# Mamo1031/Multimodal-MTRSSM

Measured on AMD Instinct MI355X. Metric: seq-steps/s (BxT) MoPoE-MRSSM train step, higher is better.
Workload: dtype bf16x2-split, fp32 accumulate; 1 GPU; BASELINE configs[1]: MoPoE-MRSSM train step, B=64/GPU T=50 deter=200 stoch=30, vision 1x64x64 + audio 1x128x32 + action 4; global_batch=64, seq_len=50, parallelism=dp1, hidden=200, embed=256, categoricals_x_classes=6x5, residual_blocks=3, activation=ELU, optimizer=AdamW lr 1e-3 + clip 10 (fused HIP), params=4151600, streams=1, launch=eager (host enqueues every launch), backend=none, rccl_ranks=0, collective_ranks=0, noise=uniforms keyed by global batch row (parallel.GlobalRowNoise)

## Files before the change

### include/mtrssm.h

```cpp
#ifndef MTRSSM_H
#define MTRSSM_H

#include <stddef.h>
#include <stdint.h>

#ifdef __cplusplus
extern "C" {
#endif

#define MTRSSM_VERSION 100

#define MTRSSM_OK 0
#define MTRSSM_EINVAL (-1)
#define MTRSSM_ELAUNCH (-2)
#define MTRSSM_ELDS (-3)

#define MTRSSM_ACT_IDENTITY 0
#define MTRSSM_ACT_RELU 1
#define MTRSSM_ACT_ELU 2
#define MTRSSM_ACT_TANH 3

int mtrssm_version(void);
const char* mtrssm_last_error(void);
const char* mtrssm_last_kernel(void);

typedef struct MtrssmMrssmDims {
  int32_t B, T;
  int32_t D, H;
  int32_t K, C;
  int32_t act;
  int32_t post;
  float kl_w_post;
  float kl_w_prior;
  int32_t rows_per_block;
  int32_t threads;
} MtrssmMrssmDims;

typedef struct MtrssmMrssmFwdWeights {
  const float* w1s_t;
  const float* w2_t;
  const float* b2;
  const float* wih_t;
  const float* bih;
  const float* whh_t;
  const float* bhh;
  const float* wh1_t;
  const float* b3;
  const float* w4;
  const float* b4;
  const float* wa2;
  const float* ba2;
  const float* wv2;
  const float* bv2;
} MtrssmMrssmFwdWeights;

typedef struct MtrssmMrssmFwdIO {
  const float* xa;
  const float* pa;
  const float* pv;
  const float* deter0;
  const float* stoch0;
  const float* u_post;
  const float* u_prior;
  float* deter;
  float* prior_logits;
  float* prior_stoch;
  float* post_logits;
  float* post_stoch;
  float* kl;
  float* sv_h1;
  float* sv_h2;
  float* sv_gates;
  float* sv_heads;
  float* sv_la;
  float* sv_lv;
  const int32_t* modality;
} MtrssmMrssmFwdIO;

int mtrssm_mrssm_rollout_fwd(const MtrssmMrssmDims* dims, const MtrssmMrssmFwdWeights* w,
                             const MtrssmMrssmFwdIO* io, void* stream);

typedef struct MtrssmMrssmClusterWeights {
  const float* w1s_t;
  const float* wf_t;
  const float* bf;
  const float* whh_t;
  const float* bhh;
  const float* wh1_t;
  const float* b3;
  const float* w4;
  const float* b4;
  const float* wa2;
  const float* ba2;
  const float* wv2;
  const float* bv2;
} MtrssmMrssmClusterWeights;
int mtrssm_mrssm_cluster_supported(const MtrssmMrssmDims* dims);
int64_t mtrssm_mrssm_cluster_workspace_bytes(const MtrssmMrssmDims* dims);
int mtrssm_mrssm_rollout_fwd_cluster(const MtrssmMrssmDims* dims, const MtrssmMrssmClusterWeights* weights, const MtrssmMrssmFwdIO* io,
                                     void* workspace, int64_t workspace_bytes, void* stream);

typedef struct MtrssmMrssmBwdWeights {
  const float* w1s_t;
  const float* w2;
  const float* wih;
  const float* whh;
  const float* wh1;
  const float* w4;
  const float* wa2;
  const float* wv2;
} MtrssmMrssmBwdWeights;

typedef struct MtrssmMrssmBwdIO {
  const float* deter0;
  const float* deter;
  const float* prior_logits;
  const float* post_logits;
  const float* sv_h1;
  const float* sv_h2;
  const float* sv_gates;
  const float* sv_heads;
  const float* sv_la;
  const float* sv_lv;
  const float* g_deter;
  const float* g_post_stoch;
  const float* g_prior_stoch;
  const float* g_post_logits;
  const float* g_prior_logits;
  const float* g_kl;
  float* g_deter0;
  float* g_stoch0;
  float* d_z1;
  float* d_h2;
  float* d_gi;
  float* d_gh;
  float* d_zh;
  float* d_lp;
  float* d_la;
  float* d_lv;
  const int32_t* modality;
} MtrssmMrssmBwdIO;

int64_t mtrssm_mrssm_cluster_bwd_workspace_bytes(const MtrssmMrssmDims* dims);
int mtrssm_mrssm_rollout_bwd_cluster(const MtrssmMrssmDims* dims, const MtrssmMrssmClusterWeights* weights, const MtrssmMrssmBwdIO* io,
                                     void* workspace, int64_t workspace_bytes, void* stream);

int mtrssm_mrssm_wide_supported(const MtrssmMrssmDims* dims, int32_t pieces);
int64_t mtrssm_mrssm_wide_workspace_bytes(const MtrssmMrssmDims* dims, int32_t pieces);
int64_t mtrssm_mrssm_wide_bwd_workspace_bytes(const MtrssmMrssmDims* dims, int32_t pieces);
int mtrssm_mrssm_rollout_fwd_wide(const MtrssmMrssmDims* dims, const MtrssmMrssmClusterWeights* weights, const MtrssmMrssmFwdIO* io,
                                  int32_t pieces, void* workspace, int64_t workspace_bytes, void* stream);
int mtrssm_mrssm_rollout_bwd_wide(const MtrssmMrssmDims* dims, const MtrssmMrssmClusterWeights* weights, const MtrssmMrssmBwdIO* io,
                                  int32_t pieces, void* workspace, int64_t workspace_bytes, void* stream);

int mtrssm_mrssm_rollout_bwd(const MtrssmMrssmDims* dims, const MtrssmMrssmBwdWeights* w,
                             const MtrssmMrssmBwdIO* io, void* stream);

typedef struct MtrssmMmtrssmDims {
  int32_t B, T;
  int32_t LD, HD;
  int32_t H;
  int32_t KL, CL;
  int32_t KH, CH;
  int32_t act;
  int32_t post;
  float tau_l, tau_h;
  float keep_l, keep_h;
  float kl_w_post, kl_w_prior;
  int32_t rows_per_block;
  int32_t threads;
} MtrssmMmtrssmDims;

typedef struct MtrssmMmtrssmFwdWeights {
  const float* wxl_s_t;
  const float* wdl_t;
  const float* wxh_t;
  const float* wdh_t;
  const float* bh;
  const float* wl1_t;
  const float* bl1;
  const float* wh1_t;
  const float* bh1;
  const float* wlp2;
  const float* blp2;
  const float* wa2;
  const float* ba2;
  const float* wv2;
  const float* bv2;
  const float* whp2;
  const float* bhp2;
  const float* whq2;
  const float* bhq2;
} MtrssmMmtrssmFwdWeights;

typedef struct MtrssmMmtrssmFwdIO {
  const float* xl;
  const float* pa;
  const float* pv;
  const float* deter_l0;
  const float* deter_h0;
  const float* hidden_l0;
  const float* hidden_h0;
  const float* stoch_l0;
  const float* stoch_h0;
  const float* u_post_l;
  const float* u_post_h;
  const float* u_prior_l;
  const float* u_prior_h;
  float* deter_l;
  float* deter_h;
  float* hidden_l;
  float* hidden_h;
  float* prior_logits_l;
  float* prior_logits_h;
  float* prior_stoch_l;
  float* prior_stoch_h;
  float* post_logits_l;
  float* post_logits_h;
  float* post_stoch_l;
  float* post_stoch_h;
  float* kl_l;
  float* kl_h;
  float* sv_l1;
  float* sv_h1;
  float* sv_la;
  float* sv_lv;
  const int32_t* modality;
} MtrssmMmtrssmFwdIO;

int mtrssm_mmtrssm_rollout_fwd(const MtrssmMmtrssmDims* dims, const MtrssmMmtrssmFwdWeights* w,
                               const MtrssmMmtrssmFwdIO* io, void* stream);

typedef struct MtrssmMmtrssmBwdWeights {
  const float* wxl_s_t;
  const float* wdl;
  const float* wxh_t;
  const float* wdh;
  const float* wl1;
  const float* wh1;
  const float* wlp2;
  const float* wa2;
  const float* wv2;
  const float* whp2;
  const float* whq2;
} MtrssmMmtrssmBwdWeights;

typedef struct MtrssmMmtrssmBwdIO {
  const float* deter_l0;
  const float* deter_h0;
  const float* deter_l;
  const float* deter_h;
  const float* prior_logits_l;
  const float* prior_logits_h;
  const float* post_logits_l;
  const float* post_logits_h;
  const float* sv_l1;
  const float* sv_h1;
  const float* sv_la;
  const float* sv_lv;
  const float* g_deter_l;
  const float* g_deter_h;
  const float* g_hidden_l;
  const float* g_hidden_h;
  const float* g_post_stoch_l;
  const float* g_post_stoch_h;
  const float* g_prior_stoch_l;
  const float* g_prior_stoch_h;
  const float* g_post_logits_l;
  const float* g_post_logits_h;
  const float* g_prior_logits_l;
  const float* g_prior_logits_h;
  const float* g_kl_l;
  const float* g_kl_h;
  float* g_deter_l0;
  float* g_deter_h0;
  float* g_hidden_l0;
  float* g_hidden_h0;
  float* g_stoch_l0;
  float* g_stoch_h0;
  float* d_ul;
  float* d_uh;
  float* d_zl1;
  float* d_zh1;
  float* d_lpl;
  float* d_la;
  float* d_lv;
  float* d_lph;
  float* d_lqh;
  const int32_t* modality;
} MtrssmMmtrssmBwdIO;

int mtrssm_mmtrssm_rollout_bwd(const MtrssmMmtrssmDims* dims, const MtrssmMmtrssmBwdWeights* w,
                               const MtrssmMmtrssmBwdIO* io, void* stream);

int mtrssm_mmtrssm_wide_supported(const MtrssmMmtrssmDims* dims, int32_t pieces);
int64_t mtrssm_mmtrssm_wide_workspace_bytes(const MtrssmMmtrssmDims* dims, int32_t pieces);
int64_t mtrssm_mmtrssm_wide_bwd_workspace_bytes(const MtrssmMmtrssmDims* dims, int32_t pieces);
int mtrssm_mmtrssm_rollout_fwd_wide(const MtrssmMmtrssmDims* dims, const MtrssmMmtrssmFwdWeights* w, const MtrssmMmtrssmFwdIO* io,
                                    int32_t pieces, void* workspace, int64_t workspace_bytes, void* stream);
int mtrssm_mmtrssm_rollout_bwd_wide(const MtrssmMmtrssmDims* dims, const MtrssmMmtrssmBwdWeights* w, const MtrssmMmtrssmBwdIO* io,
                                    int32_t pieces, void* workspace, int64_t workspace_bytes, void* stream);

typedef struct MtrssmConvGeom {
  int32_t N;
  int32_t C, Hs, Ws;
  int32_t C2;
  int32_t Cpad;
  int32_t KH, KW;
  int32_t SS, TS, OFFY, OFFX;
  int32_t Hq, Wq;
  int32_t OS, QY, QX;
  int32_t Ho, Wo;
  int32_t Cout, CoutPad;
  int32_t pre_act;
  int32_t act;
  int32_t mfma_split;
} MtrssmConvGeom;

int mtrssm_conv_gather_gemm(const MtrssmConvGeom* g, const float* src, const float* src2, const float* wp, const uint16_t* wq,
                            const float* bias, const float* actgrad_in, const float* add_in, float* out, void* stream);
int mtrssm_conv_gather_gemm_pair(const MtrssmConvGeom* ga, const float* srca, const float* src2a, const float* wpa, const uint16_t* wqa,
                                 const float* biasa, const float* actgrada, const float* adda, float* outa,
                                 const MtrssmConvGeom* gb, const float* srcb, const float* src2b, const float* wpb, const uint16_t* wqb,
                                 const float* biasb, const float* actgradb, const float* addb, float* outb, void* stream);
int mtrssm_conv_gather_pair_merges(const MtrssmConvGeom* ga, const MtrssmConvGeom* gb, int32_t has_wq);
int mtrssm_residual_block_fwd_supported(const MtrssmConvGeom* g3);
int mtrssm_residual_block_fwd(const MtrssmConvGeom* ga, const float* xa, const uint16_t* wq3a, const float* b3a, const float* w1a,
                              const float* b1a, float* ha, float* ya, const MtrssmConvGeom* gb, const float* xb, const uint16_t* wq3b,
                              const float* b3b, const float* w1b, const float* b1b, float* hb, float* yb, void* stream);
int mtrssm_pack_conv_weight(const float* w, int32_t O, int32_t I, int32_t KH, int32_t KW, int64_t so, int64_t si, int64_t sh,
                            int64_t sw, int32_t OPad, int32_t IPad, int32_t pieces, float* wp, uint16_t* wq, void* stream);
#define MTRSSM_PACK_DESC_WORDS 16
int mtrssm_pack_conv_weights(const int64_t* table, int32_t count, int32_t blocks_per_weight, void* stream);
int mtrssm_conv_weight_grad(const MtrssmConvGeom* g, const float* a, const float* src, const float* src2,
                            int32_t pre_act_a, float* dwp, float* dbias, void* workspace, int64_t workspace_bytes, void* stream);
int mtrssm_conv_weight_grad_deferred(const MtrssmConvGeom* g, const float* a, const float* src, const float* src2,
                                     int32_t pre_act_a, float* dwp, float* dbias, void* workspace, int64_t workspace_bytes, void* stream);
int mtrssm_conv_weight_grad_reduce(void* stream);
int mtrssm_conv_weight_grad_src_bias_supported(const MtrssmConvGeom* g, int32_t pre_act_a);
int mtrssm_residual_bwd1x1_supported(const MtrssmConvGeom* g);
int mtrssm_residual_bwd1x1(const MtrssmConvGeom* g, const float* gy, const float* h, const uint16_t* wq1t, float* gh, float* dwp,
                           float* dbias, void* workspace, int64_t workspace_bytes, int32_t defer, void* stream);
int mtrssm_conv_weight_grad_src_bias(const MtrssmConvGeom* g, const float* a, const float* src, int32_t pre_act_a, float* dwp,
                                     float* dsrc_bias, void* workspace, int64_t workspace_bytes, int32_t defer, void* stream);
int64_t mtrssm_conv_weight_grad_workspace_bytes(const MtrssmConvGeom* g, int32_t pre_act_a);
int mtrssm_unpack_conv_grads(const int64_t* table, int32_t count, int32_t blocks_per_entry, void* stream);
int mtrssm_convt_quad_supported(const MtrssmConvGeom* g4);
int mtrssm_convt_quad(const MtrssmConvGeom* ga4, const float* srca, const uint16_t* const* wqa4, const float* biasa, const float* actgrada,
                      float* outa, const MtrssmConvGeom* gb4, const float* srcb, const uint16_t* const* wqb4, const float* biasb,
                      const float* actgradb, float* outb, void* stream);
int mtrssm_convt_k4s2_thin(int32_t N, int32_t C, int32_t Hs, int32_t Ws, int32_t Cout, const float* src, const float* w,
                           const float* bias, int32_t pre_act, int32_t act, float* out, void* stream);
int mtrssm_convt_k4s2_band_supported(int32_t N, int32_t C, int32_t Hs, int32_t Ws, int32_t Cout);
int mtrssm_convt_k4s2_band(int32_t N, int32_t C, int32_t Hs, int32_t Ws, int32_t Cout, const float* src, const float* w,
                           const float* bias, int32_t pre_act, int32_t act, float* out, void* stream);
int mtrssm_conv_tgather_thin(int32_t N, int32_t O, int32_t Hs, int32_t Ws, int32_t Cout, int32_t KH, int32_t KW, int32_t stride, int32_t pad,
                             int32_t Ho, int32_t Wo, const float* y, const float* w, const float* bias, int32_t pre_act, int32_t act,
                             const float* actgrad_in, const float* add_in, float* out, void* stream);
int mtrssm_channel_sum(const float* x, int32_t N, int32_t C, int32_t HW, float* out, void* stream);

int mtrssm_episode_gather(const float* store, const int64_t* idx, const float* noise, int64_t n_episodes, int64_t B, int64_t T,
                          int64_t Tfull, int64_t E, float std_, float* input, float* target, void* stream);
int mtrssm_episode_gather_window(const float* store, const int64_t* idx, const int32_t* start, const float* noise, int64_t n_episodes,
                                 int64_t B, int64_t T, int64_t Tfull, int64_t E, float std_, float* input, float* target, void* stream);
int mtrssm_episode_gather_ragged(const float* store, const int64_t* idx, const int32_t* start, const int32_t* lengths, const float* noise,
                                 int64_t n_episodes, int64_t B, int64_t T, int64_t Tfull, int64_t E, float std_, float* input, float* target,
                                 int32_t* valid_out, void* stream);
int mtrssm_episode_gather_seeded(const float* store, const int64_t* idx, const int32_t* start, const int32_t* lengths, int32_t* valid_out,
                                 uint32_t key0, uint32_t key1, uint32_t epoch, int64_t n_episodes, int64_t B, int64_t T, int64_t Tfull,
                                 int64_t E, float std_, float* input, float* target, void* stream);

#define MTRSSM_STATE_MAX 6
typedef struct MtrssmStateTable {
  int32_t count;
  int32_t width[MTRSSM_STATE_MAX];
  int64_t src_stride[MTRSSM_STATE_MAX];
  const float* src[MTRSSM_STATE_MAX];
  const float* alt[MTRSSM_STATE_MAX];
  float* dst[MTRSSM_STATE_MAX];
} MtrssmStateTable;
int mtrssm_state_select(const MtrssmStateTable* table, const uint8_t* reset, int64_t B, void* stream);
int mtrssm_state_save(const MtrssmStateTable* table, int64_t B, int64_t steps, void* stream);
int mtrssm_state_save_at(const MtrssmStateTable* table, const int32_t* last, int64_t B, int64_t steps, void* stream);

int mtrssm_elbo_combine_fwd(const float* nll_a, const float* nll_v, const float* kl0, const float* kl1, int64_t n, float c0, float c1,
                            float* o_recon, float* o_k0, float* o_k1, float* o_loss, void* stream);
int mtrssm_elbo_combine_bwd(const float* g_recon, const float* g_k0, const float* g_k1, const float* g_loss, int64_t n, float c0, float c1,
                            float* g_nll_a, float* g_nll_v, float* g_kl0, float* g_kl1, void* stream);
int mtrssm_elbo_combine_counted_fwd(const float* nll_a, const float* nll_v, const float* kl0, const float* kl1, const float* live,
                                    const float* count, int64_t n, float c0, float c1, float* o_recon, float* o_k0, float* o_k1,
                                    float* o_loss, void* stream);
int mtrssm_elbo_combine_counted_bwd(const float* g_recon, const float* g_k0, const float* g_k1, const float* g_loss, const float* live,
                                    const float* count, int64_t n, float c0, float c1, float* g_nll_a, float* g_nll_v, float* g_kl0,
                                    float* g_kl1, void* stream);
int mtrssm_categorical_sample_fwd(const float* logits, const float* u, int64_t rows, int32_t K, int32_t C, float* logp, float* probs,
                                  float* onehot, void* stream);
int mtrssm_categorical_sample_bwd(const float* probs, const float* g_probs, const float* g_logp, int64_t rows, int32_t K, int32_t C,
                                  float* d_logits, void* stream);
int mtrssm_gaussian_nll_fwd(const float* pred, const float* target, int64_t frames, int64_t event, int32_t act,
                            float* out, void* stream);
int mtrssm_gaussian_nll_bwd(const float* pred, const float* target, const float* g_out,
                            int64_t frames, int64_t event, int32_t act, float* g_pred, void* stream);

int mtrssm_gaussian_nll_masked_fwd(const float* pred, const float* target, const float* present, const float* count,
                                   int64_t frames, int64_t event, int32_t act, float* out, void* stream);
int mtrssm_gaussian_nll_masked_bwd(const float* pred, const float* target, const float* present, const float* count,
                                   const float* g_out, int64_t frames, int64_t event, int32_t act, float* g_pred, void* stream);

int mtrssm_modality_dropout(const float* u, int64_t b_global, int64_t steps, int64_t span, float p_audio, float p_vision,
                            int64_t row0, int64_t b_local, int32_t* codes, float* present_audio, float* present_vision,
                            uint8_t* mask0, float* counts, void* stream);

int mtrssm_step_mask_ragged(const int32_t* valid, const float* u, int64_t b_global, int64_t steps, int64_t span, float p_audio,
                            float p_vision, int64_t row0, int64_t b_local, int32_t* codes, float* present_audio, float* present_vision,
                            float* live, uint8_t* mask0, int32_t* last, float* counts, void* stream);

int mtrssm_step_mask_forecast(const int32_t* valid, const float* u_mask, const float* u_context, int64_t b_global, int64_t steps,
                              int64_t span, float p_audio, float p_vision, int64_t lo, int64_t hi, int64_t row0, int64_t b_local,
                              int32_t* codes, float* seen_audio, float* seen_vision, float* target, float* observed, uint8_t* mask0,
                              int32_t* last, float* counts, void* stream);

int mtrssm_sumsq(const float* x, int64_t n, float* out, void* stream);
int mtrssm_adamw_step(float* param, const float* grad, float* exp_avg, float* exp_avg_sq, int64_t n,
                      const float* sumsq, float clip_norm, float grad_scale, float lr, float beta1,
                      float beta2, float eps, float weight_decay, int32_t step, void* stream);
int mtrssm_clear(void* p, int64_t bytes, void* stream);
int mtrssm_adamw_prepare(const float* grad, int64_t n, float* sumsq, float* state, const int32_t* status, float beta1, float beta2,
                         void* stream);
int mtrssm_adamw_apply(float* param, const float* grad, float* exp_avg, float* exp_avg_sq, const uint8_t* active, int64_t n,
                       const float* sumsq, const float* state, const int32_t* status, float clip_norm, float grad_scale, float beta1,
                       float beta2, float eps, float weight_decay, void* stream);

typedef struct MtrssmGemm {
  const float* A;
  const float* B;
  float* C;
  const float* bias;
  const float* zgrad;
  float* colsum;
  int32_t M, N, R, lda, ldb, ldc, ldz;
  int32_t a_rmajor, b_rmajor, act_a, act_b, act_out, act_z, accumulate, split_r;
  int32_t* tickets;
  int32_t n_tickets;
  int32_t mfma_split;
} MtrssmGemm;
int mtrssm_gemm(const MtrssmGemm* g, void* stream);
int mtrssm_gemm_group(const MtrssmGemm* problems, int32_t count, void* stream);

#ifdef __cplusplus
}
#endif
#endif
```

### multimodal_mtrssm_amd/_lib.py

```python

from __future__ import annotations

import ctypes as C
import os
from pathlib import Path

import torch
from torch import Tensor

_HERE = Path(__file__).resolve().parent
LIB_PATH = _HERE / "libmtrssm_hip.so"

ACT_IDS = {"Identity": 0, "ReLU": 1, "ELU": 2, "Tanh": 3}

_f = C.c_float
_i = C.c_int32
_p = C.c_void_p


def _struct(name: str, fields: list[tuple[str, type]]) -> type:
    return type(name, (C.Structure,), {"_fields_": fields})


def _ptrs(*names: str) -> list[tuple[str, type]]:
    return [(n, _p) for n in names]


MrssmDims = _struct("MtrssmMrssmDims", [
    ("B", _i), ("T", _i), ("D", _i), ("H", _i), ("K", _i), ("C", _i), ("act", _i), ("post", _i),
    ("kl_w_post", _f), ("kl_w_prior", _f), ("rows_per_block", _i), ("threads", _i),
])
MrssmFwdWeights = _struct("MtrssmMrssmFwdWeights", _ptrs(
    "w1s_t", "w2_t", "b2", "wih_t", "bih", "whh_t", "bhh", "wh1_t", "b3", "w4", "b4", "wa2", "ba2", "wv2", "bv2"))
MrssmFwdIO = _struct("MtrssmMrssmFwdIO", _ptrs(
    "xa", "pa", "pv", "deter0", "stoch0", "u_post", "u_prior",
    "deter", "prior_logits", "prior_stoch", "post_logits", "post_stoch", "kl",
    "sv_h1", "sv_h2", "sv_gates", "sv_heads", "sv_la", "sv_lv", "modality"))
MrssmClusterWeights = _struct("MtrssmMrssmClusterWeights", _ptrs(
    "w1s_t", "wf_t", "bf", "whh_t", "bhh", "wh1_t", "b3", "w4", "b4", "wa2", "ba2", "wv2", "bv2"))
MrssmBwdWeights = _struct("MtrssmMrssmBwdWeights", _ptrs("w1s_t", "w2", "wih", "whh", "wh1", "w4", "wa2", "wv2"))
MrssmBwdIO = _struct("MtrssmMrssmBwdIO", _ptrs(
    "deter0", "deter", "prior_logits", "post_logits", "sv_h1", "sv_h2", "sv_gates", "sv_heads", "sv_la", "sv_lv",
    "g_deter", "g_post_stoch", "g_prior_stoch", "g_post_logits", "g_prior_logits", "g_kl",
    "g_deter0", "g_stoch0", "d_z1", "d_h2", "d_gi", "d_gh", "d_zh", "d_lp", "d_la", "d_lv", "modality"))

MmtrssmDims = _struct("MtrssmMmtrssmDims", [
    ("B", _i), ("T", _i), ("LD", _i), ("HD", _i), ("H", _i), ("KL", _i), ("CL", _i), ("KH", _i), ("CH", _i),
    ("act", _i), ("post", _i), ("tau_l", _f), ("tau_h", _f), ("keep_l", _f), ("keep_h", _f),
    ("kl_w_post", _f), ("kl_w_prior", _f), ("rows_per_block", _i), ("threads", _i),
])
MmtrssmFwdWeights = _struct("MtrssmMmtrssmFwdWeights", _ptrs(
    "wxl_s_t", "wdl_t", "wxh_t", "wdh_t", "bh", "wl1_t", "bl1", "wh1_t", "bh1",
    "wlp2", "blp2", "wa2", "ba2", "wv2", "bv2", "whp2", "bhp2", "whq2", "bhq2"))
MmtrssmFwdIO = _struct("MtrssmMmtrssmFwdIO", _ptrs(
    "xl", "pa", "pv", "deter_l0", "deter_h0", "hidden_l0", "hidden_h0", "stoch_l0", "stoch_h0",
    "u_post_l", "u_post_h", "u_prior_l", "u_prior_h",
    "deter_l", "deter_h", "hidden_l", "hidden_h", "prior_logits_l", "prior_logits_h", "prior_stoch_l", "prior_stoch_h",
    "post_logits_l", "post_logits_h", "post_stoch_l", "post_stoch_h", "kl_l", "kl_h",
    "sv_l1", "sv_h1", "sv_la", "sv_lv", "modality"))
MmtrssmBwdWeights = _struct("MtrssmMmtrssmBwdWeights", _ptrs(
    "wxl_s_t", "wdl", "wxh_t", "wdh", "wl1", "wh1", "wlp2", "wa2", "wv2", "whp2", "whq2"))
MmtrssmBwdIO = _struct("MtrssmMmtrssmBwdIO", _ptrs(
    "deter_l0", "deter_h0", "deter_l", "deter_h", "prior_logits_l", "prior_logits_h", "post_logits_l", "post_logits_h",
    "sv_l1", "sv_h1", "sv_la", "sv_lv",
    "g_deter_l", "g_deter_h", "g_hidden_l", "g_hidden_h", "g_post_stoch_l", "g_post_stoch_h", "g_prior_stoch_l",
    "g_prior_stoch_h", "g_post_logits_l", "g_post_logits_h", "g_prior_logits_l", "g_prior_logits_h", "g_kl_l", "g_kl_h",
    "g_deter_l0", "g_deter_h0", "g_hidden_l0", "g_hidden_h0", "g_stoch_l0", "g_stoch_h0",
    "d_ul", "d_uh", "d_zl1", "d_zh1", "d_lpl", "d_la", "d_lv", "d_lph", "d_lqh", "modality"))

ConvGeom = _struct("MtrssmConvGeom", [(n, _i) for n in (
    "N", "C", "Hs", "Ws", "C2", "Cpad", "KH", "KW", "SS", "TS", "OFFY", "OFFX", "Hq", "Wq", "OS", "QY", "QX", "Ho", "Wo",
    "Cout", "CoutPad", "pre_act", "act", "mfma_split")])

Gemm = _struct("MtrssmGemm", _ptrs("A", "B", "C", "bias", "zgrad", "colsum") + [(n, _i) for n in (
    "M", "N", "R", "lda", "ldb", "ldc", "ldz", "a_rmajor", "b_rmajor", "act_a", "act_b", "act_out", "act_z", "accumulate", "split_r")]
    + [("tickets", _p), ("n_tickets", _i), ("mfma_split", _i)])

STATE_MAX = 6
StateTable = _struct("MtrssmStateTable", [
    ("count", _i), ("width", _i * STATE_MAX), ("src_stride", C.c_int64 * STATE_MAX), ("src", _p * STATE_MAX), ("alt", _p * STATE_MAX),
    ("dst", _p * STATE_MAX)])

SYMBOLS: dict[str, tuple[type | None, list[type]]] = {
    "mtrssm_version": (C.c_int, []),
    "mtrssm_last_error": (C.c_char_p, []),
    "mtrssm_last_kernel": (C.c_char_p, []),
    "mtrssm_mrssm_rollout_fwd": (C.c_int, [C.POINTER(MrssmDims), C.POINTER(MrssmFwdWeights), C.POINTER(MrssmFwdIO), _p]),
    "mtrssm_mrssm_cluster_supported": (C.c_int, [C.POINTER(MrssmDims)]),
    "mtrssm_mrssm_cluster_workspace_bytes": (C.c_int64, [C.POINTER(MrssmDims)]),
    "mtrssm_mrssm_rollout_fwd_cluster": (C.c_int, [C.POINTER(MrssmDims), C.POINTER(MrssmClusterWeights), C.POINTER(MrssmFwdIO), _p, C.c_int64, _p]),
    "mtrssm_mrssm_cluster_bwd_workspace_bytes": (C.c_int64, [C.POINTER(MrssmDims)]),
    "mtrssm_mrssm_rollout_bwd_cluster": (C.c_int, [C.POINTER(MrssmDims), C.POINTER(MrssmClusterWeights), C.POINTER(MrssmBwdIO), _p, C.c_int64, _p]),
    "mtrssm_mrssm_wide_supported": (C.c_int, [C.POINTER(MrssmDims), _i]),
    "mtrssm_mrssm_wide_workspace_bytes": (C.c_int64, [C.POINTER(MrssmDims), _i]),
    "mtrssm_mrssm_wide_bwd_workspace_bytes": (C.c_int64, [C.POINTER(MrssmDims), _i]),
    "mtrssm_mrssm_rollout_fwd_wide": (C.c_int, [C.POINTER(MrssmDims), C.POINTER(MrssmClusterWeights), C.POINTER(MrssmFwdIO), _i, _p, C.c_int64, _p]),
    "mtrssm_mrssm_rollout_bwd_wide": (C.c_int, [C.POINTER(MrssmDims), C.POINTER(MrssmClusterWeights), C.POINTER(MrssmBwdIO), _i, _p, C.c_int64, _p]),
    "mtrssm_mrssm_rollout_bwd": (C.c_int, [C.POINTER(MrssmDims), C.POINTER(MrssmBwdWeights), C.POINTER(MrssmBwdIO), _p]),
    "mtrssm_mmtrssm_rollout_fwd": (C.c_int, [C.POINTER(MmtrssmDims), C.POINTER(MmtrssmFwdWeights), C.POINTER(MmtrssmFwdIO), _p]),
    "mtrssm_mmtrssm_rollout_bwd": (C.c_int, [C.POINTER(MmtrssmDims), C.POINTER(MmtrssmBwdWeights), C.POINTER(MmtrssmBwdIO), _p]),
    "mtrssm_mmtrssm_wide_supported": (C.c_int, [C.POINTER(MmtrssmDims), _i]),
    "mtrssm_mmtrssm_wide_workspace_bytes": (C.c_int64, [C.POINTER(MmtrssmDims), _i]),
    "mtrssm_mmtrssm_wide_bwd_workspace_bytes": (C.c_int64, [C.POINTER(MmtrssmDims), _i]),
    "mtrssm_mmtrssm_rollout_fwd_wide": (C.c_int, [C.POINTER(MmtrssmDims), C.POINTER(MmtrssmFwdWeights), C.POINTER(MmtrssmFwdIO), _i, _p, C.c_int64, _p]),
    "mtrssm_mmtrssm_rollout_bwd_wide": (C.c_int, [C.POINTER(MmtrssmDims), C.POINTER(MmtrssmBwdWeights), C.POINTER(MmtrssmBwdIO), _i, _p, C.c_int64, _p]),
    "mtrssm_conv_gather_gemm": (C.c_int, [C.POINTER(ConvGeom), _p, _p, _p, _p, _p, _p, _p, _p, _p]),
    "mtrssm_conv_gather_gemm_pair": (C.c_int, [C.POINTER(ConvGeom), _p, _p, _p, _p, _p, _p, _p, _p,
                                               C.POINTER(ConvGeom), _p, _p, _p, _p, _p, _p, _p, _p, _p]),
    "mtrssm_conv_gather_pair_merges": (C.c_int, [C.POINTER(ConvGeom), C.POINTER(ConvGeom), _i]),
    "mtrssm_residual_block_fwd_supported": (C.c_int, [C.POINTER(ConvGeom)]),
    "mtrssm_residual_block_fwd": (C.c_int, [C.POINTER(ConvGeom), _p, _p, _p, _p, _p, _p, _p, C.POINTER(ConvGeom), _p, _p, _p, _p, _p, _p, _p, _p]),
    "mtrssm_pack_conv_weight": (C.c_int, [_p, _i, _i, _i, _i, C.c_int64, C.c_int64, C.c_int64, C.c_int64, _i, _i, _i, _p, _p, _p]),
    "mtrssm_pack_conv_weights": (C.c_int, [_p, _i, _i, _p]),
    "mtrssm_unpack_conv_grads": (C.c_int, [_p, _i, _i, _p]),
    "mtrssm_conv_weight_grad": (C.c_int, [C.POINTER(ConvGeom), _p, _p, _p, _i, _p, _p, _p, C.c_int64, _p]),
    "mtrssm_conv_weight_grad_deferred": (C.c_int, [C.POINTER(ConvGeom), _p, _p, _p, _i, _p, _p, _p, C.c_int64, _p]),
    "mtrssm_residual_bwd1x1_supported": (C.c_int, [C.POINTER(ConvGeom)]),
    "mtrssm_residual_bwd1x1": (C.c_int, [C.POINTER(ConvGeom), _p, _p, _p, _p, _p, _p, _p, C.c_int64, _i, _p]),
    "mtrssm_conv_weight_grad_src_bias_supported": (C.c_int, [C.POINTER(ConvGeom), _i]),
    "mtrssm_conv_weight_grad_src_bias": (C.c_int, [C.POINTER(ConvGeom), _p, _p, _i, _p, _p, _p, C.c_int64, _i, _p]),
    "mtrssm_conv_weight_grad_reduce": (C.c_int, [_p]),
    "mtrssm_conv_weight_grad_workspace_bytes": (C.c_int64, [C.POINTER(ConvGeom), _i]),
    "mtrssm_channel_sum": (C.c_int, [_p, _i, _i, _i, _p, _p]),
    "mtrssm_convt_k4s2_thin": (C.c_int, [_i, _i, _i, _i, _i, _p, _p, _p, _i, _i, _p, _p]),
    "mtrssm_convt_k4s2_band_supported": (C.c_int, [_i, _i, _i, _i, _i]),
    "mtrssm_convt_k4s2_band": (C.c_int, [_i, _i, _i, _i, _i, _p, _p, _p, _i, _i, _p, _p]),
    "mtrssm_convt_quad_supported": (C.c_int, [C.POINTER(ConvGeom)]),
    "mtrssm_convt_quad": (C.c_int, [C.POINTER(ConvGeom), _p, C.POINTER(C.c_void_p), _p, _p, _p, C.POINTER(ConvGeom), _p, C.POINTER(C.c_void_p),
                                    _p, _p, _p, _p]),
    "mtrssm_conv_tgather_thin": (C.c_int, [_i] * 11 + [_p, _p, _p, _i, _i, _p, _p, _p, _p]),
    "mtrssm_episode_gather": (C.c_int, [_p, _p, _p, C.c_int64, C.c_int64, C.c_int64, C.c_int64, C.c_int64, _f, _p, _p, _p]),
    "mtrssm_episode_gather_window": (C.c_int, [_p, _p, _p, _p, C.c_int64, C.c_int64, C.c_int64, C.c_int64, C.c_int64, _f, _p, _p, _p]),
    "mtrssm_state_select": (C.c_int, [C.POINTER(StateTable), _p, C.c_int64, _p]),
    "mtrssm_state_save": (C.c_int, [C.POINTER(StateTable), C.c_int64, C.c_int64, _p]),
    "mtrssm_state_save_at": (C.c_int, [C.POINTER(StateTable), _p, C.c_int64, C.c_int64, _p]),
    "mtrssm_episode_gather_ragged": (C.c_int, [_p, _p, _p, _p, _p, C.c_int64, C.c_int64, C.c_int64, C.c_int64, C.c_int64, _f, _p, _p, _p, _p]),
    "mtrssm_episode_gather_seeded": (C.c_int, [_p, _p, _p, _p, _p, C.c_uint32, C.c_uint32, C.c_uint32, C.c_int64, C.c_int64, C.c_int64, C.c_int64,
                                               C.c_int64, _f, _p, _p, _p]),
    "mtrssm_step_mask_ragged": (C.c_int, [_p, _p, C.c_int64, C.c_int64, C.c_int64, _f, _f, C.c_int64, C.c_int64, _p, _p, _p, _p, _p, _p, _p, _p]),
    "mtrssm_step_mask_forecast": (C.c_int, [_p, _p, _p, C.c_int64, C.c_int64, C.c_int64, _f, _f, C.c_int64, C.c_int64, C.c_int64, C.c_int64, _p, _p, _p,
                                            _p, _p, _p, _p, _p, _p]),
    "mtrssm_elbo_combine_counted_fwd": (C.c_int, [_p, _p, _p, _p, _p, _p, C.c_int64, C.c_float, C.c_float, _p, _p, _p, _p, _p]),
    "mtrssm_elbo_combine_counted_bwd": (C.c_int, [_p, _p, _p, _p, _p, _p, C.c_int64, C.c_float, C.c_float, _p, _p, _p, _p, _p]),
    "mtrssm_elbo_combine_fwd": (C.c_int, [_p, _p, _p, _p, C.c_int64, C.c_float, C.c_float, _p, _p, _p, _p, _p]),
    "mtrssm_elbo_combine_bwd": (C.c_int, [_p, _p, _p, _p, C.c_int64, C.c_float, C.c_float, _p, _p, _p, _p, _p]),
    "mtrssm_categorical_sample_fwd": (C.c_int, [_p, _p, C.c_int64, _i, _i, _p, _p, _p, _p]),
    "mtrssm_categorical_sample_bwd": (C.c_int, [_p, _p, _p, C.c_int64, _i, _i, _p, _p]),
    "mtrssm_gaussian_nll_fwd": (C.c_int, [_p, _p, C.c_int64, C.c_int64, _i, _p, _p]),
    "mtrssm_gaussian_nll_bwd": (C.c_int, [_p, _p, _p, C.c_int64, C.c_int64, _i, _p, _p]),
    "mtrssm_gaussian_nll_masked_fwd": (C.c_int, [_p, _p, _p, _p, C.c_int64, C.c_int64, _i, _p, _p]),
    "mtrssm_gaussian_nll_masked_bwd": (C.c_int, [_p, _p, _p, _p, _p, C.c_int64, C.c_int64, _i, _p, _p]),
    "mtrssm_modality_dropout": (C.c_int, [_p, C.c_int64, C.c_int64, C.c_int64, _f, _f, C.c_int64, C.c_int64, _p, _p, _p, _p, _p, _p]),
    "mtrssm_sumsq": (C.c_int, [_p, C.c_int64, _p, _p]),
    "mtrssm_adamw_step": (C.c_int, [_p, _p, _p, _p, C.c_int64, _p, _f, _f, _f, _f, _f, _f, _f, _i, _p]),
    "mtrssm_gemm": (C.c_int, [C.POINTER(Gemm), _p]),
    "mtrssm_gemm_group": (C.c_int, [C.POINTER(Gemm), _i, _p]),
    "mtrssm_clear": (C.c_int, [_p, C.c_int64, _p]),
    "mtrssm_adamw_prepare": (C.c_int, [_p, C.c_int64, _p, _p, _p, _f, _f, _p]),
    "mtrssm_adamw_apply": (C.c_int, [_p, _p, _p, _p, _p, C.c_int64, _p, _p, _p, _f, _f, _f, _f, _f, _f, _p]),
}

_LIB: C.CDLL | None = None


class MtrssmLibraryError(RuntimeError):
    """The HIP library is missing or a kernel call failed.  There is no fallback path."""


def load() -> C.CDLL:
    global _LIB
    if _LIB is not None:
        return _LIB
    path = Path(os.environ.get("MTRSSM_LIB", LIB_PATH))
    if not path.exists():
        msg = (f"{path} not found: build it with `make -C multimodal_mtrssm_amd/csrc` (or __graft_entry__.build()). "
               "multimodal_mtrssm_amd has no CPU or eager fallback for the rollout path.")
        raise MtrssmLibraryError(msg)
    lib = C.CDLL(str(path))
    for name, (res, args) in SYMBOLS.items():
        fn = getattr(lib, name)
        fn.restype = res
        fn.argtypes = args
    _LIB = lib
    return lib


def check(rc: int, what: str) -> None:
    if rc != 0:
        err = load().mtrssm_last_error()
        msg = f"{what} failed with code {rc}: {err.decode() if err else '?'}"
        raise MtrssmLibraryError(msg)


def ptr(t: Tensor | None) -> int | None:
    if t is None:
        return None
    if not t.is_cuda:
        msg = "multimodal_mtrssm_amd kernels run on MI355X only: got a CPU tensor (there is no CPU fallback)"
        raise MtrssmLibraryError(msg)
    if t.dtype != torch.float32 or not t.is_contiguous():
        msg = f"expected a contiguous float32 tensor, got {t.dtype} contiguous={t.is_contiguous()}"
        raise MtrssmLibraryError(msg)
    return t.data_ptr()


_INT32_FIELDS = frozenset({"modality"})


def index_ptr(t: Tensor | None) -> int | None:
    if t is None:
        return None
    if not t.is_cuda:
        msg = "multimodal_mtrssm_amd kernels run on MI355X only: got a CPU tensor (there is no CPU fallback)"
        raise MtrssmLibraryError(msg)
    if t.dtype != torch.int32 or not t.is_contiguous():
        msg = f"expected a contiguous int32 tensor, got {t.dtype} contiguous={t.is_contiguous()}"
        raise MtrssmLibraryError(msg)
    return t.data_ptr()


def raw_ptr(t: Tensor | None) -> int | None:
    if t is None:
        return None
    if not t.is_cuda:
        msg = "multimodal_mtrssm_amd kernels run on MI355X only: got a CPU tensor (there is no CPU fallback)"
        raise MtrssmLibraryError(msg)
    return t.data_ptr()


def stream_ptr(device: torch.device) -> int:
    return torch.cuda.current_stream(device).cuda_stream


class KernelTimers:

    def __init__(self) -> None:
        self.on = False
        self._rows: dict[str, list[tuple[torch.cuda.Event, torch.cuda.Event, float, float]]] = {}

    def enable(self) -> None:
        self.on = True
        self._rows = {}

    def disable(self) -> None:
        self.on = False

    def call(self, name: str, fn, *args, flops: float = 0.0, nbytes: float = 0.0) -> int:
        if not self.on:
            return fn(*args)
        start, end = torch.cuda.Event(enable_timing=True), torch.cuda.Event(enable_timing=True)
        start.record()
        rc = fn(*args)
        end.record()
        kernel = load().mtrssm_last_kernel()
        key = kernel.decode() if kernel else name
        self._rows.setdefault(key, []).append((start, end, flops, nbytes))
        return rc

    def summary(self) -> dict[str, dict[str, float]]:
        torch.cuda.synchronize()
        out: dict[str, dict[str, float]] = {}
        for k, rows in self._rows.items():
            total = sum(s.elapsed_time(e) for s, e, _, _ in rows)
            out[k] = {"launches": len(rows), "total_ms": total, "avg_ms": total / len(rows),
                      "flops": sum(r[2] for r in rows), "bytes": sum(r[3] for r in rows)}
        return out


TIMERS = KernelTimers()


def fill(struct: C.Structure, **tensors: Tensor | None) -> C.Structure:
    struct._refs = tensors
    for name, _ in struct._fields_:
        setattr(struct, name, index_ptr(tensors.get(name)) if name in _INT32_FIELDS else ptr(tensors.get(name)))
    unknown = set(tensors) - {n for n, _ in struct._fields_}
    if unknown:
        msg = f"unknown fields for {type(struct).__name__}: {sorted(unknown)}"
        raise KeyError(msg)
    return struct
```

### multimodal_mtrssm_amd/csrc/capi.hip

```cpp
#include <stdarg.h>
#include <stdio.h>

#include "scan_common.h"

namespace mtrssm {

static thread_local char g_err[512] = "";
static thread_local const char* g_kernel = "";

void set_last_kernel(const char* name) { g_kernel = name; }

void set_error(const char* fmt, ...) {
  va_list ap;
  va_start(ap, fmt);
  vsnprintf(g_err, sizeof(g_err), fmt, ap);
  va_end(ap);
}

int mrssm_fwd_launch(const MtrssmMrssmDims*, const MtrssmMrssmFwdWeights*, const MtrssmMrssmFwdIO*, hipStream_t);
int mrssm_bwd_launch(const MtrssmMrssmDims*, const MtrssmMrssmBwdWeights*, const MtrssmMrssmBwdIO*, hipStream_t);
int mmtrssm_fwd_launch(const MtrssmMmtrssmDims*, const MtrssmMmtrssmFwdWeights*, const MtrssmMmtrssmFwdIO*, hipStream_t);
int mmtrssm_bwd_launch(const MtrssmMmtrssmDims*, const MtrssmMmtrssmBwdWeights*, const MtrssmMmtrssmBwdIO*, hipStream_t);
int conv_gather_gemm_launch(const MtrssmConvGeom*, const float*, const float*, const float*, const unsigned short*, const float*, const float*, const float*, float*, hipStream_t);
int episode_gather_launch(const float*, const int64_t*, const float*, int64_t, int64_t, int64_t, int64_t, int64_t, float, float*, float*, hipStream_t);
int episode_gather_window_launch(const float*, const int64_t*, const int32_t*, const float*, int64_t, int64_t, int64_t, int64_t, int64_t, float, float*,
                                 float*, hipStream_t);
int state_select_launch(const MtrssmStateTable*, const unsigned char*, int64_t, hipStream_t);
int state_save_launch(const MtrssmStateTable*, int64_t, int64_t, hipStream_t);
int state_save_at_launch(const MtrssmStateTable*, const int32_t*, int64_t, int64_t, hipStream_t);
int episode_gather_ragged_launch(const float*, const int64_t*, const int32_t*, const int32_t*, const float*, int64_t, int64_t, int64_t, int64_t,
                                 int64_t, float, float*, float*, int32_t*, hipStream_t);
int episode_gather_seeded_launch(const float*, const int64_t*, const int32_t*, const int32_t*, int32_t*, uint32_t, uint32_t, uint32_t, int64_t, int64_t,
                                 int64_t, int64_t, int64_t, float, float*, float*, hipStream_t);
int step_mask_ragged_launch(const int32_t*, const float*, int64_t, int64_t, int64_t, float, float, int64_t, int64_t, int32_t*, float*, float*, float*,
                            unsigned char*, int32_t*, float*, hipStream_t);
int step_mask_forecast_launch(const int32_t*, const float*, const float*, int64_t, int64_t, int64_t, float, float, int64_t, int64_t, int64_t, int64_t,
                              int32_t*, float*, float*, float*, float*, unsigned char*, int32_t*, float*, hipStream_t);
int elbo_combine_counted_fwd_launch(const float*, const float*, const float*, const float*, const float*, const float*, int64_t, float, float, float*,
                                    float*, float*, float*, hipStream_t);
int elbo_combine_counted_bwd_launch(const float*, const float*, const float*, const float*, const float*, const float*, int64_t, float, float, float*,
                                    float*, float*, float*, hipStream_t);
int conv_gather_gemm_pair_launch(const MtrssmConvGeom*, const float*, const float*, const float*, const unsigned short*, const float*, const float*, const float*, float*,
                                 const MtrssmConvGeom*, const float*, const float*, const float*, const unsigned short*, const float*, const float*, const float*, float*, hipStream_t);
int conv_residual_fwd_supported(const MtrssmConvGeom*);
int conv_residual_fwd_launch(const MtrssmConvGeom*, const float*, const unsigned short*, const float*, const float*, const float*, float*, float*,
                             const MtrssmConvGeom*, const float*, const unsigned short*, const float*, const float*, const float*, float*, float*, hipStream_t);
int pack_conv_weight_launch(const float*, int, int, int, int, long, long, long, long, int, int, int, float*, unsigned short*, hipStream_t);
int pack_conv_weights_launch(const int64_t*, int, int, hipStream_t);
int conv_gather_pair_merges(const MtrssmConvGeom*, const MtrssmConvGeom*, bool);
int conv_weight_grad_launch(const MtrssmConvGeom*, const float*, const float*, const float*, int, float*, float*, void*, size_t, size_t*, hipStream_t);
int conv_weight_grad_deferred_launch(const MtrssmConvGeom*, const float*, const float*, const float*, int, float*, float*, void*, size_t, hipStream_t);
int conv_weight_grad_reduce_flush(hipStream_t);
int conv_residual_bwd1x1_supported(const MtrssmConvGeom*);
int conv_residual_bwd1x1_launch(const MtrssmConvGeom*, const float*, const float*, const unsigned short*, float*, float*, float*, void*, size_t, int,
                                hipStream_t);
int conv_weight_grad_src_bias_supported(const MtrssmConvGeom*, int);
int conv_weight_grad_src_bias_launch(const MtrssmConvGeom*, const float*, const float*, int, float*, float*, void*, size_t, int, hipStream_t);
int channel_sum_launch(const float*, int, int, int, float*, hipStream_t);
int convt_k4s2_band_supported(int, int, int, int, int);
int convt_k4s2_band_launch(int, int, int, int, int, const float*, const float*, const float*, int, int, float*, hipStream_t);
int convt_k4s2_thin_launch(int, int, int, int, int, const float*, const float*, const float*, int, int, float*, hipStream_t);
int conv_convt_quad_supported(const MtrssmConvGeom*);
int conv_convt_quad_launch(const MtrssmConvGeom*, const float*, const unsigned short* const*, const float*, const float*, float*,
                           const MtrssmConvGeom*, const float*, const unsigned short* const*, const float*, const float*, float*, hipStream_t);
int conv_tgather_thin_launch(int, int, int, int, int, int, int, int, int, int, int, const float*, const float*, const float*, int, int, const float*,
                             const float*, float*, hipStream_t);
int categorical_sample_fwd_launch(const float*, const float*, int64_t, int, int, float*, float*, float*, hipStream_t);
int categorical_sample_bwd_launch(const float*, const float*, const float*, int64_t, int, int, float*, hipStream_t);
int elbo_combine_fwd_launch(const float*, const float*, const float*, const float*, int64_t, float, float, float*, float*, float*, float*, hipStream_t);
int elbo_combine_bwd_launch(const float*, const float*, const float*, const float*, int64_t, float, float, float*, float*, float*, float*, hipStream_t);
int nll_fwd_launch(const float*, const float*, int64_t, int64_t, int, float*, hipStream_t);
int nll_bwd_launch(const float*, const float*, const float*, int64_t, int64_t, int, float*, hipStream_t);
int nll_masked_fwd_launch(const float*, const float*, const float*, const float*, int64_t, int64_t, int, float*, hipStream_t);
int nll_masked_bwd_launch(const float*, const float*, const float*, const float*, const float*, int64_t, int64_t, int, float*, hipStream_t);
int modality_dropout_launch(const float*, int64_t, int64_t, int64_t, float, float, int64_t, int64_t, int32_t*, float*, float*, unsigned char*, float*,
                            hipStream_t);
int sumsq_launch(const float*, int64_t, float*, hipStream_t);
int adamw_launch(float*, const float*, float*, float*, int64_t, const float*, float, float, float, float, float, float, float, int, hipStream_t);
int gemm_launch(const MtrssmGemm*, hipStream_t);
int gemm_group_launch(const MtrssmGemm*, int, hipStream_t);
int debug_set_cluster_profile(void*);
int debug_set_resident_profile(void*);
int debug_set_wide_profile(void*);
int debug_set_mmt_profile(void*);
int mrssm_cluster_supported(const MtrssmMrssmDims*);
size_t mrssm_cluster_workspace_bytes(const MtrssmMrssmDims*);
size_t mrssm_cluster_bwd_workspace_bytes(const MtrssmMrssmDims*);
int mrssm_bwd_cluster_launch(const MtrssmMrssmDims*, const MtrssmMrssmClusterWeights*, const MtrssmMrssmBwdIO*, void*, size_t, hipStream_t);
int mrssm_fwd_cluster_launch(const MtrssmMrssmDims*, const MtrssmMrssmClusterWeights*, const MtrssmMrssmFwdIO*, void*, size_t, hipStream_t);
int unpack_conv_grads_launch(const int64_t*, int, int, hipStream_t);
int mrssm_wide_supported(const MtrssmMrssmDims*, int);
size_t mrssm_wide_workspace_bytes(const MtrssmMrssmDims*, int);
size_t mrssm_wide_bwd_workspace_bytes(const MtrssmMrssmDims*, int);
int mrssm_wide_fwd_launch(const MtrssmMrssmDims*, const MtrssmMrssmClusterWeights*, const MtrssmMrssmFwdIO*, int, void*, size_t, hipStream_t);
int mrssm_wide_bwd_launch(const MtrssmMrssmDims*, const MtrssmMrssmClusterWeights*, const MtrssmMrssmBwdIO*, int, void*, size_t, hipStream_t);
int adamw_prepare_launch(const float*, int64_t, float*, float*, const int*, float, float, hipStream_t);
int adamw_apply_launch(float*, const float*, float*, float*, const unsigned char*, int64_t, const float*, const float*, const int*, float, float, float,
                       float, float, float, hipStream_t);

int mmtrssm_wide_supported(const MtrssmMmtrssmDims*, int);
size_t mmtrssm_wide_workspace_bytes(const MtrssmMmtrssmDims*, int);
size_t mmtrssm_wide_bwd_workspace_bytes(const MtrssmMmtrssmDims*, int);
int mmtrssm_wide_fwd_launch(const MtrssmMmtrssmDims*, const MtrssmMmtrssmFwdWeights*, const MtrssmMmtrssmFwdIO*, int, void*, size_t, hipStream_t);
int mmtrssm_wide_bwd_launch(const MtrssmMmtrssmDims*, const MtrssmMmtrssmBwdWeights*, const MtrssmMmtrssmBwdIO*, int, void*, size_t, hipStream_t);

int device_cu_count() {
  static int cached[64] = {0};
  int dev = 0;
  if (hipGetDevice(&dev) != hipSuccess) { (void)hipGetLastError(); return 0; }
  if (dev < 0 || dev >= 64) return 0;
  if (cached[dev] > 0) return cached[dev];
  int v = 0;
  if (hipDeviceGetAttribute(&v, hipDeviceAttributeMultiprocessorCount, dev) != hipSuccess || v <= 0) { (void)hipGetLastError(); return 0; }
  cached[dev] = v;
  return v;
}

}

using namespace mtrssm;
#define MTRSSM_API extern "C" __attribute__((visibility("default")))

MTRSSM_API int mtrssm_version(void) { return MTRSSM_VERSION; }
MTRSSM_API const char* mtrssm_last_error(void) { return g_err; }
MTRSSM_API const char* mtrssm_last_kernel(void) { return g_kernel; }

MTRSSM_API int mtrssm_mrssm_rollout_fwd(const MtrssmMrssmDims* d, const MtrssmMrssmFwdWeights* w, const MtrssmMrssmFwdIO* io, void* stream) {
  return mrssm_fwd_launch(d, w, io, static_cast<hipStream_t>(stream));
}
MTRSSM_API int mtrssm_mrssm_rollout_bwd(const MtrssmMrssmDims* d, const MtrssmMrssmBwdWeights* w, const MtrssmMrssmBwdIO* io, void* stream) {
  return mrssm_bwd_launch(d, w, io, static_cast<hipStream_t>(stream));
}
MTRSSM_API int mtrssm_mmtrssm_rollout_fwd(const MtrssmMmtrssmDims* d, const MtrssmMmtrssmFwdWeights* w, const MtrssmMmtrssmFwdIO* io, void* stream) {
  return mmtrssm_fwd_launch(d, w, io, static_cast<hipStream_t>(stream));
}
MTRSSM_API int mtrssm_mmtrssm_rollout_bwd(const MtrssmMmtrssmDims* d, const MtrssmMmtrssmBwdWeights* w, const MtrssmMmtrssmBwdIO* io, void* stream) {
  return mmtrssm_bwd_launch(d, w, io, static_cast<hipStream_t>(stream));
}
MTRSSM_API int mtrssm_categorical_sample_fwd(const float* logits, const float* u, int64_t rows, int32_t K, int32_t C, float* logp, float* probs,
                                            float* onehot, void* stream) {
  return categorical_sample_fwd_launch(logits, u, rows, K, C, logp, probs, onehot, static_cast<hipStream_t>(stream));
}
MTRSSM_API int mtrssm_categorical_sample_bwd(const float* probs, const float* g_probs, const float* g_logp, int64_t rows, int32_t K, int32_t C,
                                            float* d_logits, void* stream) {
  return categorical_sample_bwd_launch(probs, g_probs, g_logp, rows, K, C, d_logits, static_cast<hipStream_t>(stream));
}
MTRSSM_API int mtrssm_elbo_combine_fwd(const float* nll_a, const float* nll_v, const float* kl0, const float* kl1, int64_t n, float c0, float c1,
                                      float* o_recon, float* o_k0, float* o_k1, float* o_loss, void* stream) {
  return elbo_combine_fwd_launch(nll_a, nll_v, kl0, kl1, n, c0, c1, o_recon, o_k0, o_k1, o_loss, static_cast<hipStream_t>(stream));
}
MTRSSM_API int mtrssm_elbo_combine_bwd(const float* g_recon, const float* g_k0, const float* g_k1, const float* g_loss, int64_t n, float c0,
                                      float c1, float* g_nll_a, float* g_nll_v, float* g_kl0, float* g_kl1, void* stream) {
  return elbo_combine_bwd_launch(g_recon, g_k0, g_k1, g_loss, n, c0, c1, g_nll_a, g_nll_v, g_kl0, g_kl1, static_cast<hipStream_t>(stream));
}
MTRSSM_API int mtrssm_gaussian_nll_fwd(const float* pred, const float* target, int64_t frames, int64_t event, int32_t act, float* out, void* stream) {
  return nll_fwd_launch(pred, target, frames, event, act, out, static_cast<hipStream_t>(stream));
}
MTRSSM_API int mtrssm_gaussian_nll_bwd(const float* pred, const float* target, const float* g_out, int64_t frames, int64_t event, int32_t act,
                                       float* g_pred, void* stream) {
  return nll_bwd_launch(pred, target, g_out, frames, event, act, g_pred, static_cast<hipStream_t>(stream));
}
MTRSSM_API int mtrssm_gaussian_nll_masked_fwd(const float* pred, const float* target, const float* present, const float* count, int64_t frames,
                                              int64_t event, int32_t act, float* out, void* stream) {
  return nll_masked_fwd_launch(pred, target, present, count, frames, event, act, out, static_cast<hipStream_t>(stream));
}
MTRSSM_API int mtrssm_gaussian_nll_masked_bwd(const float* pred, const float* target, const float* present, const float* count,
                                              const float* g_out, int64_t frames, int64_t event, int32_t act, float* g_pred, void* stream) {
  return nll_masked_bwd_launch(pred, target, present, count, g_out, frames, event, act, g_pred, static_cast<hipStream_t>(stream));
}
MTRSSM_API int mtrssm_modality_dropout(const float* u, int64_t b_global, int64_t steps, int64_t span, float p_audio, float p_vision, int64_t row0,
                                       int64_t b_local, int32_t* codes, float* present_audio, float* present_vision, uint8_t* mask0,
                                       float* counts, void* stream) {
  return modality_dropout_launch(u, b_global, steps, span, p_audio, p_vision, row0, b_local, codes, present_audio, present_vision, mask0, counts,
                                 static_cast<hipStream_t>(stream));
}
MTRSSM_API int mtrssm_sumsq(const float* x, int64_t n, float* out, void* stream) {
  return sumsq_launch(x, n, out, static_cast<hipStream_t>(stream));
}
MTRSSM_API int mtrssm_adamw_step(float* param, const float* grad, float* exp_avg, float* exp_avg_sq, int64_t n, const float* sumsq,
                                 float clip_norm, float grad_scale, float lr, float beta1, float beta2, float eps, float weight_decay,
                                 int32_t step, void* stream) {
  return adamw_launch(param, grad, exp_avg, exp_avg_sq, n, sumsq, clip_norm, grad_scale, lr, beta1, beta2, eps, weight_decay, step,
                      static_cast<hipStream_t>(stream));
}
MTRSSM_API int mtrssm_unpack_conv_grads(const int64_t* table, int32_t count, int32_t blocks_per_entry, void* stream) {
  return unpack_conv_grads_launch(table, count, blocks_per_entry, static_cast<hipStream_t>(stream));
}
MTRSSM_API int mtrssm_mrssm_cluster_supported(const MtrssmMrssmDims* d) { return mrssm_cluster_supported(d); }
MTRSSM_API int64_t mtrssm_mrssm_cluster_workspace_bytes(const MtrssmMrssmDims* d) { return (int64_t)mrssm_cluster_workspace_bytes(d); }
MTRSSM_API int mtrssm_mrssm_rollout_fwd_cluster(const MtrssmMrssmDims* d, const MtrssmMrssmClusterWeights* w, const MtrssmMrssmFwdIO* io,
                                                void* workspace, int64_t workspace_bytes, void* stream) {
  return mrssm_fwd_cluster_launch(d, w, io, workspace, workspace_bytes < 0 ? 0 : (size_t)workspace_bytes, static_cast<hipStream_t>(stream));
}
extern "C" __attribute__((visibility("default"))) int mtrssm_debug_set_cluster_profile(void* buf) { return debug_set_cluster_profile(buf); }
extern "C" __attribute__((visibility("default"))) int mtrssm_debug_set_resident_profile(void* buf) { return debug_set_resident_profile(buf); }
extern "C" __attribute__((visibility("default"))) int mtrssm_debug_set_wide_profile(void* buf) { return debug_set_wide_profile(buf); }
extern "C" __attribute__((visibility("default"))) int mtrssm_debug_set_mmt_profile(void* buf) { return debug_set_mmt_profile(buf); }
MTRSSM_API int64_t mtrssm_mrssm_cluster_bwd_workspace_bytes(const MtrssmMrssmDims* d) { return (int64_t)mrssm_cluster_bwd_workspace_bytes(d); }
MTRSSM_API int mtrssm_mrssm_rollout_bwd_cluster(const MtrssmMrssmDims* d, const MtrssmMrssmClusterWeights* w, const MtrssmMrssmBwdIO* io,
                                                void* workspace, int64_t workspace_bytes, void* stream) {
  return mrssm_bwd_cluster_launch(d, w, io, workspace, workspace_bytes < 0 ? 0 : (size_t)workspace_bytes, static_cast<hipStream_t>(stream));
}
MTRSSM_API int mtrssm_mrssm_wide_supported(const MtrssmMrssmDims* d, int32_t pieces) { return mrssm_wide_supported(d, pieces); }
MTRSSM_API int64_t mtrssm_mrssm_wide_workspace_bytes(const MtrssmMrssmDims* d, int32_t pieces) { return (int64_t)mrssm_wide_workspace_bytes(d, pieces); }
MTRSSM_API int64_t mtrssm_mrssm_wide_bwd_workspace_bytes(const MtrssmMrssmDims* d, int32_t pieces) {
  return (int64_t)mrssm_wide_bwd_workspace_bytes(d, pieces);
}
MTRSSM_API int mtrssm_mrssm_rollout_fwd_wide(const MtrssmMrssmDims* d, const MtrssmMrssmClusterWeights* w, const MtrssmMrssmFwdIO* io, int32_t pieces,
                                             void* workspace, int64_t workspace_bytes, void* stream) {
  return mrssm_wide_fwd_launch(d, w, io, pieces, workspace, workspace_bytes < 0 ? 0 : (size_t)workspace_bytes, static_cast<hipStream_t>(stream));
}
MTRSSM_API int mtrssm_mrssm_rollout_bwd_wide(const MtrssmMrssmDims* d, const MtrssmMrssmClusterWeights* w, const MtrssmMrssmBwdIO* io, int32_t pieces,
                                             void* workspace, int64_t workspace_bytes, void* stream) {
  return mrssm_wide_bwd_launch(d, w, io, pieces, workspace, workspace_bytes < 0 ? 0 : (size_t)workspace_bytes, static_cast<hipStream_t>(stream));
}
MTRSSM_API int mtrssm_mmtrssm_wide_supported(const MtrssmMmtrssmDims* d, int32_t pieces) { return mmtrssm_wide_supported(d, pieces); }
MTRSSM_API int64_t mtrssm_mmtrssm_wide_workspace_bytes(const MtrssmMmtrssmDims* d, int32_t pieces) { return (int64_t)mmtrssm_wide_workspace_bytes(d, pieces); }
MTRSSM_API int64_t mtrssm_mmtrssm_wide_bwd_workspace_bytes(const MtrssmMmtrssmDims* d, int32_t pieces) {
  return (int64_t)mmtrssm_wide_bwd_workspace_bytes(d, pieces);
}
MTRSSM_API int mtrssm_mmtrssm_rollout_fwd_wide(const MtrssmMmtrssmDims* d, const MtrssmMmtrssmFwdWeights* w, const MtrssmMmtrssmFwdIO* io, int32_t pieces,
                                               void* workspace, int64_t workspace_bytes, void* stream) {
  return mmtrssm_wide_fwd_launch(d, w, io, pieces, workspace, workspace_bytes < 0 ? 0 : (size_t)workspace_bytes, static_cast<hipStream_t>(stream));
}
MTRSSM_API int mtrssm_mmtrssm_rollout_bwd_wide(const MtrssmMmtrssmDims* d, const MtrssmMmtrssmBwdWeights* w, const MtrssmMmtrssmBwdIO* io, int32_t pieces,
                                               void* workspace, int64_t workspace_bytes, void* stream) {
  return mmtrssm_wide_bwd_launch(d, w, io, pieces, workspace, workspace_bytes < 0 ? 0 : (size_t)workspace_bytes, static_cast<hipStream_t>(stream));
}
MTRSSM_API int mtrssm_gemm(const MtrssmGemm* g, void* stream) { return gemm_launch(g, static_cast<hipStream_t>(stream)); }
MTRSSM_API int mtrssm_gemm_group(const MtrssmGemm* problems, int32_t count, void* stream) {
  return gemm_group_launch(problems, count, static_cast<hipStream_t>(stream));
}
MTRSSM_API int mtrssm_clear(void* p, int64_t bytes, void* stream) {
  return clear_async(p, bytes < 0 ? 0 : (size_t)bytes, static_cast<hipStream_t>(stream));
}
MTRSSM_API int mtrssm_adamw_prepare(const float* grad, int64_t n, float* sumsq, float* state, const int32_t* status, float beta1, float beta2,
                                    void* stream) {
  return adamw_prepare_launch(grad, n, sumsq, state, status, beta1, beta2, static_cast<hipStream_t>(stream));
}
MTRSSM_API int mtrssm_adamw_apply(float* param, const float* grad, float* exp_avg, float* exp_avg_sq, const uint8_t* active, int64_t n,
                                  const float* sumsq, const float* state, const int32_t* status, float clip_norm, float grad_scale, float beta1,
                                  float beta2, float eps, float weight_decay, void* stream) {
  return adamw_apply_launch(param, grad, exp_avg, exp_avg_sq, active, n, sumsq, state, status, clip_norm, grad_scale, beta1, beta2, eps,
                            weight_decay, static_cast<hipStream_t>(stream));
}
MTRSSM_API int mtrssm_conv_gather_gemm(const MtrssmConvGeom* g, const float* src, const float* src2, const float* wp, const uint16_t* wq,
                                       const float* bias, const float* actgrad_in, const float* add_in, float* out, void* stream) {
  return conv_gather_gemm_launch(g, src, src2, wp, wq, bias, actgrad_in, add_in, out, static_cast<hipStream_t>(stream));
}
MTRSSM_API int mtrssm_episode_gather(const float* store, const int64_t* idx, const float* noise, int64_t n_episodes, int64_t B, int64_t T,
                                     int64_t Tfull, int64_t E, float std_, float* input, float* target, void* stream) {
  return episode_gather_launch(store, idx, noise, n_episodes, B, T, Tfull, E, std_, input, target, static_cast<hipStream_t>(stream));
}
MTRSSM_API int mtrssm_episode_gather_window(const float* store, const int64_t* idx, const int32_t* start, const float* noise, int64_t n_episodes,
                                            int64_t B, int64_t T, int64_t Tfull, int64_t E, float std_, float* input, float* target, void* stream) {
  return episode_gather_window_launch(store, idx, start, noise, n_episodes, B, T, Tfull, E, std_, input, target, static_cast<hipStream_t>(stream));
}
MTRSSM_API int mtrssm_state_select(const MtrssmStateTable* table, const uint8_t* reset, int64_t B, void* stream) {
  return state_select_launch(table, reset, B, static_cast<hipStream_t>(stream));
}
MTRSSM_API int mtrssm_state_save(const MtrssmStateTable* table, int64_t B, int64_t steps, void* stream) {
  return state_save_launch(table, B, steps, static_cast<hipStream_t>(stream));
}
MTRSSM_API int mtrssm_state_save_at(const MtrssmStateTable* table, const int32_t* last, int64_t B, int64_t steps, void* stream) {
  return state_save_at_launch(table, last, B, steps, static_cast<hipStream_t>(stream));
}
MTRSSM_API int mtrssm_episode_gather_ragged(const float* store, const int64_t* idx, const int32_t* start, const int32_t* lengths,
                                            const float* noise, int64_t n_episodes, int64_t B, int64_t T, int64_t Tfull, int64_t E, float std_,
                                            float* input, float* target, int32_t* valid_out, void* stream) {
  return episode_gather_ragged_launch(store, idx, start, lengths, noise, n_episodes, B, T, Tfull, E, std_, input, target, valid_out,
                                      static_cast<hipStream_t>(stream));
}
MTRSSM_API int mtrssm_episode_gather_seeded(const float* store, const int64_t* idx, const int32_t* start, const int32_t* lengths,
                                            int32_t* valid_out, uint32_t key0, uint32_t key1, uint32_t epoch, int64_t n_episodes, int64_t B,
                                            int64_t T, int64_t Tfull, int64_t E, float std_, float* input, float* target, void* stream) {
  return episode_gather_seeded_launch(store, idx, start, lengths, valid_out, key0, key1, epoch, n_episodes, B, T, Tfull, E, std_, input, target,
                                      static_cast<hipStream_t>(stream));
}
MTRSSM_API int mtrssm_step_mask_ragged(const int32_t* valid, const float* u, int64_t b_global, int64_t steps, int64_t span, float p_audio,
                                       float p_vision, int64_t row0, int64_t b_local, int32_t* codes, float* present_audio,
                                       float* present_vision, float* live, uint8_t* mask0, int32_t* last, float* counts, void* stream) {
  return step_mask_ragged_launch(valid, u, b_global, steps, span, p_audio, p_vision, row0, b_local, codes, present_audio, present_vision, live,
                                 mask0, last, counts, static_cast<hipStream_t>(stream));
}
MTRSSM_API int mtrssm_step_mask_forecast(const int32_t* valid, const float* u_mask, const float* u_context, int64_t b_global, int64_t steps,
                                         int64_t span, float p_audio, float p_vision, int64_t lo, int64_t hi, int64_t row0, int64_t b_local,
                                         int32_t* codes, float* seen_audio, float* seen_vision, float* target, float* observed, uint8_t* mask0,
                                         int32_t* last, float* counts, void* stream) {
  return step_mask_forecast_launch(valid, u_mask, u_context, b_global, steps, span, p_audio, p_vision, lo, hi, row0, b_local, codes, seen_audio,
                                   seen_vision, target, observed, mask0, last, counts, static_cast<hipStream_t>(stream));
}
MTRSSM_API int mtrssm_elbo_combine_counted_fwd(const float* nll_a, const float* nll_v, const float* kl0, const float* kl1, const float* live,
                                               const float* count, int64_t n, float c0, float c1, float* o_recon, float* o_k0, float* o_k1,
                                               float* o_loss, void* stream) {
  return elbo_combine_counted_fwd_launch(nll_a, nll_v, kl0, kl1, live, count, n, c0, c1, o_recon, o_k0, o_k1, o_loss,
                                         static_cast<hipStream_t>(stream));
}
MTRSSM_API int mtrssm_elbo_combine_counted_bwd(const float* g_recon, const float* g_k0, const float* g_k1, const float* g_loss, const float* live,
                                               const float* count, int64_t n, float c0, float c1, float* g_nll_a, float* g_nll_v, float* g_kl0,
                                               float* g_kl1, void* stream) {
  return elbo_combine_counted_bwd_launch(g_recon, g_k0, g_k1, g_loss, live, count, n, c0, c1, g_nll_a, g_nll_v, g_kl0, g_kl1,
                                         static_cast<hipStream_t>(stream));
}
MTRSSM_API int mtrssm_conv_gather_gemm_pair(const MtrssmConvGeom* ga, const float* srca, const float* src2a, const float* wpa, const uint16_t* wqa,
                                            const float* biasa, const float* actgrada, const float* adda, float* outa,
                                            const MtrssmConvGeom* gb, const float* srcb, const float* src2b, const float* wpb, const uint16_t* wqb,
                                            const float* biasb, const float* actgradb, const float* addb, float* outb, void* stream) {
  return conv_gather_gemm_pair_launch(ga, srca, src2a, wpa, wqa, biasa, actgrada, adda, outa, gb, srcb, src2b, wpb, wqb, biasb, actgradb, addb,
                                      outb, static_cast<hipStream_t>(stream));
}
MTRSSM_API int mtrssm_residual_block_fwd_supported(const MtrssmConvGeom* g3) { return conv_residual_fwd_supported(g3) != 0; }
MTRSSM_API int mtrssm_residual_block_fwd(const MtrssmConvGeom* ga, const float* xa, const uint16_t* wq3a, const float* b3a, const float* w1a,
                                         const float* b1a, float* ha, float* ya, const MtrssmConvGeom* gb, const float* xb, const uint16_t* wq3b,
                                         const float* b3b, const float* w1b, const float* b1b, float* hb, float* yb, void* stream) {
  return conv_residual_fwd_launch(ga, xa, wq3a, b3a, w1a, b1a, ha, ya, gb, xb, wq3b, b3b, w1b, b1b, hb, yb, static_cast<hipStream_t>(stream));
}
MTRSSM_API int mtrssm_pack_conv_weight(const float* w, int32_t O, int32_t I, int32_t KH, int32_t KW, int64_t so, int64_t si, int64_t sh,
                                       int64_t sw, int32_t OPad, int32_t IPad, int32_t pieces, float* wp, uint16_t* wq, void* stream) {
  return pack_conv_weight_launch(w, O, I, KH, KW, so, si, sh, sw, OPad, IPad, pieces, wp, wq, static_cast<hipStream_t>(stream));
}
MTRSSM_API int mtrssm_conv_gather_pair_merges(const MtrssmConvGeom* ga, const MtrssmConvGeom* gb, int32_t has_wq) {
  return conv_gather_pair_merges(ga, gb, has_wq != 0);
}
MTRSSM_API int mtrssm_pack_conv_weights(const int64_t* table, int32_t count, int32_t blocks_per_weight, void* stream) {
  return pack_conv_weights_launch(table, count, blocks_per_weight, static_cast<hipStream_t>(stream));
}
MTRSSM_API int mtrssm_conv_weight_grad(const MtrssmConvGeom* g, const float* a, const float* src, const float* src2, int32_t pre_act_a,
                                       float* dwp, float* dbias, void* workspace, int64_t workspace_bytes, void* stream) {
  return conv_weight_grad_launch(g, a, src, src2, pre_act_a, dwp, dbias, workspace, workspace_bytes < 0 ? 0 : (size_t)workspace_bytes, nullptr,
                                 static_cast<hipStream_t>(stream));
}
MTRSSM_API int mtrssm_conv_weight_grad_deferred(const MtrssmConvGeom* g, const float* a, const float* src, const float* src2, int32_t pre_act_a,
                                               float* dwp, float* dbias, void* workspace, int64_t workspace_bytes, void* stream) {
  return conv_weight_grad_deferred_launch(g, a, src, src2, pre_act_a, dwp, dbias, workspace, workspace_bytes < 0 ? 0 : (size_t)workspace_bytes,
                                          static_cast<hipStream_t>(stream));
}
MTRSSM_API int mtrssm_residual_bwd1x1_supported(const MtrssmConvGeom* g) { return conv_residual_bwd1x1_supported(g) != 0; }
MTRSSM_API int mtrssm_residual_bwd1x1(const MtrssmConvGeom* g, const float* gy, const float* h, const uint16_t* wq1t, float* gh, float* dwp,
                                      float* dbias, void* workspace, int64_t workspace_bytes, int32_t defer, void* stream) {
  return conv_residual_bwd1x1_launch(g, gy, h, wq1t, gh, dwp, dbias, workspace, workspace_bytes < 0 ? 0 : (size_t)workspace_bytes, defer,
                                     static_cast<hipStream_t>(stream));
}
MTRSSM_API int mtrssm_conv_weight_grad_src_bias_supported(const MtrssmConvGeom* g, int32_t pre_act_a) {
  return conv_weight_grad_src_bias_supported(g, pre_act_a);
}
MTRSSM_API int mtrssm_conv_weight_grad_src_bias(const MtrssmConvGeom* g, const float* a, const float* src, int32_t pre_act_a, float* dwp,
                                                float* dsrc_bias, void* workspace, int64_t workspace_bytes, int32_t defer, void* stream) {
  return conv_weight_grad_src_bias_launch(g, a, src, pre_act_a, dwp, dsrc_bias, workspace, workspace_bytes < 0 ? 0 : (size_t)workspace_bytes,
                                          defer, static_cast<hipStream_t>(stream));
}
MTRSSM_API int mtrssm_conv_weight_grad_reduce(void* stream) { return conv_weight_grad_reduce_flush(static_cast<hipStream_t>(stream)); }
MTRSSM_API int64_t mtrssm_conv_weight_grad_workspace_bytes(const MtrssmConvGeom* g, int32_t pre_act_a) {
  size_t need = 0;
  if (conv_weight_grad_launch(g, nullptr, nullptr, nullptr, pre_act_a, nullptr, nullptr, nullptr, 0, &need, nullptr) != MTRSSM_OK) return -1;
  return (int64_t)need;
}
MTRSSM_API int mtrssm_channel_sum(const float* x, int32_t N, int32_t C, int32_t HW, float* out, void* stream) {
  return channel_sum_launch(x, N, C, HW, out, static_cast<hipStream_t>(stream));
}
MTRSSM_API int mtrssm_conv_tgather_thin(int32_t N, int32_t O, int32_t Hs, int32_t Ws, int32_t Cout, int32_t KH, int32_t KW, int32_t stride,
                                        int32_t pad, int32_t Ho, int32_t Wo, const float* y, const float* w, const float* bias, int32_t pre_act,
                                        int32_t act, const float* actgrad_in, const float* add_in, float* out, void* stream) {
  return conv_tgather_thin_launch(N, O, Hs, Ws, Cout, KH, KW, stride, pad, Ho, Wo, y, w, bias, pre_act, act, actgrad_in, add_in, out,
                                  static_cast<hipStream_t>(stream));
}
MTRSSM_API int mtrssm_convt_quad_supported(const MtrssmConvGeom* g4) { return conv_convt_quad_supported(g4); }
MTRSSM_API int mtrssm_convt_quad(const MtrssmConvGeom* ga4, const float* srca, const uint16_t* const* wqa4, const float* biasa,
                                 const float* actgrada, float* outa, const MtrssmConvGeom* gb4, const float* srcb,
                                 const uint16_t* const* wqb4, const float* biasb, const float* actgradb, float* outb, void* stream) {
  return conv_convt_quad_launch(ga4, srca, reinterpret_cast<const unsigned short* const*>(wqa4), biasa, actgrada, outa, gb4, srcb,
                                reinterpret_cast<const unsigned short* const*>(wqb4), biasb, actgradb, outb,
                                static_cast<hipStream_t>(stream));
}
MTRSSM_API int mtrssm_convt_k4s2_band_supported(int32_t N, int32_t C, int32_t Hs, int32_t Ws, int32_t Cout) {
  return convt_k4s2_band_supported(N, C, Hs, Ws, Cout);
}
MTRSSM_API int mtrssm_convt_k4s2_band(int32_t N, int32_t C, int32_t Hs, int32_t Ws, int32_t Cout, const float* src, const float* w,
                                     const float* bias, int32_t pre_act, int32_t act, float* out, void* stream) {
  return convt_k4s2_band_launch(N, C, Hs, Ws, Cout, src, w, bias, pre_act, act, out, static_cast<hipStream_t>(stream));
}
MTRSSM_API int mtrssm_convt_k4s2_thin(int32_t N, int32_t C, int32_t Hs, int32_t Ws, int32_t Cout, const float* src, const float* w,
                                      const float* bias, int32_t pre_act, int32_t act, float* out, void* stream) {
  return convt_k4s2_thin_launch(N, C, Hs, Ws, Cout, src, w, bias, pre_act, act, out, static_cast<hipStream_t>(stream));
}
```

### multimodal_mtrssm_amd/csrc/mrssm_cluster.hip

```cpp
#include "scan_common.h"

namespace mtrssm {

void set_error(const char* fmt, ...);
void set_last_kernel(const char* name);
int device_cu_count();

constexpr int kClu = 4;
constexpr int kCluThreads = 256;
constexpr unsigned kSpinLimit = 1u << 22;

__device__ unsigned long long* g_cluster_prof = nullptr;
#define MTRSSM_CLU_STAMP(i)                                                                                  \
  do {                                                                                                       \
    if (prof && t >= 8 && t < 12) prof[(t - 8) * 16 + (i)] = __builtin_readcyclecounter();                   \
  } while (0)

__device__ __forceinline__ void granule_store(unsigned long long* p, unsigned epoch, float v) {
  __hip_atomic_store(p, ((unsigned long long)epoch << 32) | (unsigned long long)__float_as_uint(v), __ATOMIC_RELAXED,
                     __HIP_MEMORY_SCOPE_AGENT);
}

template <int NJ>
__device__ __forceinline__ bool wave_gather(const unsigned long long* g, float* dst, int total, unsigned epoch, int lane) {
  unsigned done = 0;
  const unsigned full = (1u << NJ) - 1u;
#pragma unroll
  for (int j = 0; j < NJ; ++j)
    if (lane + 64 * j >= total) done |= 1u << j;
  for (unsigned spins = 0;; ++spins) {
#pragma unroll
    for (int j = 0; j < NJ; ++j) {
      if (!(done & (1u << j))) {
        const unsigned long long x = __hip_atomic_load(g + lane + 64 * j, __ATOMIC_RELAXED, __HIP_MEMORY_SCOPE_AGENT);
        if ((unsigned)(x >> 32) == epoch) {
          dst[lane + 64 * j] = __uint_as_float((unsigned)x);
          done |= 1u << j;
        }
      }
    }
    if (__all(done == full)) return true;
    if (spins > kSpinLimit) return false;
    __builtin_amdgcn_s_sleep(1);
  }
}

template <int DH, int NP, int PPT, bool MASKED>
__global__ __launch_bounds__(kCluThreads) void mrssm_fwd_cluster_kernel(const MtrssmMrssmDims dm, const MtrssmMrssmClusterWeights w,
                                                                        const MtrssmMrssmFwdIO io, unsigned long long* __restrict__ gran,
                                                                        int* __restrict__ status, int nclusters) {
  extern __shared__ __attribute__((aligned(16))) float lds[];
  constexpr int D = DH, H = DH;
  constexpr int UD = D / kClu, UH = H / kClu;
  constexpr int NG = 3 * UD, NH = 3 * UH;
  constexpr int KP = DH / NP;
  constexpr int NPIECE = 2 * NG * NP;
  static_assert(KP % 4 == 0 && DH % NP == 0, "pieces are whole float4 runs");
  static_assert(PPT * kCluThreads >= NPIECE, "every piece has a thread");
  const int K = dm.K, C = dm.C, S = K * C, T = dm.T, act = dm.act;
  const int tid = threadIdx.x, lane = tid & (kWave - 1), wave = tid / kWave;
  const int blk = blockIdx.x;
  const int member = (blk >> 3) & (kClu - 1);
  const int cluster = (blk & 7) + 8 * (blk >> 5);
  if (cluster >= nclusters) return;

  int o = 0;
  auto take = [&](int n) { const int r = o; o += (n + 3) & ~3; return r; };
  const int Ls = take(S), Lh1 = take(DH), Ld0 = take(DH), Ld1 = take(DH), Lhd = take(3 * 64);
  const int Llp = take(S), Lla = take(S), Llv = take(S), Lmx = take(S);
  const int Lpart = take(kClu * 3 * S);
  const int Lred = take(NPIECE > NH * NP ? NPIECE : NH * NP);
  const int Lw1 = take(S * H);
  const int Lwh = take(D * NH);
  const int Lbl = take(3 * S);
  const int Lu = take(2 * 64);
  const int Lflag = take(4);
  (void)o;
  int* abort_flag = reinterpret_cast<int*>(lds + Lflag);

  float wreg[PPT][KP];
  int xsel[PPT];
#pragma unroll
  for (int i = 0; i < PPT; ++i) {
    const int pc = tid * PPT + i;
    const int pcc = pc < NPIECE ? pc : NPIECE - 1;
    const int col = pcc / NP, part = pcc - col * NP;
    const bool is_h = col >= NG;
    const int og = is_h ? col - NG : col;
    const int gcol = (og / UD) * D + member * UD + (og % UD);
    const float* src = (is_h ? w.whh_t : w.wf_t) + (size_t)(part * KP) * 3 * D + gcol;
    xsel[i] = (is_h ? 1 : 0) | (part * KP) << 1;
#pragma unroll
    for (int k = 0; k < KP; ++k) wreg[i][k] = src[(size_t)k * 3 * D];
  }
  float wrow[64];
  {
    const bool roleL = tid < 3 * S;
    const int which = roleL ? tid / S : 0, srow = roleL ? tid - which * S : 0;
    const float* rowsrc = (which == 0 ? w.w4 : (which == 1 ? w.wa2 : w.wv2)) + (size_t)srow * H + member * UH;
#pragma unroll
    for (int k = 0; k < 64; ++k) wrow[k] = k < UH ? rowsrc[k] : 0.f;
  }
  for (int idx = tid; idx < S * H; idx += kCluThreads) lds[Lw1 + idx] = w.w1s_t[idx];
  for (int idx = tid; idx < D * NH; idx += kCluThreads) {
    const int k = idx / NH, oh = idx - k * NH;
    lds[Lwh + idx] = w.wh1_t[(size_t)k * 3 * H + (oh / UH) * H + member * UH + (oh % UH)];
  }
  for (int i = tid; i < 3 * 64; i += kCluThreads) lds[Lhd + i] = 0.f;
  for (int i = tid; i < 3 * S; i += kCluThreads) {
    const int which = i / S, s2 = i - which * S;
    lds[Lbl + i] = (which == 0 ? w.b4 : (which == 1 ? w.ba2 : w.bv2))[s2];
  }
  float bias_g[6] = {0.f, 0.f, 0.f, 0.f, 0.f, 0.f};
  if (tid < UD) {
#pragma unroll
    for (int g = 0; g < 3; ++g) {
      bias_g[g] = w.bf[g * D + member * UD + tid];
      bias_g[3 + g] = w.bhh[g * D + member * UD + tid];
    }
  }
  const float bias_h = (tid < UH) ? w.b3[member * UH + tid] : 0.f;
  if (tid == 0) *abort_flag = 0;

  const int slotsD = UD, slotsL = 3 * S;
  const int per_parity = kClu * (slotsD + slotsL);
  unsigned long long* gbase = gran + (size_t)cluster * 2 * per_parity;
  unsigned epoch = 0;
  unsigned long long* prof = (blockIdx.x == 0 && tid == 0) ? g_cluster_prof : nullptr;

  for (int row = cluster; row < dm.B; row += nclusters) {
    int cur = Ld0, nxt = Ld1;
    lds_barrier();
    for (int i = tid; i < D; i += kCluThreads) lds[cur + i] = io.deter0[(size_t)row * D + i];
    for (int i = tid; i < S; i += kCluThreads) lds[Ls + i] = io.stoch0[(size_t)row * S + i];
    lds_barrier();

    auto load_inputs = [&](size_t q, float& xa_r, float& pa_r, float& up_r, float& ur_r, int& code_r) {
      code_r = modality_code<MASKED>(io.modality, q);
      xa_r = tid < H ? io.xa[q * H + tid] : 0.f;
      pa_r = 0.f;
      if (tid >= UH && tid < NH) {
        const int which = tid / UH, u = tid - which * UH;
        pa_r = (which == 1 ? io.pa : io.pv)[q * H + member * UH + u];
      }
      up_r = (wave == 3 && lane < K) ? io.u_post[q * K + lane] : 0.f;
      ur_r = (wave == 3 && lane < K && io.u_prior) ? io.u_prior[q * K + lane] : 0.f;
    };
    float xa_n, pav_n, up_n, ur_n;
    int code_n;
    load_inputs((size_t)row * T, xa_n, pav_n, up_n, ur_n, code_n);

    for (int t = 0; t < T; ++t) {
      const size_t bt = (size_t)row * T + t;
      unsigned long long* gpar = gbase + (size_t)(t & 1) * per_parity;
      const float xa_v = xa_n, pav = pav_n;
      const int code = code_n;
      if (wave == 3 && lane < K) { lds[Lu + lane] = up_n; lds[Lu + 64 + lane] = ur_n; }
      if (t + 1 < T) load_inputs(bt + 1, xa_n, pav_n, up_n, ur_n, code_n);

      MTRSSM_CLU_STAMP(0);
      if (tid < H) {
        const float* wc = lds + Lw1 + tid;
        float a0 = xa_v, a1 = 0.f, a2 = 0.f, a3 = 0.f;
        int k = 0;
        for (; k + 8 <= S; k += 8) {
          float wv[8], sv[8];
#pragma unroll
          for (int i = 0; i < 8; ++i) { wv[i] = wc[(size_t)(k + i) * H]; sv[i] = lds[Ls + k + i]; }
          a0 = fmaf(wv[0], sv[0], a0); a1 = fmaf(wv[1], sv[1], a1); a2 = fmaf(wv[2], sv[2], a2); a3 = fmaf(wv[3], sv[3], a3);
          a0 = fmaf(wv[4], sv[4], a0); a1 = fmaf(wv[5], sv[5], a1); a2 = fmaf(wv[6], sv[6], a2); a3 = fmaf(wv[7], sv[7], a3);
        }
        for (; k < S; ++k) a0 = fmaf(wc[(size_t)k * H], lds[Ls + k], a0);
        const float h = act_fwd((a0 + a1) + (a2 + a3), act);
        lds[Lh1 + tid] = h;
        if (member == 0 && io.sv_h1) io.sv_h1[bt * H + tid] = h;
      }
      lds_barrier();

      MTRSSM_CLU_STAMP(1);
#pragma unroll
      for (int i = 0; i < PPT; ++i) {
        const float* xv = lds + ((xsel[i] & 1) ? cur : Lh1) + (xsel[i] >> 1);
        float a0 = 0.f, a1 = 0.f, a2 = 0.f, a3 = 0.f;
#pragma unroll
        for (int k = 0; k < KP; k += 4) {
          const float4 x = *reinterpret_cast<const float4*>(xv + k);
          a0 = fmaf(wreg[i][k], x.x, a0);
          a1 = fmaf(wreg[i][k + 1], x.y, a1);
          a2 = fmaf(wreg[i][k + 2], x.z, a2);
          a3 = fmaf(wreg[i][k + 3], x.w, a3);
        }
        if (tid * PPT + i < NPIECE) lds[Lred + tid * PPT + i] = (a0 + a1) + (a2 + a3);
      }
      lds_barrier();

      MTRSSM_CLU_STAMP(2);
      ++epoch;
      if (tid < UD) {
        float gs[6];
#pragma unroll
        for (int g = 0; g < 6; ++g) {
          const float* pr = lds + Lred + ((g < 3 ? g : g - 3) * UD + tid + (g < 3 ? 0 : NG)) * NP;
          float a = bias_g[g];
#pragma unroll
          for (int q = 0; q < NP; ++q) a += pr[q];
          gs[g] = a;
        }
        const float rg = __fdividef(1.f, 1.f + __expf(-(gs[3] + gs[0])));
        const float zg = __fdividef(1.f, 1.f + __expf(-(gs[4] + gs[1])));
        const float ng = 1.f - __fdividef(2.f, __expf(2.f * (gs[2] + gs[5] * rg)) + 1.f);
        const int unit = member * UD + tid;
        const float dnew = (lds[cur + unit] - ng) * zg + ng;
        lds[nxt + unit] = dnew;
        granule_store(gpar + (size_t)member * slotsD + tid, epoch, dnew);
        io.deter[bt * D + unit] = dnew;
        if (io.sv_gates) {
          float* gsv = io.sv_gates + bt * 4 * D;
          gsv[unit] = rg; gsv[D + unit] = zg; gsv[2 * D + unit] = ng; gsv[3 * D + unit] = gs[5];
        }
      }
      if (wave == 3) {
        const bool ok = wave_gather<4>(gpar, lds + nxt, D, epoch, lane);
        if (!ok && lane == 0) { *abort_flag = 1; atomicExch(status, 1 + 2 * t); }
      }
      lds_barrier();
      if (*abort_flag) return;

      MTRSSM_CLU_STAMP(3);
      for (int pc = tid; pc < NH * NP; pc += kCluThreads) {
        const int oh = pc / NP, part = pc - oh * NP;
        const float* wcol = lds + Lwh + (size_t)(part * KP) * NH + oh;
        const float* dv = lds + nxt + part * KP;
        float p0 = 0.f, p1 = 0.f, p2 = 0.f, p3 = 0.f;
#pragma unroll
        for (int k = 0; k < KP; k += 8) {
          float wv[8];
#pragma unroll
          for (int i = 0; i < 8; ++i) wv[i] = k + i < KP ? wcol[(size_t)(k + i) * NH] : 0.f;
          const float4 d0 = *reinterpret_cast<const float4*>(dv + k);
          const float4 d1 = k + 4 < KP ? *reinterpret_cast<const float4*>(dv + k + 4) : make_float4(0.f, 0.f, 0.f, 0.f);
          p0 = fmaf(wv[0], d0.x, p0); p1 = fmaf(wv[1], d0.y, p1); p2 = fmaf(wv[2], d0.z, p2); p3 = fmaf(wv[3], d0.w, p3);
          p0 = fmaf(wv[4], d1.x, p0); p1 = fmaf(wv[5], d1.y, p1); p2 = fmaf(wv[6], d1.z, p2); p3 = fmaf(wv[7], d1.w, p3);
        }
        lds[Lred + pc] = (p0 + p1) + (p2 + p3);
      }
      lds_barrier();
      if (tid < NH) {
        float z = tid < UH ? bias_h : pav;
#pragma unroll
        for (int q = 0; q < NP; ++q) z += lds[Lred + tid * NP + q];
        const float h = act_fwd(z, act);
        const int which = tid / UH, u = tid - which * UH;
        lds[Lhd + which * 64 + u] = h;
        if (io.sv_heads) io.sv_heads[bt * 3 * H + which * H + member * UH + u] = h;
      }
      lds_barrier();

      MTRSSM_CLU_STAMP(4);
      ++epoch;
      unsigned long long* gl = gpar + (size_t)kClu * slotsD;
      if (tid < 3 * S) {
        const float* hv = lds + Lhd + (tid / S) * 64;
        float p0 = 0.f, p1 = 0.f;
#pragma unroll
        for (int u = 0; u < 64; u += 4) {
          const float4 x = *reinterpret_cast<const float4*>(hv + u);
          p0 = fmaf(wrow[u], x.x, p0);
          p1 = fmaf(wrow[u + 1], x.y, p1);
          p0 = fmaf(wrow[u + 2], x.z, p0);
          p1 = fmaf(wrow[u + 3], x.w, p1);
        }
        const float p = p0 + p1;
        lds[Lpart + member * 3 * S + tid] = p;
        granule_store(gl + (size_t)member * slotsL + tid, epoch, p);
      }
      if (wave == 3) {
        const bool ok = wave_gather<6>(gl, lds + Lpart, kClu * 3 * S, epoch, lane);
        if (!ok && lane == 0) { *abort_flag = 1; atomicExch(status, 2 + 2 * t); }
      }
      lds_barrier();
      if (*abort_flag) return;

      MTRSSM_CLU_STAMP(5);
      if (wave == 3) {
        const bool writer = member == 0;
        for (int i = lane; i < 3 * S; i += kWave) {
          const int which = i / S, s2 = i - which * S;
          float v = lds[Lbl + i];
#pragma unroll
          for (int m2 = 0; m2 < kClu; ++m2) v += lds[Lpart + m2 * 3 * S + i];
          lds[(which == 0 ? Llp : (which == 1 ? Lla : Llv)) + s2] = v;
        }
        wave_mopoe_mix_masked<true, MASKED>(lds + Lla, lds + Llv, lds + Llp, lds + Lmx, S, lane, code);
        for (int s = lane; s < S; s += kWave) {
          if (writer) {
            io.prior_logits[bt * S + s] = lds[Llp + s];
            io.post_logits[bt * S + s] = lds[Lmx + s];
            if (io.sv_la) { io.sv_la[bt * S + s] = lds[Lla + s]; io.sv_lv[bt * S + s] = lds[Llv + s]; }
          }
        }
        float kl = C <= 8 ? cat_block_fwd_fast8(lds + Lmx, lds + Llp, K, C, lane, lds + Lu, io.u_prior ? lds + Lu + 64 : nullptr, lds + Ls,
                                                io.post_stoch + bt * S, io.prior_stoch ? io.prior_stoch + bt * S : nullptr, writer)
                          : cat_block_fwd<true, true>(lds + Lmx, lds + Llp, K, C, lane, lds + Lu, io.u_prior ? lds + Lu + 64 : nullptr, lds + Ls,
                                                      io.post_stoch + bt * S, io.prior_stoch ? io.prior_stoch + bt * S : nullptr, writer);
        if (io.kl) {
          kl = wave_sum(kl);
          if (lane == 0 && writer) io.kl[bt] = kl;
        }
      }
      lds_barrier();
      MTRSSM_CLU_STAMP(7);
      const int tmp = cur; cur = nxt; nxt = tmp;
    }
  }
}

template <int NJ, typename Map>
__device__ __forceinline__ bool wave_gather_map(int total, unsigned epoch, int lane, Map map) {
  unsigned done = 0;
  const unsigned full = (1u << NJ) - 1u;
#pragma unroll
  for (int j = 0; j < NJ; ++j)
    if (lane + 64 * j >= total) done |= 1u << j;
  for (unsigned spins = 0;; ++spins) {
#pragma unroll
    for (int j = 0; j < NJ; ++j) {
      if (!(done & (1u << j))) {
        const unsigned long long* slot;
        float* dst;
        map(lane + 64 * j, slot, dst);
        const unsigned long long x = __hip_atomic_load(slot, __ATOMIC_RELAXED, __HIP_MEMORY_SCOPE_AGENT);
        if ((unsigned)(x >> 32) == epoch) {
          *dst = __uint_as_float((unsigned)x);
          done |= 1u << j;
        }
      }
    }
    if (__all(done == full)) return true;
    if (spins > kSpinLimit) return false;
    __builtin_amdgcn_s_sleep(1);
  }
}

template <int DH, int NPB, int PPT, bool MASKED>
__global__ __launch_bounds__(kCluThreads) void mrssm_bwd_cluster_kernel(const MtrssmMrssmDims dm, const MtrssmMrssmClusterWeights w,
                                                                        const MtrssmMrssmBwdIO io, unsigned long long* __restrict__ gran,
                                                                        int* __restrict__ status, int nclusters) {
  extern __shared__ __attribute__((aligned(16))) float lds[];
  constexpr int D = DH, H = DH;
  constexpr int UD = D / kClu, UH = H / kClu;
  constexpr int NG = 3 * UD, NH = 3 * UH;
  constexpr int NHP = (NH + 3) & ~3;
  constexpr int KPB = NG / NPB;
  constexpr int NPIECE = 2 * DH * NPB;
  constexpr int W1P = 8;
  constexpr int KW1 = (DH + W1P - 1) / W1P;
  static_assert(NG % NPB == 0 && KPB % 2 == 0, "row pieces are whole float2 runs");
  static_assert(PPT * kCluThreads >= NPIECE, "every row piece has a thread");
  const int K = dm.K, C = dm.C, S = K * C, T = dm.T, act = dm.act;
  const int tid = threadIdx.x, lane = tid & (kWave - 1), wave = tid / kWave;
  const int blk = blockIdx.x;
  const int member = (blk >> 3) & (kClu - 1);
  const int cluster = (blk & 7) + 8 * (blk >> 5);
  if (cluster >= nclusters) return;

  int o = 0;
  auto take = [&](int n) { const int r = o; o += (n + 3) & ~3; return r; };
  const int Lla = take(S), Llv = take(S), Lmx = take(S), Llp = take(S), Ldmx = take(S), Ldlp = take(S), Ldla = take(S), Ldlv = take(S);
  const int Lgps = take(S), Lcs = take(S);
  const int Lhd = take(NHP), Ldzh = take(NHP);
  const int Lgate = take(4 * UD), Ldprev = take(UD), Lgd = take(UD), Lcd = take(UD);
  const int Ldg = take(2 * NG);
  const int Lh1 = take(DH), Ldz1 = take(DH);
  const int Lpdd = take(kClu * UD);
  const int Lpcd = take(kClu * UD), Lpdh = take(kClu * DH);
  const int Lred = take(NPIECE > DH ? NPIECE : DH);
  const int Lred2 = take(W1P * 64 > 3 * 64 ? W1P * 64 : 3 * 64);
  const int Lwh = take(D * NHP);
  const int Lw2 = take(32 * NHP);
  const int Lflag = take(4);
  (void)o;
  int* abort_flag = reinterpret_cast<int*>(lds + Lflag);
  float* gk_lds = lds + Lflag + 1;

  float wreg[PPT][KPB];
#pragma unroll
  for (int i = 0; i < PPT; ++i) {
    const int pc = tid * PPT + i;
    const int pcc = pc < NPIECE ? pc : NPIECE - 1;
    const int rowi = pcc / NPB, part = pcc - rowi * NPB;
    const bool is_f = rowi >= DH;
    const float* src = (is_f ? w.wf_t : w.whh_t) + (size_t)(is_f ? rowi - DH : rowi) * 3 * D;
#pragma unroll
    for (int k = 0; k < KPB; ++k) {
      const int og = part * KPB + k;
      wreg[i][k] = src[(og / UD) * D + member * UD + (og % UD)];
    }
  }
  for (int idx = tid; idx < 32 * NHP; idx += kCluThreads) {
    const int s2 = idx / NHP, j = idx - s2 * NHP;
    float v = 0.f;
    if (s2 < S && j < NH) {
      const int which = j / UH, u = j - which * UH;
      v = (which == 0 ? w.w4 : (which == 1 ? w.wa2 : w.wv2))[(size_t)s2 * H + member * UH + u];
    }
    lds[Lw2 + idx] = v;
  }
  float w1r[KW1];
  {
    const int srow = tid / W1P < S ? tid / W1P : 0, part = tid % W1P;
#pragma unroll
    for (int k = 0; k < KW1; ++k) {
      const int kk = part * KW1 + k;
      w1r[k] = w.w1s_t[(size_t)srow * H + (kk < H ? kk : H - 1)];
    }
  }
  for (int idx = tid; idx < D * NHP; idx += kCluThreads) {
    const int k = idx / NHP, oh = idx - k * NHP;
    lds[Lwh + idx] = oh < NH ? w.wh1_t[(size_t)k * 3 * H + (oh / UH) * H + member * UH + (oh % UH)] : 0.f;
  }
  for (int i = tid; i < NHP; i += kCluThreads) { lds[Lhd + i] = 0.f; lds[Ldzh + i] = 0.f; }
  if (tid == 0) *abort_flag = 0;

  const int per_parity = kClu * 3 * D;
  unsigned long long* gbase = gran + (size_t)cluster * 2 * per_parity;
  unsigned epoch = 0;

  for (int row = cluster; row < dm.B; row += nclusters) {
    lds_barrier();
    for (int i = tid; i < UD; i += kCluThreads) lds[Lcd + i] = 0.f;
    for (int i = tid; i < S; i += kCluThreads) lds[Lcs + i] = 0.f;
    lds_barrier();

    float r0 = 0.f, r1 = 0.f, r2 = 0.f, r3 = 0.f, r4 = 0.f;
    int code_n = kModBoth;
    auto stage_load = [&](int tt) {
      const size_t q = (size_t)row * T + tt;
      code_n = modality_code<MASKED>(io.modality, q);
      if (tid < 4 * S) {
        const int which = tid / S, s2 = tid - which * S;
        const float* src = which == 0 ? io.sv_la : (which == 1 ? io.sv_lv : (which == 2 ? io.post_logits : io.prior_logits));
        r0 = src[q * S + s2];
      }
      if (tid < NH) {
        const int which = tid / UH, u = tid - which * UH;
        r1 = io.sv_heads[q * 3 * H + which * H + member * UH + u];
      } else if (tid < NH + S) {
        r1 = io.g_post_stoch ? io.g_post_stoch[q * S + (tid - NH)] : 0.f;
      }
      if (tid < 4 * UD) {
        const int g = tid / UD, u = tid - g * UD;
        r2 = io.sv_gates[q * 4 * D + g * D + member * UD + u];
      } else if (tid == 4 * UD) {
        r2 = io.g_kl ? io.g_kl[q] : 0.f;
      }
      if (tid < H) r3 = io.sv_h1[q * H + tid];
      if (tid < UD) {
        const int unit = member * UD + tid;
        r4 = tt > 0 ? io.deter[(q - 1) * D + unit] : io.deter0[(size_t)row * D + unit];
      } else if (tid >= 64 && tid < 64 + UD) {
        r4 = io.g_deter ? io.g_deter[q * D + member * UD + (tid - 64)] : 0.f;
      }
    };
    auto stage_store = [&]() {
      if (tid < 4 * S) {
        const int which = tid / S, s2 = tid - which * S;
        lds[(which == 0 ? Lla : (which == 1 ? Llv : (which == 2 ? Lmx : Llp))) + s2] = r0;
      }
      if (tid < NH) lds[Lhd + tid] = r1;
      else if (tid < NH + S) lds[Lgps + tid - NH] = r1;
      if (tid < 4 * UD) lds[Lgate + tid] = r2;
      else if (tid == 4 * UD) *gk_lds = r2;
      if (tid < H) lds[Lh1 + tid] = r3;
      if (tid < UD) lds[Ldprev + tid] = r4;
      else if (tid >= 64 && tid < 64 + UD) lds[Lgd + tid - 64] = r4;
    };
    stage_load(T - 1);

    for (int t = T - 1; t >= 0; --t) {
      const size_t bt = (size_t)row * T + t;
      unsigned long long* gpar = gbase + (size_t)(t & 1) * per_parity;

      stage_store();
      const int code = code_n;
      if (t > 0) stage_load(t - 1);
      lds_barrier();

      if (wave == 3) {
        if (C <= 8)
          cat_block_bwd_fast8(lds + Lmx, lds + Llp, K, C, lane, lds + Lgps, lds + Lcs, io.g_prior_stoch ? io.g_prior_stoch + bt * S : nullptr,
                              io.g_post_logits ? io.g_post_logits + bt * S : nullptr, io.g_prior_logits ? io.g_prior_logits + bt * S : nullptr,
                              *gk_lds, dm.kl_w_post, dm.kl_w_prior, lds + Ldmx, lds + Ldlp);
        else
          cat_block_bwd<true>(lds + Lmx, lds + Llp, K, C, lane, lds + Lgps, lds + Lcs, io.g_prior_stoch ? io.g_prior_stoch + bt * S : nullptr,
                              io.g_post_logits ? io.g_post_logits + bt * S : nullptr, io.g_prior_logits ? io.g_prior_logits + bt * S : nullptr,
                              *gk_lds, dm.kl_w_post, dm.kl_w_prior, lds + Ldmx, lds + Ldlp);
        wave_mopoe_mix_bwd_masked<true, MASKED>(lds + Lla, lds + Llv, lds + Lmx, lds + Ldmx, lds + Ldla, lds + Ldlv, lds + Ldlp, S, lane,
                                                code);
        if (member == 0) {
          for (int s2 = lane; s2 < S; s2 += kWave) {
            io.d_la[bt * S + s2] = lds[Ldla + s2];
            io.d_lv[bt * S + s2] = lds[Ldlv + s2];
            io.d_lp[bt * S + s2] = lds[Ldlp + s2];
          }
        }
      }
      lds_barrier();

      if (tid < NH) {
        const int which = tid / UH;
        const float* dl = lds + (which == 0 ? Ldlp : (which == 1 ? Ldla : Ldlv));
        const float* wc2 = lds + Lw2 + tid;
        float a0 = 0.f, a1 = 0.f;
#pragma unroll
        for (int s2 = 0; s2 < 32; s2 += 2) {
          a0 = fmaf(wc2[s2 * NHP], s2 < S ? dl[s2] : 0.f, a0);
          a1 = fmaf(wc2[(s2 + 1) * NHP], s2 + 1 < S ? dl[s2 + 1] : 0.f, a1);
        }
        const float g = (a0 + a1) * act_grad_from_out(lds[Lhd + tid], act);
        lds[Ldzh + tid] = g;
        const int u = tid - which * UH;
        io.d_zh[bt * 3 * H + which * H + member * UH + u] = g;
      }
      lds_barrier();

      ++epoch;
      if (tid < D) {
        const float* wr = lds + Lwh + (size_t)tid * NHP;
        const float* dz = lds + Ldzh;
        float p0 = 0.f, p1 = 0.f, p2 = 0.f, p3 = 0.f;
#pragma unroll
        for (int j = 0; j < NHP; j += 4) {
          const float4 a = *reinterpret_cast<const float4*>(wr + j);
          const float4 b = *reinterpret_cast<const float4*>(dz + j);
          p0 = fmaf(a.x, b.x, p0); p1 = fmaf(a.y, b.y, p1); p2 = fmaf(a.z, b.z, p2); p3 = fmaf(a.w, b.w, p3);
        }
        granule_store(gpar + (size_t)member * D + tid, epoch, (p0 + p1) + (p2 + p3));
      }
      if (wave == 3) {
        const bool ok = wave_gather_map<4>(kClu * UD, epoch, lane, [&](int i, const unsigned long long*& slot, float*& dst) {
          const int m2 = i / UD, u = i - m2 * UD;
          slot = gpar + (size_t)m2 * D + member * UD + u;
          dst = lds + Lpdd + i;
        });
        if (!ok && lane == 0) { *abort_flag = 1; atomicExch(status, 1 + 2 * t); }
      }
      lds_barrier();
      if (*abort_flag) return;

      if (tid < UD) {
        float dd = lds[Lgd + tid] + lds[Lcd + tid];
#pragma unroll
        for (int m2 = 0; m2 < kClu; ++m2) dd += lds[Lpdd + m2 * UD + tid];
        const float rg = lds[Lgate + tid], zg = lds[Lgate + UD + tid], ng = lds[Lgate + 2 * UD + tid], ghn = lds[Lgate + 3 * UD + tid];
        const float dprev = lds[Ldprev + tid];
        const float dn = dd * (1.f - zg);
        const float dz = dd * (dprev - ng);
        const float dn_pre = dn * (1.f - ng * ng);
        const float dr = dn_pre * ghn;
        const float dr_pre = dr * rg * (1.f - rg);
        const float dz_pre = dz * zg * (1.f - zg);
        lds[Lcd + tid] = dd * zg;
        lds[Ldg + tid] = dr_pre; lds[Ldg + UD + tid] = dz_pre; lds[Ldg + 2 * UD + tid] = dn_pre;
        lds[Ldg + NG + tid] = dr_pre; lds[Ldg + NG + UD + tid] = dz_pre; lds[Ldg + NG + 2 * UD + tid] = dn_pre * rg;
        const int unit = member * UD + tid;
        float* gi = io.d_gi + bt * 3 * D;
        float* gh = io.d_gh + bt * 3 * D;
        gi[unit] = dr_pre; gi[D + unit] = dz_pre; gi[2 * D + unit] = dn_pre;
        gh[unit] = dr_pre; gh[D + unit] = dz_pre; gh[2 * D + unit] = dn_pre * rg;
      }
      lds_barrier();

#pragma unroll
      for (int i = 0; i < PPT; ++i) {
        const int pc = tid * PPT + i;
        const int pcc = pc < NPIECE ? pc : NPIECE - 1;
        const int rowi = pcc / NPB, part = pcc - rowi * NPB;
        const float* xv = lds + Ldg + (rowi >= DH ? 0 : NG) + part * KPB;
        float a0 = 0.f, a1 = 0.f;
#pragma unroll
        for (int k = 0; k < KPB; k += 2) {
          const float2 x = *reinterpret_cast<const float2*>(xv + k);
          a0 = fmaf(wreg[i][k], x.x, a0);
          a1 = fmaf(wreg[i][k + 1], x.y, a1);
        }
        if (pc < NPIECE) lds[Lred + pc] = a0 + a1;
      }
      lds_barrier();
      ++epoch;
      unsigned long long* g2 = gpar + (size_t)kClu * D;
      for (int r2 = tid; r2 < 2 * DH; r2 += kCluThreads) {
        float a = 0.f;
#pragma unroll
        for (int q = 0; q < NPB; ++q) a += lds[Lred + r2 * NPB + q];
        granule_store(g2 + (size_t)member * 2 * D + r2, epoch, a);
      }
      if (wave >= 1) {
        bool ok;
        if (wave == 1) {
          ok = wave_gather_map<4>(kClu * UD, epoch, lane, [&](int i, const unsigned long long*& slot, float*& dst) {
            const int m2 = i / UD, u = i - m2 * UD;
            slot = g2 + (size_t)m2 * 2 * D + member * UD + u;
            dst = lds + Lpcd + i;
          });
        } else {
          const int mb = (wave - 2) * 2;
          ok = wave_gather_map<(2 * DH + 63) / 64>(2 * DH, epoch, lane, [&](int i, const unsigned long long*& slot, float*& dst) {
            const int m2 = mb + i / DH, k = i % DH;
            slot = g2 + (size_t)m2 * 2 * D + D + k;
            dst = lds + Lpdh + m2 * DH + k;
          });
        }
        if (!ok && lane == 0) { *abort_flag = 1; atomicExch(status, 2 + 2 * t); }
      }
      lds_barrier();
      if (*abort_flag) return;

      if (tid < UD) {
        float a = lds[Lcd + tid];
#pragma unroll
        for (int m2 = 0; m2 < kClu; ++m2) a += lds[Lpcd + m2 * UD + tid];
        lds[Lcd + tid] = a;
      }
      if (tid < H) {
        float a = 0.f;
#pragma unroll
        for (int m2 = 0; m2 < kClu; ++m2) a += lds[Lpdh + m2 * DH + tid];
        const float g = a * act_grad_from_out(lds[Lh1 + tid], act);
        lds[Ldz1 + tid] = g;
        if (member == 0) io.d_z1[bt * H + tid] = g;
      }
      lds_barrier();
      {
        const int srow = tid / W1P, part = tid % W1P;
        if (srow < S) {
          float a0 = 0.f;
#pragma unroll
          for (int k = 0; k < KW1; ++k) {
            const int kk = part * KW1 + k;
            a0 = fmaf(w1r[k], kk < H ? lds[Ldz1 + kk] : 0.f, a0);
          }
          lds[Lred2 + srow * W1P + part] = a0;
        }
      }
      lds_barrier();
      if (tid < S) {
        float a = 0.f;
#pragma unroll
        for (int q = 0; q < W1P; ++q) a += lds[Lred2 + tid * W1P + q];
        lds[Lcs + tid] = a;
      }
      lds_barrier();
    }
    if (tid < UD) io.g_deter0[(size_t)row * D + member * UD + tid] = lds[Lcd + tid];
    if (member == 0 && tid < S) io.g_stoch0[(size_t)row * S + tid] = lds[Lcs + tid];
  }
}

static int cluster_npb(int DH) { return (DH == 200 || DH == 128) ? 3 : 1; }

static size_t cluster_bwd_lds_floats(int DH, int S) {
  const int UD = DH / kClu, NG = 3 * UD, NH = NG, NHP = (NH + 3) & ~3, NPB = cluster_npb(DH), NPIECE = 2 * DH * NPB;
  size_t o = 0;
  auto take = [&](size_t n) { o += (n + 3) & ~(size_t)3; };
  for (int i = 0; i < 10; ++i) take(S);
  take(NHP); take(NHP);
  take((size_t)4 * UD); take(UD); take(UD); take(UD);
  take((size_t)2 * NG);
  take(DH); take(DH);
  take((size_t)kClu * UD);
  take((size_t)kClu * UD); take((size_t)kClu * DH);
  take((size_t)(NPIECE > DH ? NPIECE : DH));
  take((size_t)(8 * 64));
  take((size_t)DH * NHP);
  take((size_t)32 * NHP);
  take(4);
  return o;
}

size_t mrssm_cluster_bwd_workspace_bytes(const MtrssmMrssmDims* d) {
  if (!d || d->B <= 0 || d->D <= 0) return 0;
  const int nclusters = d->B < 64 ? d->B : 64;
  return 16 + (size_t)nclusters * 2 * (size_t)kClu * 3 * d->D * sizeof(unsigned long long);
}

int mrssm_cluster_supported(const MtrssmMrssmDims* d);

int mrssm_bwd_cluster_launch(const MtrssmMrssmDims* d, const MtrssmMrssmClusterWeights* w, const MtrssmMrssmBwdIO* io, void* workspace,
                             size_t workspace_bytes, hipStream_t stream) {
  if (!mrssm_cluster_supported(d) || d->K * d->C > 32) {
    set_error("mrssm_rollout_bwd_cluster: dims outside the cluster kernel's regime (ask mtrssm_mrssm_cluster_supported first; S <= 32)");
    return MTRSSM_EINVAL;
  }
  if (!w || !io || !workspace || !w->w1s_t || !w->wf_t || !w->whh_t || !w->wh1_t || !w->w4 || !w->wa2 || !w->wv2 || !io->deter0 ||
      !io->deter || !io->prior_logits || !io->post_logits || !io->sv_h1 || !io->sv_gates || !io->sv_heads || !io->sv_la || !io->sv_lv ||
      !io->g_deter0 || !io->g_stoch0 || !io->d_z1 || !io->d_gi || !io->d_gh || !io->d_zh || !io->d_lp || !io->d_la || !io->d_lv) {
    set_error("mrssm_rollout_bwd_cluster: null required pointer");
    return MTRSSM_EINVAL;
  }
  if (workspace_bytes < mrssm_cluster_bwd_workspace_bytes(d) || ((uintptr_t)workspace & 15)) {
    set_error("mrssm_rollout_bwd_cluster: workspace too small (%zu < %zu) or not 16-byte aligned", workspace_bytes,
              mrssm_cluster_bwd_workspace_bytes(d));
    return MTRSSM_EINVAL;
  }
  const int nclusters = d->B < 64 ? d->B : 64;
  const int grid = ((nclusters + 7) / 8) * 32;
  const size_t lds = cluster_bwd_lds_floats(d->D, d->K * d->C) * sizeof(float);
  if (lds > 160 * 1024) { set_error("mrssm_rollout_bwd_cluster: %zu bytes of LDS", lds); return MTRSSM_ELDS; }
  if (int rc = clear_async(static_cast<char*>(workspace) + 16, mrssm_cluster_bwd_workspace_bytes(d) - 16, stream)) return rc;
  hipError_t e = hipSuccess;
  int* status = reinterpret_cast<int*>(workspace);
  unsigned long long* gran = reinterpret_cast<unsigned long long*>(reinterpret_cast<char*>(workspace) + 16);
#define MTRSSM_CLUB_LAUNCH_M(DHV, NPV, PPTV, MV)                                                                                    \
  {                                                                                                                               \
    e = hipFuncSetAttribute(reinterpret_cast<const void*>(mrssm_bwd_cluster_kernel<DHV, NPV, PPTV, MV>),                          \
                            hipFuncAttributeMaxDynamicSharedMemorySize, (int)lds);                                               \
    if (e != hipSuccess) { set_error("hipFuncSetAttribute(max dynamic LDS=%zu): %s", lds, hipGetErrorString(e)); return MTRSSM_ELAUNCH; } \
    set_last_kernel("mtrssm::mrssm_bwd_cluster_kernel<" #DHV ", " #NPV ", " #PPTV ", " #MV ">");                                 \
    hipLaunchKernelGGL((mrssm_bwd_cluster_kernel<DHV, NPV, PPTV, MV>), dim3(grid), dim3(kCluThreads), lds, stream, *d, *w, *io,     \
                       gran, status, nclusters);                                                                                  \
  }
#define MTRSSM_CLUB_LAUNCH(DHV, NPV, PPTV)                      \
  {                                                            \
    if (io->modality) MTRSSM_CLUB_LAUNCH_M(DHV, NPV, PPTV, true) \
    else MTRSSM_CLUB_LAUNCH_M(DHV, NPV, PPTV, false)             \
  }
  if (d->D == 32) MTRSSM_CLUB_LAUNCH(32, 1, 1)
  else if (d->D == 64) MTRSSM_CLUB_LAUNCH(64, 1, 1)
  else if (d->D == 128) MTRSSM_CLUB_LAUNCH(128, 3, 3)
  else MTRSSM_CLUB_LAUNCH(200, 3, 5)
#undef MTRSSM_CLUB_LAUNCH
#undef MTRSSM_CLUB_LAUNCH_M
  e = hipGetLastError();
  if (e != hipSuccess) { set_error("cluster backward scan launch failed: %s", hipGetErrorString(e)); return MTRSSM_ELAUNCH; }
  return MTRSSM_OK;
}

int debug_set_cluster_profile(void* buf) {
  unsigned long long* p = static_cast<unsigned long long*>(buf);
  return hipMemcpyToSymbol(HIP_SYMBOL(g_cluster_prof), &p, sizeof(p)) == hipSuccess ? MTRSSM_OK : MTRSSM_ELAUNCH;
}

static int cluster_kw(int D, int H) { return D > H ? D : H; }

static int cluster_np(int DH) { return DH == 200 ? 5 : (DH == 128 ? 4 : (DH == 64 ? 2 : 1)); }

static size_t cluster_lds_floats(int D, int H, int S) {
  const int UD = D / kClu, UH = H / kClu, NG = 3 * UD, NH = 3 * UH, KW = cluster_kw(D, H), NP = cluster_np(KW);
  size_t o = 0;
  auto take = [&](size_t n) { o += (n + 3) & ~(size_t)3; };
  take(S); take(KW); take(KW); take(KW); take(3 * 64);
  take(S); take(S); take(S); take(S);
  take((size_t)kClu * 3 * S);
  take((size_t)(2 * NG * NP > NH * NP ? 2 * NG * NP : NH * NP));
  take((size_t)S * H);
  take((size_t)D * NH);
  take((size_t)3 * S);
  take(2 * 64);
  take(4);
  return o;
}

size_t mrssm_cluster_workspace_bytes(const MtrssmMrssmDims* d) {
  if (!d || d->B <= 0 || d->D <= 0 || d->K <= 0 || d->C <= 0) return 0;
  const int nclusters = d->B < 64 ? d->B : 64;
  const size_t per_parity = (size_t)kClu * (d->D / kClu + 3 * d->K * d->C);
  return 16 + (size_t)nclusters * 2 * per_parity * sizeof(unsigned long long);
}

int mrssm_cluster_supported(const MtrssmMrssmDims* d) {
  if (!d || d->B <= 0 || d->T <= 0 || d->D <= 0 || d->H <= 0 || d->K <= 0 || d->C <= 0 || !d->post) return 0;
  const int S = d->K * d->C, D = d->D, H = d->H;
  if (D != H || (D != 32 && D != 64 && D != 128 && D != 200)) return 0;
  if (3 * S > kCluThreads || H / kClu > 64 || 3 * H / kClu > kCluThreads || d->K > 64) return 0;
  if (D > 4 * kWave || kClu * 3 * S > 6 * kWave) return 0;
  if (cluster_lds_floats(D, H, S) * sizeof(float) > 160 * 1024) return 0;
  const int nclusters = d->B < 64 ? d->B : 64;
  if (device_cu_count() < ((nclusters + 7) / 8) * 32) return 0;
  return 1;
}

int mrssm_fwd_cluster_launch(const MtrssmMrssmDims* d, const MtrssmMrssmClusterWeights* w, const MtrssmMrssmFwdIO* io, void* workspace,
                             size_t workspace_bytes, hipStream_t stream) {
  if (!mrssm_cluster_supported(d)) {
    set_error("mrssm_rollout_fwd_cluster: dims outside the cluster kernel's regime (ask mtrssm_mrssm_cluster_supported first)");
    return MTRSSM_EINVAL;
  }
  if (!w || !io || !workspace || !w->w1s_t || !w->wf_t || !w->bf || !w->whh_t || !w->bhh || !w->wh1_t || !w->b3 || !w->w4 || !w->b4 ||
      !w->wa2 || !w->ba2 || !w->wv2 || !w->bv2 || !io->xa || !io->pa || !io->pv || !io->deter0 || !io->stoch0 || !io->u_post ||
      !io->deter || !io->prior_logits || !io->post_logits || !io->post_stoch) {
    set_error("mrssm_rollout_fwd_cluster: null required pointer");
    return MTRSSM_EINVAL;
  }
  if (workspace_bytes < mrssm_cluster_workspace_bytes(d) || ((uintptr_t)workspace & 15)) {
    set_error("mrssm_rollout_fwd_cluster: workspace too small (%zu < %zu) or not 16-byte aligned", workspace_bytes,
              mrssm_cluster_workspace_bytes(d));
    return MTRSSM_EINVAL;
  }
  const int nclusters = d->B < 64 ? d->B : 64;
  const int groups = (nclusters + 7) / 8;
  const int grid = groups * 32;
  const size_t lds = cluster_lds_floats(d->D, d->H, d->K * d->C) * sizeof(float);
  if (int rc = clear_async(static_cast<char*>(workspace) + 16, mrssm_cluster_workspace_bytes(d) - 16, stream)) return rc;
  hipError_t e = hipSuccess;
  int* status = reinterpret_cast<int*>(workspace);
  unsigned long long* gran = reinterpret_cast<unsigned long long*>(reinterpret_cast<char*>(workspace) + 16);
  const int kw = cluster_kw(d->D, d->H);
#define MTRSSM_CLU_LAUNCH_M(DHV, NPV, PPTV, MV)                                                                                     \
  {                                                                                                                               \
    e = hipFuncSetAttribute(reinterpret_cast<const void*>(mrssm_fwd_cluster_kernel<DHV, NPV, PPTV, MV>),                          \
                            hipFuncAttributeMaxDynamicSharedMemorySize, (int)lds);                                               \
    if (e != hipSuccess) { set_error("hipFuncSetAttribute(max dynamic LDS=%zu): %s", lds, hipGetErrorString(e)); return MTRSSM_ELAUNCH; } \
    set_last_kernel("mtrssm::mrssm_fwd_cluster_kernel<" #DHV ", " #NPV ", " #PPTV ", " #MV ">");                                 \
    hipLaunchKernelGGL((mrssm_fwd_cluster_kernel<DHV, NPV, PPTV, MV>), dim3(grid), dim3(kCluThreads), lds, stream, *d, *w, *io,     \
                       gran, status, nclusters);                                                                                  \
  }
#define MTRSSM_CLU_LAUNCH(DHV, NPV, PPTV)                      \
  {                                                           \
    if (io->modality) MTRSSM_CLU_LAUNCH_M(DHV, NPV, PPTV, true) \
    else MTRSSM_CLU_LAUNCH_M(DHV, NPV, PPTV, false)             \
  }
  if (kw == 32) MTRSSM_CLU_LAUNCH(32, 1, 1)
  else if (kw == 64) MTRSSM_CLU_LAUNCH(64, 2, 1)
  else if (kw == 128) MTRSSM_CLU_LAUNCH(128, 4, 3)
  else MTRSSM_CLU_LAUNCH(200, 5, 6)
#undef MTRSSM_CLU_LAUNCH
#undef MTRSSM_CLU_LAUNCH_M
  e = hipGetLastError();
  if (e != hipSuccess) { set_error("cluster scan launch failed: %s", hipGetErrorString(e)); return MTRSSM_ELAUNCH; }
  return MTRSSM_OK;
}

}
```

### multimodal_mtrssm_amd/scan.py

```python

from __future__ import annotations

import ctypes as C
from dataclasses import dataclass

import torch
from torch import Tensor

from multimodal_mtrssm_amd import _lib
from multimodal_mtrssm_amd.distributions import KL_BALANCE_ALPHA
from multimodal_mtrssm_amd import linear as _linear
from multimodal_mtrssm_amd.linear import gemm, gemm_group, grad_target, linear


@dataclass(frozen=True)
class ScanConfig:
    cats: int
    classes: int
    act: int
    balancing: bool = True
    rows_per_block: int = 0
    threads: int = 0

    @property
    def kl_weights(self) -> tuple[float, float]:
        return (1.0 - KL_BALANCE_ALPHA, KL_BALANCE_ALPHA) if self.balancing else (1.0, 1.0)


KERNEL_TIMERS = _lib.TIMERS
DEFER_SCAN_GRADS = True

import os as _os

CLUSTER_SCAN = _os.environ.get("MTRSSM_SCAN_CLUSTER", "1") != "0"
WIDE_SCAN = _os.environ.get("MTRSSM_SCAN_WIDE", "1") != "0"
WIDE_BWD = _os.environ.get("MTRSSM_SCAN_WIDE_BWD", "1") != "0"
WIDE_PIECES = int(_os.environ.get("MTRSSM_WIDE_PIECES", "2"))
_WS: dict[tuple, Tensor] = {}
_WS_RETIRED: list[Tensor] = []


def _workspace(device: torch.device, nbytes: int) -> Tensor:
    key = (torch.device(device).index or 0, _lib.stream_ptr(device))
    ws = _WS.get(key)
    if ws is None or ws.numel() * 8 < nbytes:
        new = torch.zeros((nbytes + 7) // 8 + 32, device=device, dtype=torch.int64)
        if ws is not None:
            new[:2].copy_(ws[:2])
            _WS_RETIRED.append(ws)
        ws = _WS[key] = new
        STATUS.watch(key, ws)
    return ws


def status_word(device: torch.device) -> Tensor | None:
    ws = _WS.get((torch.device(device).index or 0, _lib.stream_ptr(device)))
    return None if ws is None else ws[:1].view(torch.int32)[:1]


class StatusMonitor:

    def __init__(self) -> None:
        self._words: dict[tuple, Tensor] = {}
        self._pending: list[tuple[tuple, Tensor, object]] = []

    def watch(self, key: tuple, ws: Tensor) -> None:
        self._words[key] = ws

    @staticmethod
    def _raise(key: tuple, code: int) -> None:
        msg = (f"cooperative scan kernel (workspace {key}): an exchange between workgroups timed out (status {code}); the results of "
               "that step are invalid and the optimizer skipped its update.  The GPU was probably shared, partitioned or CU-masked: "
               "set MTRSSM_SCAN_CLUSTER=0 MTRSSM_SCAN_WIDE=0")
        raise _lib.MtrssmLibraryError(msg)

    def post(self) -> None:
        for key, ws in self._words.items():
            word = ws[:1].view(torch.int32)[:1]
            if word.is_cuda:
                host = torch.empty(1, dtype=torch.int32, pin_memory=True)
                host.copy_(word, non_blocking=True)
                ev = torch.cuda.Event()
                ev.record(torch.cuda.current_stream(word.device))
            else:
                host, ev = word.clone(), None
            self._pending.append((key, host, ev))

    def poll(self) -> None:
        keep = []
        for key, host, ev in self._pending:
            if ev is not None and not ev.query():
                keep.append((key, host, ev))
                continue
            code = int(host[0])
            if code:
                self._pending = []
                self._raise(key, code)
        self._pending = keep

    def check(self) -> None:
        for key, ws in self._words.items():
            code = int(ws[:1].view(torch.int32)[0].item())
            if code:
                self._raise(key, code)

    def reset(self) -> None:
        for ws in self._words.values():
            ws[:1].zero_()
        self._pending = []


STATUS = StatusMonitor()


def check_cluster_status() -> None:
    STATUS.check()


def _c(t: Tensor) -> Tensor:
    return t.contiguous()


def _flat2(t: Tensor) -> Tensor:
    return t.reshape(-1, t.shape[-1])


def _new(like: Tensor, *shape: int) -> Tensor:
    return torch.empty(shape, device=like.device, dtype=torch.float32)


def _opt(t: Tensor | None) -> Tensor | None:
    return None if t is None else _c(t)


class _WeightGrads:

    def __init__(self) -> None:
        self.own: dict[int, Tensor] = {}
        self.pending: list = []

    def _target(self, w: Tensor, rows: slice | None, cols: slice | None) -> tuple[Tensor, bool]:
        view = w
        if rows is not None:
            view = view[rows]
        if cols is not None:
            view = view[:, cols]
        tgt = grad_target(view)
        if tgt is not None:
            return tgt, True
        full = self.own.get(id(w))
        if full is None:
            full = self.own[id(w)] = torch.zeros_like(w)
        out = full
        if rows is not None:
            out = out[rows]
        if cols is not None:
            out = out[:, cols]
        return out, False

    def add(self, gy: Tensor, x: Tensor, w: Tensor, *, cols: slice | None = None, bias: Tensor | None = None) -> None:
        target, sunk = self._target(w, None, cols)
        colsum = None
        if bias is not None:
            colsum, bias_sunk = self._target(bias, None, None)
            sunk = sunk and bias_sunk
        self.pending.append((((gy, x, target), dict(a_rmajor=True, b_rmajor=True, colsum=colsum, accumulate=True)), sunk))

    def flush(self) -> None:
        now = [problem for problem, sunk in self.pending if not (DEFER_SCAN_GRADS and sunk and _linear._DEFERRED.add(problem))]
        gemm_group(now)
        self.pending = []

    def result(self, w: Tensor) -> Tensor | None:
        if self.pending:
            self.flush()
        return self.own.get(id(w))


def _modality(modality: Tensor | None, B: int, T: int) -> Tensor | None:
    if modality is None:
        return None
    if modality.dtype != torch.int32 or tuple(modality.shape) != (B, T):
        msg = f"modality codes must be int32 [{B}, {T}], got {modality.dtype} {tuple(modality.shape)}"
        raise ValueError(msg)
    return _c(modality)


def modality_codes(mask: Tensor) -> Tensor:
    return (mask[..., 0].to(torch.int32) + 2 * mask[..., 1].to(torch.int32)).contiguous()


def _projection(embed: Tensor | None, layer, deter: int, like: Tensor) -> Tensor:
    if embed is None:
        return like.new_zeros(*like.shape[:-1], layer.weight.shape[0])
    return linear(embed, layer.weight[:, deter:], layer.bias)


def _expect(**named: tuple[Tensor | None, tuple[int, ...]]) -> None:
    for name, (t, shape) in named.items():
        if t is not None and tuple(t.shape) != tuple(shape):
            msg = f"{name}: expected shape {tuple(shape)}, got {tuple(t.shape)}"
            raise ValueError(msg)


class _MrssmScan(torch.autograd.Function):

    @staticmethod
    def forward(
        ctx, cfg: ScanConfig, xa, pa, pv, deter0, stoch0, u_post, u_prior,
        w1, w2, b2, wih, bih, whh, bhh, w3, b3, w4, b4, wa1, wa2, ba2, wv1, wv2, bv2, modality=None,
    ):
        ctx.set_materialize_grads(False)
        lib = _lib.load()
        B, T, H = xa.shape
        D = deter0.shape[1]
        S = cfg.cats * cfg.classes
        A = w1.shape[1] - S
        K = cfg.cats
        _expect(pa=(pa, (B, T, H)), pv=(pv, (B, T, H)), deter0=(deter0, (B, D)), stoch0=(stoch0, (B, S)),
                u_post=(u_post, (B, T, K)), u_prior=(u_prior, (B, T, K)), w1=(w1, (H, A + S)), w2=(w2, (H, H)), b2=(b2, (H,)),
                wih=(wih, (3 * D, H)), bih=(bih, (3 * D,)), whh=(whh, (3 * D, D)), bhh=(bhh, (3 * D,)), w3=(w3, (H, D)),
                b3=(b3, (H,)), w4=(w4, (S, H)), b4=(b4, (S,)), wa2=(wa2, (S, H)), ba2=(ba2, (S,)), wv2=(wv2, (S, H)),
                bv2=(bv2, (S,)), wa1_rows=(wa1[:, :1], (H, 1)), wv1_rows=(wv1[:, :1], (H, 1)))
        if A < 0 or wa1.shape[1] <= D or wv1.shape[1] <= D:
            msg = "weight shapes are inconsistent with (deter, stoch, action, embed)"
            raise ValueError(msg)
        xa, pa, pv, deter0, stoch0, u_post = map(_c, (xa, pa, pv, deter0, stoch0, u_post))
        modality = _modality(modality, B, T)
        u_prior = _opt(u_prior)
        w1s_t = _c(w1[:, A:].t())
        wh1 = torch.cat([w3, wa1[:, :D], wv1[:, :D]], dim=0)
        whh_t, wh1_t = _c(whh.t()), _c(wh1.t())
        deter = _new(xa, B, T, D)
        prior_logits, post_logits, post_stoch = (_new(xa, B, T, S) for _ in range(3))
        prior_stoch = _new(xa, B, T, S) if u_prior is not None else None
        kl = _new(xa, B, T)
        need_grad = any(ctx.needs_input_grad)
        sv = dict(sv_h1=None, sv_h2=None, sv_gates=None, sv_heads=None, sv_la=None, sv_lv=None)
        if need_grad:
            sv = dict(sv_h1=_new(xa, B, T, H), sv_h2=_new(xa, B, T, H), sv_gates=_new(xa, B, T, 4 * D),
                      sv_heads=_new(xa, B, T, 3 * H), sv_la=_new(xa, B, T, S), sv_lv=_new(xa, B, T, S))
        io = _lib.fill(
            _lib.MrssmFwdIO(), xa=xa, pa=pa, pv=pv, deter0=deter0, stoch0=stoch0, u_post=u_post, u_prior=u_prior,
            deter=deter, prior_logits=prior_logits, prior_stoch=prior_stoch, post_logits=post_logits, post_stoch=post_stoch,
            kl=kl, **sv, modality=modality,
        )
        wp, wq = cfg.kl_weights
        dims = _lib.MrssmDims(B, T, D, H, cfg.cats, cfg.classes, cfg.act, 1, wp, wq, cfg.rows_per_block, cfg.threads)
        per_bt = 3 * H + 2 * K + D + 3 * S + 1 + (2 * H + 4 * D + 3 * H + 2 * S if need_grad else 0)
        macs = S * H + H * H + 3 * D * H + 3 * D * D + 3 * H * D + 3 * S * H
        plain = cfg.rows_per_block == 0 and cfg.threads == 0
        cluster = CLUSTER_SCAN and plain and bool(lib.mtrssm_mrssm_cluster_supported(C.byref(dims)))
        wide = WIDE_SCAN and plain and not cluster and bool(lib.mtrssm_mrssm_wide_supported(C.byref(dims), WIDE_PIECES))
        ctx.scan_kind = "cluster" if cluster else ("wide" if wide else None)
        if cluster or wide:
            wf_t = _new(xa, H, 3 * D)
            gemm(w2, wih, wf_t, a_rmajor=True, b_rmajor=False)
            bf = _new(xa, 1, 3 * D)
            gemm(b2.reshape(1, H), wih, bf, a_rmajor=False, b_rmajor=False, bias=_c(bih))
            cw = _lib.fill(_lib.MrssmClusterWeights(), w1s_t=w1s_t, wf_t=wf_t, bf=bf.reshape(-1), whh_t=whh_t, bhh=_c(bhh),
                           wh1_t=wh1_t, b3=_c(b3), w4=_c(w4), b4=_c(b4), wa2=_c(wa2), ba2=_c(ba2), wv2=_c(wv2), bv2=_c(bv2))
            io.sv_h2 = None
            stream = _lib.stream_ptr(xa.device)
            if cluster:
                ws = _workspace(xa.device, int(lib.mtrssm_mrssm_cluster_workspace_bytes(C.byref(dims))))
                _lib.check(_lib.TIMERS.call("mtrssm_mrssm_rollout_fwd_cluster", lib.mtrssm_mrssm_rollout_fwd_cluster, C.byref(dims), C.byref(cw),
                                            C.byref(io), _lib.raw_ptr(ws), ws.numel() * 8, stream,
                                            flops=2.0 * B * T * macs, nbytes=4.0 * B * T * per_bt), "mtrssm_mrssm_rollout_fwd_cluster")
            else:
                ws = _workspace(xa.device, int(lib.mtrssm_mrssm_wide_workspace_bytes(C.byref(dims), WIDE_PIECES)))
                _lib.check(_lib.TIMERS.call("mtrssm_mrssm_rollout_fwd_wide", lib.mtrssm_mrssm_rollout_fwd_wide, C.byref(dims), C.byref(cw),
                                            C.byref(io), WIDE_PIECES, _lib.raw_ptr(ws), ws.numel() * 8, stream,
                                            flops=2.0 * B * T * macs, nbytes=4.0 * B * T * per_bt), "mtrssm_mrssm_rollout_fwd_wide")
            sv["sv_h2"] = None
            ctx.cluster_w = (wf_t, whh_t, wh1_t)
        else:
            ctx.cluster_w = None
            fw = _lib.fill(
                _lib.MrssmFwdWeights(), w1s_t=w1s_t, w2_t=_c(w2.t()), b2=_c(b2), wih_t=_c(wih.t()), bih=_c(bih), whh_t=whh_t,
                bhh=_c(bhh), wh1_t=wh1_t, b3=_c(b3), w4=_c(w4), b4=_c(b4), wa2=_c(wa2), ba2=_c(ba2), wv2=_c(wv2), bv2=_c(bv2),
            )
            _lib.check(_lib.TIMERS.call("mtrssm_mrssm_rollout_fwd", lib.mtrssm_mrssm_rollout_fwd, C.byref(dims), C.byref(fw), C.byref(io),
                                        _lib.stream_ptr(xa.device), flops=2.0 * B * T * macs, nbytes=4.0 * B * T * per_bt),
                       "mtrssm_mrssm_rollout_fwd")
        if need_grad:
            ctx.cfg, ctx.A, ctx.modality = cfg, A, modality
            ctx.biases, ctx.w3 = (b2, bih, bhh, b3, b4, ba2, bv2), w3
            ctx.save_for_backward(deter0, stoch0, deter, prior_logits, post_logits, post_stoch, sv["sv_h1"], sv["sv_h2"],
                                  sv["sv_gates"], sv["sv_heads"], sv["sv_la"], sv["sv_lv"], w1s_t, wh1,
                                  w1, w2, wih, whh, w4, wa1, wa2, wv1, wv2)
        ctx.has_prior_stoch = prior_stoch is not None
        outs = (deter, prior_logits, post_logits, post_stoch, prior_stoch if prior_stoch is not None else deter.new_empty(()), kl)
        return outs

    @staticmethod
    def backward(ctx, g_deter, g_prior_logits, g_post_logits, g_post_stoch, g_prior_stoch, g_kl):
        lib = _lib.load()
        (deter0, stoch0, deter, prior_logits, post_logits, post_stoch, sv_h1, sv_h2, sv_gates, sv_heads, sv_la, sv_lv,
         w1s_t, wh1, w1, w2, wih, whh, w4, wa1, wa2, wv1, wv2) = ctx.saved_tensors
        cfg, A = ctx.cfg, ctx.A
        B, T, D = deter.shape
        H = sv_h1.shape[-1]
        S = cfg.cats * cfg.classes
        if not ctx.has_prior_stoch:
            g_prior_stoch = None
        _expect(g_deter=(g_deter, (B, T, D)), g_prior_logits=(g_prior_logits, (B, T, S)), g_post_logits=(g_post_logits, (B, T, S)),
                g_post_stoch=(g_post_stoch, (B, T, S)), g_prior_stoch=(g_prior_stoch, (B, T, S)), g_kl=(g_kl, (B, T)))
        bw = _lib.fill(_lib.MrssmBwdWeights(), w1s_t=w1s_t, w2=_c(w2), wih=_c(wih), whh=_c(whh), wh1=wh1, w4=_c(w4), wa2=_c(wa2),
                       wv2=_c(wv2))
        g_deter0, g_stoch0 = _new(deter, B, D), _new(deter, B, S)
        d_z1, d_h2 = _new(deter, B, T, H), _new(deter, B, T, H)
        d_gi, d_gh = _new(deter, B, T, 3 * D), _new(deter, B, T, 3 * D)
        d_zh = _new(deter, B, T, 3 * H)
        d_lp, d_la, d_lv = (_new(deter, B, T, S) for _ in range(3))
        io = _lib.fill(
            _lib.MrssmBwdIO(), deter0=deter0, deter=deter, prior_logits=prior_logits, post_logits=post_logits, sv_h1=sv_h1,
            sv_h2=sv_h2, sv_gates=sv_gates, sv_heads=sv_heads, sv_la=sv_la, sv_lv=sv_lv,
            g_deter=_opt(g_deter), g_post_stoch=_opt(g_post_stoch), g_prior_stoch=_opt(g_prior_stoch),
            g_post_logits=_opt(g_post_logits), g_prior_logits=_opt(g_prior_logits), g_kl=_opt(g_kl),
            g_deter0=g_deter0, g_stoch0=g_stoch0, d_z1=d_z1, d_h2=d_h2, d_gi=d_gi, d_gh=d_gh, d_zh=d_zh, d_lp=d_lp, d_la=d_la,
            d_lv=d_lv, modality=ctx.modality,
        )
        wp, wq = cfg.kl_weights
        dims = _lib.MrssmDims(B, T, D, H, cfg.cats, cfg.classes, cfg.act, 1, wp, wq, cfg.rows_per_block, cfg.threads)
        per_bt = (2 * H + 4 * D + 3 * H + 2 * S) + D + 2 * S + (D + S + 1) + 2 * H + 6 * D + 3 * H + 3 * S
        macs = S * H + H * H + 3 * D * H + 3 * D * D + 3 * H * D + 3 * S * H
        cw3 = getattr(ctx, "cluster_w", None)
        kind = getattr(ctx, "scan_kind", None)
        use_cluster = kind == "cluster" and CLUSTER_SCAN and cfg.classes * cfg.cats <= 32
        use_wide = kind == "wide" and WIDE_SCAN and WIDE_BWD
        if cw3 is not None and (use_cluster or use_wide):
            wf_t, whh_t, wh1_t = cw3
            cw = _lib.fill(_lib.MrssmClusterWeights(), w1s_t=w1s_t, wf_t=wf_t, whh_t=whh_t, wh1_t=wh1_t, w4=_c(w4), wa2=_c(wa2), wv2=_c(wv2))
            stream = _lib.stream_ptr(deter.device)
            if use_cluster:
                ws = _workspace(deter.device, int(lib.mtrssm_mrssm_cluster_bwd_workspace_bytes(C.byref(dims))))
                _lib.check(_lib.TIMERS.call("mtrssm_mrssm_rollout_bwd_cluster", lib.mtrssm_mrssm_rollout_bwd_cluster, C.byref(dims), C.byref(cw),
                                            C.byref(io), _lib.raw_ptr(ws), ws.numel() * 8, stream,
                                            flops=2.0 * B * T * macs, nbytes=4.0 * B * T * per_bt), "mtrssm_mrssm_rollout_bwd_cluster")
            else:
                ws = _workspace(deter.device, int(lib.mtrssm_mrssm_wide_bwd_workspace_bytes(C.byref(dims), WIDE_PIECES)))
                _lib.check(_lib.TIMERS.call("mtrssm_mrssm_rollout_bwd_wide", lib.mtrssm_mrssm_rollout_bwd_wide, C.byref(dims), C.byref(cw),
                                            C.byref(io), WIDE_PIECES, _lib.raw_ptr(ws), ws.numel() * 8, stream,
                                            flops=2.0 * B * T * macs, nbytes=4.0 * B * T * per_bt), "mtrssm_mrssm_rollout_bwd_wide")
            gemm(_flat2(d_gi), wih, _flat2(d_h2), a_rmajor=False, b_rmajor=True)
        else:
            _lib.check(_lib.TIMERS.call("mtrssm_mrssm_rollout_bwd", lib.mtrssm_mrssm_rollout_bwd, C.byref(dims), C.byref(bw), C.byref(io),
                                        _lib.stream_ptr(deter.device), flops=2.0 * B * T * macs, nbytes=4.0 * B * T * per_bt),
                       "mtrssm_mrssm_rollout_bwd")

        prev_stoch = _flat2(torch.cat([stoch0.unsqueeze(1), post_stoch[:, :-1]], dim=1))
        prev_deter = _flat2(torch.cat([deter0.unsqueeze(1), deter[:, :-1]], dim=1))
        fz1, fh2, fgi, fgh, fzh = map(_flat2, (d_z1, d_h2, d_gi, d_gh, d_zh))
        flp, fla, flv = map(_flat2, (d_lp, d_la, d_lv))
        (b2, bih, bhh, b3, b4, ba2, bv2) = ctx.biases
        if sv_h2 is None:
            sv_h2 = _new(deter, B, T, H)
            gemm(_flat2(sv_h1), w2, _flat2(sv_h2), a_rmajor=False, b_rmajor=False, bias=_c(b2))
        fdet, fh1, fsh2, fheads = map(_flat2, (deter, sv_h1, sv_h2, sv_heads))
        wg = _WeightGrads()
        wg.add(fz1, prev_stoch, w1, cols=slice(A, None))
        wg.add(fh2, fh1, w2, bias=b2)
        wg.add(fgi, fsh2, wih, bias=bih)
        wg.add(fgh, prev_deter, whh, bias=bhh)
        w3 = ctx.w3
        wg.add(fzh[:, :H], fdet, w3, bias=b3)
        wg.add(fzh[:, H : 2 * H], fdet, wa1, cols=slice(0, D))
        wg.add(fzh[:, 2 * H :], fdet, wv1, cols=slice(0, D))
        wg.add(flp, fheads[:, :H], w4, bias=b4)
        wg.add(fla, fheads[:, H : 2 * H], wa2, bias=ba2)
        wg.add(flv, fheads[:, 2 * H :], wv2, bias=bv2)
        g_pa, g_pv = d_zh[..., H : 2 * H], d_zh[..., 2 * H :]
        r = wg.result
        return (None, d_z1, g_pa, g_pv, g_deter0, g_stoch0, None, None,
                r(w1), r(w2), r(b2), r(wih), r(bih), r(whh), r(bhh), r(w3), r(b3), r(w4), r(b4), r(wa1), r(wa2), r(ba2), r(wv1), r(wv2),
                r(bv2), None)


def mrssm_posterior_rollout(
    transition, audio_rep, vision_rep, actions: Tensor, audio_embed: Tensor, vision_embed: Tensor,
    deter0: Tensor, stoch0: Tensor, u_post: Tensor, u_prior: Tensor | None, *, balancing: bool, rows_per_block: int = 0,
    threads: int = 0, modality: Tensor | None = None,
) -> dict[str, Tensor]:
    factory = transition.distribution_factory
    K, Cc = factory.category_size, factory.class_size
    D = transition.deterministic_size
    A = actions.shape[-1]
    l1, l2 = transition.action_state_projector.two_layer()
    p1, p2 = transition.rnn_to_prior_projector.two_layer()
    a1, a2 = audio_rep.rnn_to_post_projector.two_layer()
    v1, v2 = vision_rep.rnn_to_post_projector.two_layer()
    act_names = {transition.action_state_projector.activation_name, transition.rnn_to_prior_projector.activation_name,
                 audio_rep.rnn_to_post_projector.activation_name, vision_rep.rnn_to_post_projector.activation_name}
    if len(act_names) != 1:
        msg = f"the HIP scan uses one activation for all heads, got {sorted(act_names)}"
        raise NotImplementedError(msg)
    cfg = ScanConfig(K, Cc, _lib.ACT_IDS[act_names.pop()], balancing, rows_per_block, threads)
    xa = linear(actions, l1.weight[:, :A], l1.bias)
    pa = _projection(audio_embed, a1, D, xa)
    pv = _projection(vision_embed, v1, D, xa)
    cell = transition.rnn_cell
    deter, prior_logits, post_logits, post_stoch, prior_stoch, kl = _MrssmScan.apply(
        cfg, xa, pa, pv, deter0, stoch0, u_post, u_prior,
        l1.weight, l2.weight, l2.bias, cell.weight_ih, cell.bias_ih, cell.weight_hh, cell.bias_hh,
        p1.weight, p1.bias, p2.weight, p2.bias, a1.weight, a2.weight, a2.bias, v1.weight, v2.weight, v2.bias, modality,
    )
    return {"deter": deter, "prior_logits": prior_logits, "post_logits": post_logits, "post_stoch": post_stoch,
            "prior_stoch": prior_stoch if u_prior is not None else None, "kl": kl}


def _st_sample(logits: Tensor, cats: int, classes: int, u: Tensor) -> tuple[Tensor, Tensor]:
    from multimodal_mtrssm_amd.distributions import onehot_from_uniforms

    probs = torch.softmax(logits.reshape(*logits.shape[:-1], cats, classes), dim=-1)
    onehot = onehot_from_uniforms(probs.detach(), u)
    return (onehot + (probs - probs.detach())).flatten(start_dim=-2), probs


def _mrssm_prior_rollout_differentiable(transition, actions: Tensor, deter0: Tensor, stoch0: Tensor,
                                        u_prior: Tensor | None) -> dict[str, Tensor]:
    factory = transition.distribution_factory
    cats, classes = factory.category_size, factory.class_size
    B, T, _ = actions.shape
    cell = transition.rnn_cell
    if u_prior is None:
        u_prior = torch.rand(B, T, cats, device=actions.device)
    actions, deter, stoch, u_prior = actions.float(), deter0.float(), stoch0.float(), u_prior.float()
    deters, logits_all, stochs = [], [], []
    for t in range(T):
        x = transition.action_state_projector(_c(torch.cat([actions[:, t], stoch], dim=-1)))
        gi = linear(x, cell.weight_ih, cell.bias_ih)
        gh = linear(_c(deter), cell.weight_hh, cell.bias_hh)
        i_r, i_z, i_n = gi.chunk(3, dim=-1)
        h_r, h_z, h_n = gh.chunk(3, dim=-1)
        r, z = torch.sigmoid(i_r + h_r), torch.sigmoid(i_z + h_z)
        deter = (1.0 - z) * torch.tanh(i_n + r * h_n) + z * deter
        logits = transition.rnn_to_prior_projector(_c(deter))
        stoch, _ = _st_sample(logits, cats, classes, u_prior[:, t])
        deters.append(deter)
        logits_all.append(logits)
        stochs.append(stoch)
    return {"deter": torch.stack(deters, 1), "prior_logits": torch.stack(logits_all, 1), "prior_stoch": torch.stack(stochs, 1)}


def mrssm_prior_rollout(transition, actions: Tensor, deter0: Tensor, stoch0: Tensor, u_prior: Tensor | None,
                        *, rows_per_block: int = 0, threads: int = 0) -> dict[str, Tensor]:
    lib = _lib.load()
    if torch.is_grad_enabled() and (actions.requires_grad or deter0.requires_grad or stoch0.requires_grad
                                    or any(p.requires_grad for p in transition.parameters())):
        return _mrssm_prior_rollout_differentiable(transition, actions, deter0, stoch0, u_prior)
    with torch.no_grad():
        factory = transition.distribution_factory
        K, Cc = factory.category_size, factory.class_size
        S = K * Cc
        B, T, A = actions.shape
        D, H = transition.deterministic_size, transition.hidden_size
        l1, l2 = transition.action_state_projector.two_layer()
        p1, p2 = transition.rnn_to_prior_projector.two_layer()
        cell = transition.rnn_cell
        if u_prior is None:
            u_prior = torch.rand(B, T, K, device=actions.device)
        xa = _c(linear(actions, l1.weight[:, :A], l1.bias))
        tensors = dict(w1s_t=_c(l1.weight[:, A:].t()), w2_t=_c(l2.weight.t()), b2=_c(l2.bias), wih_t=_c(cell.weight_ih.t()),
                       bih=_c(cell.bias_ih), whh_t=_c(cell.weight_hh.t()), bhh=_c(cell.bias_hh), wh1_t=_c(p1.weight.t()),
                       b3=_c(p1.bias), w4=_c(p2.weight), b4=_c(p2.bias))
        fw = _lib.fill(_lib.MrssmFwdWeights(), **tensors)
        deter, prior_logits, prior_stoch = _new(xa, B, T, D), _new(xa, B, T, S), _new(xa, B, T, S)
        deter0, stoch0, u_prior = _c(deter0.float()), _c(stoch0.float()), _c(u_prior.float())
        _expect(deter0=(deter0, (B, D)), stoch0=(stoch0, (B, S)), u_prior=(u_prior, (B, T, K)), xa=(xa, (B, T, H)),
                w1=(l1.weight, (H, A + S)), wih=(cell.weight_ih, (3 * D, H)), whh=(cell.weight_hh, (3 * D, D)),
                w3=(p1.weight, (H, D)), w4=(p2.weight, (S, H)))
        io = _lib.fill(_lib.MrssmFwdIO(), xa=xa, deter0=deter0, stoch0=stoch0, u_prior=u_prior, deter=deter,
                       prior_logits=prior_logits, prior_stoch=prior_stoch)
        act = _lib.ACT_IDS[transition.action_state_projector.activation_name]
        dims = _lib.MrssmDims(B, T, D, H, K, Cc, act, 0, 1.0, 1.0, rows_per_block, threads)
        _lib.check(lib.mtrssm_mrssm_rollout_fwd(C.byref(dims), C.byref(fw), C.byref(io), _lib.stream_ptr(xa.device)),
                   "mtrssm_mrssm_rollout_fwd(prior-only)")
        del tensors
    return {"deter": deter, "prior_logits": prior_logits, "prior_stoch": prior_stoch}


@dataclass(frozen=True)
class MTScanConfig:
    kl_cats: int
    kl_classes: int
    kh_cats: int
    kh_classes: int
    act: int
    tau_l: float
    tau_h: float
    balancing: bool = True
    rows_per_block: int = 0
    threads: int = 0

    @property
    def kl_weights(self) -> tuple[float, float]:
        return (1.0 - KL_BALANCE_ALPHA, KL_BALANCE_ALPHA) if self.balancing else (1.0, 1.0)

    def dims(self, B: int, T: int, LD: int, HD: int, H: int, post: int) -> C.Structure:
        wp, wq = self.kl_weights
        return _lib.MmtrssmDims(B, T, LD, HD, H, self.kl_cats, self.kl_classes, self.kh_cats, self.kh_classes, self.act, post,
                                self.tau_l, self.tau_h, 1.0 - 1.0 / self.tau_l, 1.0 - 1.0 / self.tau_h, wp, wq,
                                self.rows_per_block, self.threads)


class _MmtrssmScan(torch.autograd.Function):
    @staticmethod
    def forward(
        ctx, cfg: MTScanConfig, xl, pa, pv, deter_l0, deter_h0, hidden_l0, hidden_h0, stoch_l0, stoch_h0,
        u_post_l, u_post_h, u_prior_l, u_prior_h,
        wxl, wdl, wxh, wdh, bh, wlp1, blp1, wlp2, blp2, wa1, wa2, ba2, wv1, wv2, bv2, whp1, bhp1, whp2, bhp2, whq1, bhq1, whq2, bhq2,
        modality=None,
    ):
        ctx.set_materialize_grads(False)
        lib = _lib.load()
        B, T, LD = xl.shape
        HD = deter_h0.shape[1]
        H = pa.shape[-1]
        LS, HS = cfg.kl_cats * cfg.kl_classes, cfg.kh_cats * cfg.kh_classes
        A = wxl.shape[1] - LS - HS
        _expect(pa=(pa, (B, T, H)), pv=(pv, (B, T, H)), deter_l0=(deter_l0, (B, LD)), deter_h0=(deter_h0, (B, HD)),
                hidden_l0=(hidden_l0, (B, LD)), hidden_h0=(hidden_h0, (B, HD)), stoch_l0=(stoch_l0, (B, LS)),
                stoch_h0=(stoch_h0, (B, HS)), u_post_l=(u_post_l, (B, T, cfg.kl_cats)), u_post_h=(u_post_h, (B, T, cfg.kh_cats)),
                u_prior_l=(u_prior_l, (B, T, cfg.kl_cats)), u_prior_h=(u_prior_h, (B, T, cfg.kh_cats)),
                wxl=(wxl, (LD, A + LS + HS)), wdl=(wdl, (LD, LD)), wxh=(wxh, (HD, HS)), wdh=(wdh, (HD, HD)), bh=(bh, (HD,)),
                wlp1=(wlp1, (H, LD)), blp1=(blp1, (H,)), wlp2=(wlp2, (LS, H)), blp2=(blp2, (LS,)), wa2=(wa2, (LS, H)),
                ba2=(ba2, (LS,)), wv2=(wv2, (LS, H)), bv2=(bv2, (LS,)), whp1=(whp1, (H, HD)), bhp1=(bhp1, (H,)),
                whp2=(whp2, (HS, H)), bhp2=(bhp2, (HS,)), whq1=(whq1, (H, LD + HD)), bhq1=(bhq1, (H,)), whq2=(whq2, (HS, H)),
                bhq2=(bhq2, (HS,)), wa1_rows=(wa1[:, :1], (H, 1)), wv1_rows=(wv1[:, :1], (H, 1)))
        if A < 0 or wa1.shape[1] <= LD or wv1.shape[1] <= LD:
            msg = "weight shapes are inconsistent with (ld, ls, hs, action, embed)"
            raise ValueError(msg)
        (xl, pa, pv, deter_l0, deter_h0, hidden_l0, hidden_h0, stoch_l0, stoch_h0, u_post_l, u_post_h) = map(
            _c, (xl, pa, pv, deter_l0, deter_h0, hidden_l0, hidden_h0, stoch_l0, stoch_h0, u_post_l, u_post_h))
        u_prior_l, u_prior_h = _opt(u_prior_l), _opt(u_prior_h)
        wxl_s_t = _c(wxl[:, A:].t())
        wxh_t = _c(wxh.t())
        wl1 = torch.cat([wlp1, wa1[:, :LD], wv1[:, :LD], whq1[:, :LD]], dim=0)
        wh1 = torch.cat([whp1, whq1[:, LD:]], dim=0)
        bh1 = torch.cat([bhp1, bhq1], dim=0)
        tensors = dict(wxl_s_t=wxl_s_t, wdl_t=_c(wdl.t()), wxh_t=wxh_t, wdh_t=_c(wdh.t()), bh=_c(bh), wl1_t=_c(wl1.t()),
                       bl1=_c(blp1), wh1_t=_c(wh1.t()), bh1=bh1, wlp2=_c(wlp2), blp2=_c(blp2), wa2=_c(wa2), ba2=_c(ba2),
                       wv2=_c(wv2), bv2=_c(bv2), whp2=_c(whp2), bhp2=_c(bhp2), whq2=_c(whq2), bhq2=_c(bhq2))
        fw = _lib.fill(_lib.MmtrssmFwdWeights(), **tensors)
        o = dict(
            deter_l=_new(xl, B, T, LD), deter_h=_new(xl, B, T, HD), hidden_l=_new(xl, B, T, LD), hidden_h=_new(xl, B, T, HD),
            prior_logits_l=_new(xl, B, T, LS), prior_logits_h=_new(xl, B, T, HS),
            prior_stoch_l=_new(xl, B, T, LS) if u_prior_l is not None else None,
            prior_stoch_h=_new(xl, B, T, HS) if u_prior_h is not None else None,
            post_logits_l=_new(xl, B, T, LS), post_logits_h=_new(xl, B, T, HS),
            post_stoch_l=_new(xl, B, T, LS), post_stoch_h=_new(xl, B, T, HS), kl_l=_new(xl, B, T), kl_h=_new(xl, B, T),
        )
        modality = _modality(modality, B, T)
        need_grad = any(ctx.needs_input_grad)
        sv = dict(sv_l1=None, sv_h1=None, sv_la=None, sv_lv=None)
        if need_grad:
            sv = dict(sv_l1=_new(xl, B, T, 4 * H), sv_h1=_new(xl, B, T, H), sv_la=_new(xl, B, T, LS), sv_lv=_new(xl, B, T, LS))
        io = _lib.fill(
            _lib.MmtrssmFwdIO(), xl=xl, pa=pa, pv=pv, deter_l0=deter_l0, deter_h0=deter_h0, hidden_l0=hidden_l0,
            hidden_h0=hidden_h0, stoch_l0=stoch_l0, stoch_h0=stoch_h0, u_post_l=u_post_l, u_post_h=u_post_h,
            u_prior_l=u_prior_l, u_prior_h=u_prior_h, **o, **sv, modality=modality,
        )
        dims = cfg.dims(B, T, LD, HD, H, 1)
        macs = (LS + HS) * LD + LD * LD + HS * HD + HD * HD + 4 * H * LD + 2 * H * HD + 3 * LS * H + 2 * HS * H
        per_bt = LD + 2 * H + 2 * (LD + HD) + 2 * (LS + HS) + 2 * (LS + HS) + 2 + (5 * H + 2 * LS if need_grad else 0)
        wide = (WIDE_SCAN and cfg.rows_per_block == 0 and cfg.threads == 0
                and bool(lib.mtrssm_mmtrssm_wide_supported(C.byref(dims), WIDE_PIECES)))
        ctx.scan_kind = "wide" if wide else None
        if wide:
            ws = _workspace(xl.device, int(lib.mtrssm_mmtrssm_wide_workspace_bytes(C.byref(dims), WIDE_PIECES)))
            _lib.check(_lib.TIMERS.call("mtrssm_mmtrssm_rollout_fwd_wide", lib.mtrssm_mmtrssm_rollout_fwd_wide, C.byref(dims), C.byref(fw),
                                         C.byref(io), WIDE_PIECES, _lib.raw_ptr(ws), ws.numel() * 8, _lib.stream_ptr(xl.device),
                                         flops=2.0 * B * T * macs, nbytes=4.0 * B * T * per_bt), "mtrssm_mmtrssm_rollout_fwd_wide")
        else:
            _lib.check(_lib.TIMERS.call("mtrssm_mmtrssm_rollout_fwd", lib.mtrssm_mmtrssm_rollout_fwd, C.byref(dims), C.byref(fw), C.byref(io),
                                         _lib.stream_ptr(xl.device), flops=2.0 * B * T * macs, nbytes=4.0 * B * T * per_bt),
                       "mtrssm_mmtrssm_rollout_fwd")
        del tensors
        if need_grad:
            ctx.cfg, ctx.A, ctx.modality = cfg, A, modality
            ctx.biases, ctx.first_layers = (bh, blp1, blp2, ba2, bv2, bhp1, bhp2, bhq1, bhq2), (wlp1, whp1)
            ctx.save_for_backward(
                deter_l0, deter_h0, stoch_l0, stoch_h0, o["deter_l"], o["deter_h"], o["prior_logits_l"], o["prior_logits_h"],
                o["post_logits_l"], o["post_logits_h"], o["post_stoch_l"], o["post_stoch_h"], sv["sv_l1"], sv["sv_h1"],
                sv["sv_la"], sv["sv_lv"], wxl_s_t, wxh_t, wl1, wh1, wxl, wdl, wxh, wdh, wlp2, wa1, wa2, wv1, wv2, whp2, whq1, whq2)
        ctx.has_prior = (o["prior_stoch_l"] is not None, o["prior_stoch_h"] is not None)
        z = o["deter_l"].new_empty(())
        return (o["deter_l"], o["deter_h"], o["hidden_l"], o["hidden_h"], o["prior_logits_l"], o["prior_logits_h"],
                o["post_logits_l"], o["post_logits_h"], o["post_stoch_l"], o["post_stoch_h"],
                o["prior_stoch_l"] if o["prior_stoch_l"] is not None else z,
                o["prior_stoch_h"] if o["prior_stoch_h"] is not None else z, o["kl_l"], o["kl_h"])

    @staticmethod
    def backward(ctx, g_dl, g_dh, g_hl, g_hh, g_pll, g_plh, g_qll, g_qlh, g_qsl, g_qsh, g_psl, g_psh, g_kll, g_klh):
        lib = _lib.load()
        (deter_l0, deter_h0, stoch_l0, stoch_h0, deter_l, deter_h, prior_logits_l, prior_logits_h, post_logits_l, post_logits_h,
         post_stoch_l, post_stoch_h, sv_l1, sv_h1, sv_la, sv_lv, wxl_s_t, wxh_t, wl1, wh1, wxl, wdl, wxh, wdh, wlp2, wa1, wa2,
         wv1, wv2, whp2, whq1, whq2) = ctx.saved_tensors
        cfg, A = ctx.cfg, ctx.A
        B, T, LD = deter_l.shape
        HD = deter_h.shape[-1]
        H = sv_h1.shape[-1]
        LS, HS = cfg.kl_cats * cfg.kl_classes, cfg.kh_cats * cfg.kh_classes
        if not ctx.has_prior[0]:
            g_psl = None
        if not ctx.has_prior[1]:
            g_psh = None
        bw = _lib.fill(_lib.MmtrssmBwdWeights(), wxl_s_t=wxl_s_t, wdl=_c(wdl), wxh_t=wxh_t, wdh=_c(wdh), wl1=wl1, wh1=wh1,
                       wlp2=_c(wlp2), wa2=_c(wa2), wv2=_c(wv2), whp2=_c(whp2), whq2=_c(whq2))
        g0 = dict(g_deter_l0=_new(deter_l, B, LD), g_deter_h0=_new(deter_l, B, HD), g_hidden_l0=_new(deter_l, B, LD),
                  g_hidden_h0=_new(deter_l, B, HD), g_stoch_l0=_new(deter_l, B, LS), g_stoch_h0=_new(deter_l, B, HS))
        d = dict(d_ul=_new(deter_l, B, T, LD), d_uh=_new(deter_l, B, T, HD), d_zl1=_new(deter_l, B, T, 4 * H),
                 d_zh1=_new(deter_l, B, T, H), d_lpl=_new(deter_l, B, T, LS), d_la=_new(deter_l, B, T, LS),
                 d_lv=_new(deter_l, B, T, LS), d_lph=_new(deter_l, B, T, HS), d_lqh=_new(deter_l, B, T, HS))
        io = _lib.fill(
            _lib.MmtrssmBwdIO(), deter_l0=deter_l0, deter_h0=deter_h0, deter_l=deter_l, deter_h=deter_h,
            prior_logits_l=prior_logits_l, prior_logits_h=prior_logits_h, post_logits_l=post_logits_l, post_logits_h=post_logits_h,
            sv_l1=sv_l1, sv_h1=sv_h1, sv_la=sv_la, sv_lv=sv_lv,
            g_deter_l=_opt(g_dl), g_deter_h=_opt(g_dh), g_hidden_l=_opt(g_hl), g_hidden_h=_opt(g_hh),
            g_post_stoch_l=_opt(g_qsl), g_post_stoch_h=_opt(g_qsh), g_prior_stoch_l=_opt(g_psl), g_prior_stoch_h=_opt(g_psh),
            g_post_logits_l=_opt(g_qll), g_post_logits_h=_opt(g_qlh), g_prior_logits_l=_opt(g_pll), g_prior_logits_h=_opt(g_plh),
            g_kl_l=_opt(g_kll), g_kl_h=_opt(g_klh), **g0, **d, modality=ctx.modality,
        )
        dims = cfg.dims(B, T, LD, HD, H, 1)
        macs = (LS + HS) * LD + LD * LD + HS * HD + HD * HD + 4 * H * LD + 2 * H * HD + 3 * LS * H + 2 * HS * H
        per_bt = 5 * H + 2 * LS + 4 * (LD + HD) + 4 * (LS + HS) + 2 * (LD + HD) + 5 * H + 3 * LS + 2 * HS
        if getattr(ctx, "scan_kind", None) == "wide" and WIDE_SCAN and WIDE_BWD:
            ws = _workspace(deter_l.device, int(lib.mtrssm_mmtrssm_wide_bwd_workspace_bytes(C.byref(dims), WIDE_PIECES)))
            _lib.check(_lib.TIMERS.call("mtrssm_mmtrssm_rollout_bwd_wide", lib.mtrssm_mmtrssm_rollout_bwd_wide, C.byref(dims), C.byref(bw),
                                         C.byref(io), WIDE_PIECES, _lib.raw_ptr(ws), ws.numel() * 8, _lib.stream_ptr(deter_l.device),
                                         flops=2.0 * B * T * macs, nbytes=4.0 * B * T * per_bt), "mtrssm_mmtrssm_rollout_bwd_wide")
        else:
            _lib.check(_lib.TIMERS.call("mtrssm_mmtrssm_rollout_bwd", lib.mtrssm_mmtrssm_rollout_bwd, C.byref(dims), C.byref(bw), C.byref(io),
                                         _lib.stream_ptr(deter_l.device), flops=2.0 * B * T * macs, nbytes=4.0 * B * T * per_bt),
                       "mtrssm_mmtrssm_rollout_bwd")

        prev_sl = torch.cat([stoch_l0.unsqueeze(1), post_stoch_l[:, :-1]], dim=1)
        prev_sh = torch.cat([stoch_h0.unsqueeze(1), post_stoch_h[:, :-1]], dim=1)
        prev_slh = _flat2(torch.cat([prev_sl, prev_sh], dim=-1))
        prev_dl = _flat2(torch.cat([deter_l0.unsqueeze(1), deter_l[:, :-1]], dim=1))
        prev_dh = _flat2(torch.cat([deter_h0.unsqueeze(1), deter_h[:, :-1]], dim=1))
        ful, fuh, fzl, fzh = map(_flat2, (d["d_ul"], d["d_uh"], d["d_zl1"], d["d_zh1"]))
        flpl, fla, flv, flph, flqh = map(_flat2, (d["d_lpl"], d["d_la"], d["d_lv"], d["d_lph"], d["d_lqh"]))
        fdl, fdh, fl1, fh1 = map(_flat2, (deter_l, deter_h, sv_l1, sv_h1))
        (bh, blp1, blp2, ba2, bv2, bhp1, bhp2, bhq1, bhq2) = ctx.biases
        wlp1, whp1 = ctx.first_layers
        wg = _WeightGrads()
        wg.add(ful, prev_slh, wxl, cols=slice(A, None))
        wg.add(ful, prev_dl, wdl)
        wg.add(fuh, prev_slh[:, LS:], wxh, bias=bh)
        wg.add(fuh, prev_dh, wdh)
        wg.add(fzl[:, :H], fdl, wlp1, bias=blp1)
        wg.add(fzl[:, H : 2 * H], fdl, wa1, cols=slice(0, LD))
        wg.add(fzl[:, 2 * H : 3 * H], fdl, wv1, cols=slice(0, LD))
        fzq = fzl[:, 3 * H :]
        wg.add(fzq, fdl, whq1, cols=slice(0, LD), bias=bhq1)
        wg.add(fzq, fdh, whq1, cols=slice(LD, None))
        wg.add(fzh, fdh, whp1, bias=bhp1)
        wg.add(flpl, fl1[:, :H], wlp2, bias=blp2)
        wg.add(fla, fl1[:, H : 2 * H], wa2, bias=ba2)
        wg.add(flv, fl1[:, 2 * H : 3 * H], wv2, bias=bv2)
        wg.add(flqh, fl1[:, 3 * H :], whq2, bias=bhq2)
        wg.add(flph, fh1, whp2, bias=bhp2)
        zl = d["d_zl1"]
        r = wg.result
        return (None, d["d_ul"], zl[..., H : 2 * H], zl[..., 2 * H : 3 * H], g0["g_deter_l0"], g0["g_deter_h0"], g0["g_hidden_l0"],
                g0["g_hidden_h0"], g0["g_stoch_l0"], g0["g_stoch_h0"], None, None, None, None,
                r(wxl), r(wdl), r(wxh), r(wdh), r(bh), r(wlp1), r(blp1), r(wlp2), r(blp2), r(wa1), r(wa2), r(ba2), r(wv1), r(wv2), r(bv2),
                r(whp1), r(bhp1), r(whp2), r(bhp2), r(whq1), r(bhq1), r(whq2), r(bhq2), None)


def _mt_act(model) -> int:
    names = {model.l_prior.activation_name, model.h_prior.activation_name, model.h_posterior.activation_name,
             model.audio_representation.rnn_to_post_projector.activation_name,
             model.vision_representation.rnn_to_post_projector.activation_name}
    if len(names) != 1:
        msg = f"the HIP scan uses one activation for all heads, got {sorted(names)}"
        raise NotImplementedError(msg)
    return _lib.ACT_IDS[names.pop()]


def mmtrssm_posterior_rollout(model, actions: Tensor, audio_embed: Tensor, vision_embed: Tensor, state0: dict[str, Tensor],
                              noise: dict[str, Tensor | None], *, rows_per_block: int = 0, threads: int = 0,
                              modality: Tensor | None = None) -> dict[str, Tensor]:
    LD = model.ld_dim
    A = actions.shape[-1]
    cfg = MTScanConfig(model.l_dist.category_size, model.l_dist.class_size, model.h_dist.category_size, model.h_dist.class_size,
                       _mt_act(model), float(model.l_rnn.tau), float(model.h_rnn.tau), bool(model.use_kl_balancing),
                       rows_per_block, threads)
    lp1, lp2 = model.l_prior.two_layer()
    hp1, hp2 = model.h_prior.two_layer()
    hq1, hq2 = model.h_posterior.two_layer()
    a1, a2 = model.audio_representation.rnn_to_post_projector.two_layer()
    v1, v2 = model.vision_representation.rnn_to_post_projector.two_layer()
    lr, hr = model.l_rnn, model.h_rnn
    xl = linear(actions, lr._input2h.weight[:, :A], lr._input2h.bias + lr._d2h.bias)
    pa = _projection(audio_embed, a1, LD, xl)
    pv = _projection(vision_embed, v1, LD, xl)
    bh = hr._input2h.bias + hr._d2h.bias
    out = _MmtrssmScan.apply(
        cfg, xl, pa, pv, state0["deter_l"], state0["deter_h"], state0["hidden_l"], state0["hidden_h"], state0["stoch_l"],
        state0["stoch_h"], noise["u_post_l"], noise["u_post_h"], noise.get("u_prior_l"), noise.get("u_prior_h"),
        lr._input2h.weight, lr._d2h.weight, hr._input2h.weight, hr._d2h.weight, bh,
        lp1.weight, lp1.bias, lp2.weight, lp2.bias, a1.weight, a2.weight, a2.bias, v1.weight, v2.weight, v2.bias,
        hp1.weight, hp1.bias, hp2.weight, hp2.bias, hq1.weight, hq1.bias, hq2.weight, hq2.bias, modality,
    )
    names = ("deter_l", "deter_h", "hidden_l", "hidden_h", "prior_logits_l", "prior_logits_h", "post_logits_l", "post_logits_h",
             "post_stoch_l", "post_stoch_h", "prior_stoch_l", "prior_stoch_h", "kl_l", "kl_h")
    res = dict(zip(names, out, strict=True))
    if noise.get("u_prior_l") is None:
        res["prior_stoch_l"] = None
    if noise.get("u_prior_h") is None:
        res["prior_stoch_h"] = None
    return res


def _mtrnn_step(rnn, x: Tensor, deter: Tensor, hidden: Tensor) -> tuple[Tensor, Tensor]:
    pre = linear(_c(deter), rnn._d2h.weight, rnn._d2h.bias) + linear(_c(x), rnn._input2h.weight, rnn._input2h.bias)
    hidden = (1.0 - 1.0 / rnn.tau) * hidden + pre / rnn.tau
    return torch.tanh(hidden), hidden


def _mmtrssm_prior_rollout_differentiable(model, actions: Tensor, state0: dict[str, Tensor],
                                          noise: dict[str, Tensor | None]) -> dict[str, Tensor]:
    kl, cl = model.l_dist.category_size, model.l_dist.class_size
    kh, ch = model.h_dist.category_size, model.h_dist.class_size
    B, T, _ = actions.shape
    u_l, u_h = noise.get("u_prior_l"), noise.get("u_prior_h")
    u_l = torch.rand(B, T, kl, device=actions.device) if u_l is None else u_l.float()
    u_h = torch.rand(B, T, kh, device=actions.device) if u_h is None else u_h.float()
    st = {k: state0[k].float() for k in ("deter_l", "deter_h", "hidden_l", "hidden_h", "stoch_l", "stoch_h")}
    deter_l, deter_h, hidden_l, hidden_h, stoch_l, stoch_h = (st[k] for k in ("deter_l", "deter_h", "hidden_l", "hidden_h", "stoch_l", "stoch_h"))
    names = ("deter_l", "deter_h", "hidden_l", "hidden_h", "prior_logits_l", "prior_logits_h", "prior_stoch_l", "prior_stoch_h")
    keep: dict[str, list[Tensor]] = {k: [] for k in names}
    actions = actions.float()
    for t in range(T):
        deter_l, hidden_l = _mtrnn_step(model.l_rnn, torch.cat([actions[:, t], stoch_l, stoch_h], dim=-1), deter_l, hidden_l)
        logits_l = model.l_prior(_c(deter_l))
        deter_h, hidden_h = _mtrnn_step(model.h_rnn, stoch_h, deter_h, hidden_h)
        logits_h = model.h_prior(_c(deter_h))
        stoch_h, _ = _st_sample(logits_h, kh, ch, u_h[:, t])
        stoch_l, _ = _st_sample(logits_l, kl, cl, u_l[:, t])
        for k, v in zip(names, (deter_l, deter_h, hidden_l, hidden_h, logits_l, logits_h, stoch_l, stoch_h), strict=True):
            keep[k].append(v)
    return {k: torch.stack(v, dim=1) for k, v in keep.items()}


def mmtrssm_prior_rollout(model, actions: Tensor, state0: dict[str, Tensor], noise: dict[str, Tensor | None],
                          *, rows_per_block: int = 0, threads: int = 0) -> dict[str, Tensor]:
    lib = _lib.load()
    if torch.is_grad_enabled() and (actions.requires_grad or any(v is not None and v.requires_grad for v in state0.values())
                                    or any(p.requires_grad for m in (model.l_rnn, model.h_rnn, model.l_prior, model.h_prior)
                                           for p in m.parameters())):
        return _mmtrssm_prior_rollout_differentiable(model, actions, state0, noise)
    with torch.no_grad():
        LD, HD = model.ld_dim, model.hd_dim
        B, T, A = actions.shape
        cfg = MTScanConfig(model.l_dist.category_size, model.l_dist.class_size, model.h_dist.category_size,
                           model.h_dist.class_size, _mt_act(model), float(model.l_rnn.tau), float(model.h_rnn.tau), True,
                           rows_per_block, threads)
        LS, HS = cfg.kl_cats * cfg.kl_classes, cfg.kh_cats * cfg.kh_classes
        lp1, lp2 = model.l_prior.two_layer()
        hp1, hp2 = model.h_prior.two_layer()
        H = lp1.out_features
        lr, hr = model.l_rnn, model.h_rnn
        xl = _c(linear(actions, lr._input2h.weight[:, :A], lr._input2h.bias + lr._d2h.bias))
        tensors = dict(
            wxl_s_t=_c(lr._input2h.weight[:, A:].t()), wdl_t=_c(lr._d2h.weight.t()), wxh_t=_c(hr._input2h.weight.t()),
            wdh_t=_c(hr._d2h.weight.t()), bh=_c(hr._input2h.bias + hr._d2h.bias), wl1_t=_c(lp1.weight.t()), bl1=_c(lp1.bias),
            wh1_t=_c(hp1.weight.t()), bh1=_c(hp1.bias), wlp2=_c(lp2.weight), blp2=_c(lp2.bias), whp2=_c(hp2.weight), bhp2=_c(hp2.bias))
        fw = _lib.fill(_lib.MmtrssmFwdWeights(), **tensors)
        u_l = noise.get("u_prior_l")
        u_h = noise.get("u_prior_h")
        u_l = torch.rand(B, T, cfg.kl_cats, device=xl.device) if u_l is None else _c(u_l.float())
        u_h = torch.rand(B, T, cfg.kh_cats, device=xl.device) if u_h is None else _c(u_h.float())
        o = dict(deter_l=_new(xl, B, T, LD), deter_h=_new(xl, B, T, HD), hidden_l=_new(xl, B, T, LD), hidden_h=_new(xl, B, T, HD),
                 prior_logits_l=_new(xl, B, T, LS), prior_logits_h=_new(xl, B, T, HS), prior_stoch_l=_new(xl, B, T, LS),
                 prior_stoch_h=_new(xl, B, T, HS))
        st = {k: _c(state0[k].float()) for k in ("deter_l", "deter_h", "hidden_l", "hidden_h", "stoch_l", "stoch_h")}
        _expect(deter_l=(st["deter_l"], (B, LD)), deter_h=(st["deter_h"], (B, HD)), hidden_l=(st["hidden_l"], (B, LD)),
                hidden_h=(st["hidden_h"], (B, HD)), stoch_l=(st["stoch_l"], (B, LS)), stoch_h=(st["stoch_h"], (B, HS)),
                u_prior_l=(u_l, (B, T, cfg.kl_cats)), u_prior_h=(u_h, (B, T, cfg.kh_cats)),
                wxl=(lr._input2h.weight, (LD, A + LS + HS)), wdl=(lr._d2h.weight, (LD, LD)),
                wxh=(hr._input2h.weight, (HD, HS)), wdh=(hr._d2h.weight, (HD, HD)), wlp1=(lp1.weight, (H, LD)),
                wlp2=(lp2.weight, (LS, H)), whp1=(hp1.weight, (H, HD)), whp2=(hp2.weight, (HS, H)))
        io = _lib.fill(_lib.MmtrssmFwdIO(), xl=xl, deter_l0=st["deter_l"], deter_h0=st["deter_h"], hidden_l0=st["hidden_l"],
                       hidden_h0=st["hidden_h"], stoch_l0=st["stoch_l"], stoch_h0=st["stoch_h"], u_prior_l=u_l, u_prior_h=u_h, **o)
        dims = cfg.dims(B, T, LD, HD, H, 0)
        _lib.check(lib.mtrssm_mmtrssm_rollout_fwd(C.byref(dims), C.byref(fw), C.byref(io), _lib.stream_ptr(xl.device)),
                   "mtrssm_mmtrssm_rollout_fwd(prior-only)")
        del tensors
    return o
```

Baseline: 368,100 seq-steps/s.

## Keep head-projection weights in registers in the cluster forward scan

Adds a RESH template variant of the cluster forward kernel. It keeps each thread's slice of the wh1 head weights resident in registers across timesteps instead of reading them from LDS. The per-row output-head weights (w4/wa2/wv2) move from a 64-float per-thread register array into padded LDS rows, and the gate and head biases are staged in LDS. The goal is to cut LDS traffic in the per-step head matvec while rebalancing register pressure. It also adds backward profiling stamps and a runtime toggle, which is on by default.

New measurement: 370,600 seq-steps/s (median of 6 runs). No clear change (+0.7%).

```diff
diff --git a/include/mtrssm.h b/include/mtrssm.h
--- a/include/mtrssm.h
+++ b/include/mtrssm.h
@@ -99,6 +99,7 @@
 int64_t mtrssm_mrssm_cluster_workspace_bytes(const MtrssmMrssmDims* dims);
 int mtrssm_mrssm_rollout_fwd_cluster(const MtrssmMrssmDims* dims, const MtrssmMrssmClusterWeights* weights, const MtrssmMrssmFwdIO* io,
                                      void* workspace, int64_t workspace_bytes, void* stream);
+int mtrssm_mrssm_cluster_set_resident_heads(int32_t on);
 
 typedef struct MtrssmMrssmBwdWeights {
   const float* w1s_t;
diff --git a/multimodal_mtrssm_amd/_lib.py b/multimodal_mtrssm_amd/_lib.py
--- a/multimodal_mtrssm_amd/_lib.py
+++ b/multimodal_mtrssm_amd/_lib.py
@@ -89,6 +89,7 @@
     "mtrssm_mrssm_cluster_supported": (C.c_int, [C.POINTER(MrssmDims)]),
     "mtrssm_mrssm_cluster_workspace_bytes": (C.c_int64, [C.POINTER(MrssmDims)]),
     "mtrssm_mrssm_rollout_fwd_cluster": (C.c_int, [C.POINTER(MrssmDims), C.POINTER(MrssmClusterWeights), C.POINTER(MrssmFwdIO), _p, C.c_int64, _p]),
+    "mtrssm_mrssm_cluster_set_resident_heads": (C.c_int, [_i]),
     "mtrssm_mrssm_cluster_bwd_workspace_bytes": (C.c_int64, [C.POINTER(MrssmDims)]),
     "mtrssm_mrssm_rollout_bwd_cluster": (C.c_int, [C.POINTER(MrssmDims), C.POINTER(MrssmClusterWeights), C.POINTER(MrssmBwdIO), _p, C.c_int64, _p]),
     "mtrssm_mrssm_wide_supported": (C.c_int, [C.POINTER(MrssmDims), _i]),
diff --git a/multimodal_mtrssm_amd/csrc/capi.hip b/multimodal_mtrssm_amd/csrc/capi.hip
--- a/multimodal_mtrssm_amd/csrc/capi.hip
+++ b/multimodal_mtrssm_amd/csrc/capi.hip
@@ -80,6 +80,7 @@
 int gemm_launch(const MtrssmGemm*, hipStream_t);
 int gemm_group_launch(const MtrssmGemm*, int, hipStream_t);
 int debug_set_cluster_profile(void*);
+void mrssm_cluster_set_resident_heads(int);
 int debug_set_resident_profile(void*);
 int debug_set_wide_profile(void*);
 int debug_set_mmt_profile(void*);
@@ -192,6 +193,10 @@
                                                 void* workspace, int64_t workspace_bytes, void* stream) {
   return mrssm_fwd_cluster_launch(d, w, io, workspace, workspace_bytes < 0 ? 0 : (size_t)workspace_bytes, static_cast<hipStream_t>(stream));
 }
+MTRSSM_API int mtrssm_mrssm_cluster_set_resident_heads(int32_t on) {
+  mrssm_cluster_set_resident_heads(on);
+  return MTRSSM_OK;
+}
 extern "C" __attribute__((visibility("default"))) int mtrssm_debug_set_cluster_profile(void* buf) { return debug_set_cluster_profile(buf); }
 extern "C" __attribute__((visibility("default"))) int mtrssm_debug_set_resident_profile(void* buf) { return debug_set_resident_profile(buf); }
 extern "C" __attribute__((visibility("default"))) int mtrssm_debug_set_wide_profile(void* buf) { return debug_set_wide_profile(buf); }
diff --git a/multimodal_mtrssm_amd/csrc/mrssm_cluster.hip b/multimodal_mtrssm_amd/csrc/mrssm_cluster.hip
--- a/multimodal_mtrssm_amd/csrc/mrssm_cluster.hip
+++ b/multimodal_mtrssm_amd/csrc/mrssm_cluster.hip
@@ -14,6 +14,10 @@
 #define MTRSSM_CLU_STAMP(i)                                                                                  \
   do {                                                                                                       \
     if (prof && t >= 8 && t < 12) prof[(t - 8) * 16 + (i)] = __builtin_readcyclecounter();                   \
+  } while (0)
+#define MTRSSM_CLUB_STAMP(i)                                                                                 \
+  do {                                                                                                       \
+    if (prof && t >= 8 && t < 12) prof[64 + (t - 8) * 16 + (i)] = __builtin_readcyclecounter();              \
   } while (0)
 
 __device__ __forceinline__ void granule_store(unsigned long long* p, unsigned epoch, float v) {
@@ -45,7 +49,7 @@
   }
 }
 
-template <int DH, int NP, int PPT, bool MASKED>
+template <int DH, int NP, int PPT, bool MASKED, bool RESH>
 __global__ __launch_bounds__(kCluThreads) void mrssm_fwd_cluster_kernel(const MtrssmMrssmDims dm, const MtrssmMrssmClusterWeights w,
                                                                         const MtrssmMrssmFwdIO io, unsigned long long* __restrict__ gran,
                                                                         int* __restrict__ status, int nclusters) {
@@ -55,6 +59,10 @@
   constexpr int NG = 3 * UD, NH = 3 * UH;
   constexpr int KP = DH / NP;
   constexpr int NPIECE = 2 * NG * NP;
+  constexpr int NHPIECE = NH * NP;
+  constexpr int PPH = (NHPIECE + kCluThreads - 1) / kCluThreads;
+  constexpr int UHQ = (UH + 3) & ~3;
+  constexpr int WST = UHQ | 4;
   static_assert(KP % 4 == 0 && DH % NP == 0, "pieces are whole float4 runs");
   static_assert(PPT * kCluThreads >= NPIECE, "every piece has a thread");
   const int K = dm.K, C = dm.C, S = K * C, T = dm.T, act = dm.act;
@@ -69,10 +77,12 @@
   const int Ls = take(S), Lh1 = take(DH), Ld0 = take(DH), Ld1 = take(DH), Lhd = take(3 * 64);
   const int Llp = take(S), Lla = take(S), Llv = take(S), Lmx = take(S);
   const int Lpart = take(kClu * 3 * S);
-  const int Lred = take(NPIECE > NH * NP ? NPIECE : NH * NP);
+  const int Lred = take(NPIECE > NHPIECE ? NPIECE : NHPIECE);
   const int Lw1 = take(S * H);
-  const int Lwh = take(D * NH);
+  const int Lwh = take(RESH ? 0 : D * NH);
   const int Lbl = take(3 * S);
+  const int Lwr = take(RESH ? 3 * S * WST : 0);
+  const int Lbg = take(RESH ? 6 * UD + UH : 0);
   const int Lu = take(2 * 64);
   const int Lflag = take(4);
   (void)o;
@@ -93,8 +103,15 @@
 #pragma unroll
     for (int k = 0; k < KP; ++k) wreg[i][k] = src[(size_t)k * 3 * D];
   }
-  float wrow[64];
-  {
+  float wrow[RESH ? 1 : 64];
+  if constexpr (RESH) {
+    wrow[0] = 0.f;
+    for (int idx = tid; idx < 3 * S * WST; idx += kCluThreads) {
+      const int r = idx / WST, k = idx - r * WST;
+      const int which = r / S, srow = r - which * S;
+      lds[Lwr + idx] = k < UH ? (which == 0 ? w.w4 : (which == 1 ? w.wa2 : w.wv2))[(size_t)srow * H + member * UH + k] : 0.f;
+    }
+  } else {
     const bool roleL = tid < 3 * S;
     const int which = roleL ? tid / S : 0, srow = roleL ? tid - which * S : 0;
     const float* rowsrc = (which == 0 ? w.w4 : (which == 1 ? w.wa2 : w.wv2)) + (size_t)srow * H + member * UH;
@@ -102,9 +119,26 @@
     for (int k = 0; k < 64; ++k) wrow[k] = k < UH ? rowsrc[k] : 0.f;
   }
   for (int idx = tid; idx < S * H; idx += kCluThreads) lds[Lw1 + idx] = w.w1s_t[idx];
-  for (int idx = tid; idx < D * NH; idx += kCluThreads) {
-    const int k = idx / NH, oh = idx - k * NH;
-    lds[Lwh + idx] = w.wh1_t[(size_t)k * 3 * H + (oh / UH) * H + member * UH + (oh % UH)];
+  float hreg[RESH ? PPH : 1][RESH ? KP : 1];
+  static_assert(PPH <= 4 && DH <= 256, "the pieces' offsets into d_new are packed into one register, eight bits each");
+  int hoff = 0;
+  if constexpr (RESH) {
+#pragma unroll
+    for (int i = 0; i < PPH; ++i) {
+      const int pc = tid * PPH + i;
+      const int pcc = pc < NHPIECE ? pc : NHPIECE - 1;
+      const int oh = pcc / NP, part = pcc - oh * NP;
+      const float* src = w.wh1_t + (size_t)(part * KP) * 3 * H + (oh / UH) * H + member * UH + (oh % UH);
+      hoff |= (part * KP) << (8 * i);
+#pragma unroll
+      for (int k = 0; k < KP; ++k) hreg[i][k] = src[(size_t)k * 3 * H];
+    }
+  } else {
+    hreg[0][0] = 0.f;
+    for (int idx = tid; idx < D * NH; idx += kCluThreads) {
+      const int k = idx / NH, oh = idx - k * NH;
+      lds[Lwh + idx] = w.wh1_t[(size_t)k * 3 * H + (oh / UH) * H + member * UH + (oh % UH)];
+    }
   }
   for (int i = tid; i < 3 * 64; i += kCluThreads) lds[Lhd + i] = 0.f;
   for (int i = tid; i < 3 * S; i += kCluThreads) {
@@ -120,6 +154,13 @@
     }
   }
   const float bias_h = (tid < UH) ? w.b3[member * UH + tid] : 0.f;
+  if constexpr (RESH) {
+    if (tid < UD) {
+#pragma unroll
+      for (int g = 0; g < 6; ++g) lds[Lbg + g * UD + tid] = bias_g[g];
+    }
+    if (tid < UH) lds[Lbg + 6 * UD + tid] = bias_h;
+  }
   if (tid == 0) *abort_flag = 0;
 
   const int slotsD = UD, slotsL = 3 * S;
@@ -201,7 +242,7 @@
 #pragma unroll
         for (int g = 0; g < 6; ++g) {
           const float* pr = lds + Lred + ((g < 3 ? g : g - 3) * UD + tid + (g < 3 ? 0 : NG)) * NP;
-          float a = bias_g[g];
+          float a = RESH ? lds[Lbg + g * UD + tid] : bias_g[g];
 #pragma unroll
           for (int q = 0; q < NP; ++q) a += pr[q];
           gs[g] = a;
@@ -227,26 +268,43 @@
       if (*abort_flag) return;
 
       MTRSSM_CLU_STAMP(3);
-      for (int pc = tid; pc < NH * NP; pc += kCluThreads) {
-        const int oh = pc / NP, part = pc - oh * NP;
-        const float* wcol = lds + Lwh + (size_t)(part * KP) * NH + oh;
-        const float* dv = lds + nxt + part * KP;
-        float p0 = 0.f, p1 = 0.f, p2 = 0.f, p3 = 0.f;
-#pragma unroll
-        for (int k = 0; k < KP; k += 8) {
-          float wv[8];
-#pragma unroll
-          for (int i = 0; i < 8; ++i) wv[i] = k + i < KP ? wcol[(size_t)(k + i) * NH] : 0.f;
-          const float4 d0 = *reinterpret_cast<const float4*>(dv + k);
-          const float4 d1 = k + 4 < KP ? *reinterpret_cast<const float4*>(dv + k + 4) : make_float4(0.f, 0.f, 0.f, 0.f);
-          p0 = fmaf(wv[0], d0.x, p0); p1 = fmaf(wv[1], d0.y, p1); p2 = fmaf(wv[2], d0.z, p2); p3 = fmaf(wv[3], d0.w, p3);
-          p0 = fmaf(wv[4], d1.x, p0); p1 = fmaf(wv[5], d1.y, p1); p2 = fmaf(wv[6], d1.z, p2); p3 = fmaf(wv[7], d1.w, p3);
-        }
-        lds[Lred + pc] = (p0 + p1) + (p2 + p3);
+      if constexpr (RESH) {
+#pragma unroll
+        for (int i = 0; i < PPH; ++i) {
+          const float* dv = lds + nxt + ((hoff >> (8 * i)) & 255);
+          float p0 = 0.f, p1 = 0.f, p2 = 0.f, p3 = 0.f;
+#pragma unroll
+          for (int k = 0; k < KP; k += 4) {
+            const float4 x = *reinterpret_cast<const float4*>(dv + k);
+            p0 = fmaf(hreg[i][k], x.x, p0);
+            p1 = fmaf(hreg[i][k + 1], x.y, p1);
+            p2 = fmaf(hreg[i][k + 2], x.z, p2);
+            p3 = fmaf(hreg[i][k + 3], x.w, p3);
+          }
+          if (tid * PPH + i < NHPIECE) lds[Lred + tid * PPH + i] = (p0 + p1) + (p2 + p3);
+        }
+      } else {
+        for (int pc = tid; pc < NHPIECE; pc += kCluThreads) {
+          const int oh = pc / NP, part = pc - oh * NP;
+          const float* wcol = lds + Lwh + (size_t)(part * KP) * NH + oh;
+          const float* dv = lds + nxt + part * KP;
+          float p0 = 0.f, p1 = 0.f, p2 = 0.f, p3 = 0.f;
+#pragma unroll
+          for (int k = 0; k < KP; k += 8) {
+            float wv[8];
+#pragma unroll
+            for (int i = 0; i < 8; ++i) wv[i] = k + i < KP ? wcol[(size_t)(k + i) * NH] : 0.f;
+            const float4 d0 = *reinterpret_cast<const float4*>(dv + k);
+            const float4 d1 = k + 4 < KP ? *reinterpret_cast<const float4*>(dv + k + 4) : make_float4(0.f, 0.f, 0.f, 0.f);
+            p0 = fmaf(wv[0], d0.x, p0); p1 = fmaf(wv[1], d0.y, p1); p2 = fmaf(wv[2], d0.z, p2); p3 = fmaf(wv[3], d0.w, p3);
+            p0 = fmaf(wv[4], d1.x, p0); p1 = fmaf(wv[5], d1.y, p1); p2 = fmaf(wv[6], d1.z, p2); p3 = fmaf(wv[7], d1.w, p3);
+          }
+          lds[Lred + pc] = (p0 + p1) + (p2 + p3);
+        }
       }
       lds_barrier();
       if (tid < NH) {
-        float z = tid < UH ? bias_h : pav;
+        float z = tid < UH ? (RESH ? lds[Lbg + 6 * UD + tid] : bias_h) : pav;
 #pragma unroll
         for (int q = 0; q < NP; ++q) z += lds[Lred + tid * NP + q];
         const float h = act_fwd(z, act);
@@ -262,13 +320,26 @@
       if (tid < 3 * S) {
         const float* hv = lds + Lhd + (tid / S) * 64;
         float p0 = 0.f, p1 = 0.f;
-#pragma unroll
-        for (int u = 0; u < 64; u += 4) {
-          const float4 x = *reinterpret_cast<const float4*>(hv + u);
-          p0 = fmaf(wrow[u], x.x, p0);
-          p1 = fmaf(wrow[u + 1], x.y, p1);
-          p0 = fmaf(wrow[u + 2], x.z, p0);
-          p1 = fmaf(wrow[u + 3], x.w, p1);
+        if constexpr (RESH) {
+          const float* wr = lds + Lwr + tid * WST;
+#pragma unroll
+          for (int u = 0; u < UHQ; u += 4) {
+            const float4 x = *reinterpret_cast<const float4*>(hv + u);
+            const float4 y = *reinterpret_cast<const float4*>(wr + u);
+            p0 = fmaf(y.x, x.x, p0);
+            p1 = fmaf(y.y, x.y, p1);
+            p0 = fmaf(y.z, x.z, p0);
+            p1 = fmaf(y.w, x.w, p1);
+          }
+        } else {
+#pragma unroll
+          for (int u = 0; u < 64; u += 4) {
+            const float4 x = *reinterpret_cast<const float4*>(hv + u);
+            p0 = fmaf(wrow[u], x.x, p0);
+            p1 = fmaf(wrow[u + 1], x.y, p1);
+            p0 = fmaf(wrow[u + 2], x.z, p0);
+            p1 = fmaf(wrow[u + 3], x.w, p1);
+          }
         }
         const float p = p0 + p1;
         lds[Lpart + member * 3 * S + tid] = p;
@@ -425,6 +496,7 @@
   const int per_parity = kClu * 3 * D;
   unsigned long long* gbase = gran + (size_t)cluster * 2 * per_parity;
   unsigned epoch = 0;
+  unsigned long long* prof = (blockIdx.x == 0 && tid == 0) ? g_cluster_prof : nullptr;
 
   for (int row = cluster; row < dm.B; row += nclusters) {
     lds_barrier();
@@ -481,11 +553,13 @@
       const size_t bt = (size_t)row * T + t;
       unsigned long long* gpar = gbase + (size_t)(t & 1) * per_parity;
 
+      MTRSSM_CLUB_STAMP(0);
       stage_store();
       const int code = code_n;
       if (t > 0) stage_load(t - 1);
       lds_barrier();
 
+      MTRSSM_CLUB_STAMP(1);
       if (wave == 3) {
         if (C <= 8)
           cat_block_bwd_fast8(lds + Lmx, lds + Llp, K, C, lane, lds + Lgps, lds + Lcs, io.g_prior_stoch ? io.g_prior_stoch + bt * S : nullptr,
@@ -507,6 +581,7 @@
       }
       lds_barrier();
 
+      MTRSSM_CLUB_STAMP(2);
       if (tid < NH) {
         const int which = tid / UH;
         const float* dl = lds + (which == 0 ? Ldlp : (which == 1 ? Ldla : Ldlv));
@@ -524,6 +599,7 @@
       }
       lds_barrier();
 
+      MTRSSM_CLUB_STAMP(3);
       ++epoch;
       if (tid < D) {
         const float* wr = lds + Lwh + (size_t)tid * NHP;
@@ -548,6 +624,7 @@
       lds_barrier();
       if (*abort_flag) return;
 
+      MTRSSM_CLUB_STAMP(4);
       if (tid < UD) {
         float dd = lds[Lgd + tid] + lds[Lcd + tid];
 #pragma unroll
@@ -571,6 +648,7 @@
       }
       lds_barrier();
 
+      MTRSSM_CLUB_STAMP(5);
 #pragma unroll
       for (int i = 0; i < PPT; ++i) {
         const int pc = tid * PPT + i;
@@ -616,6 +694,7 @@
       lds_barrier();
       if (*abort_flag) return;
 
+      MTRSSM_CLUB_STAMP(6);
       if (tid < UD) {
         float a = lds[Lcd + tid];
 #pragma unroll
@@ -631,6 +710,7 @@
         if (member == 0) io.d_z1[bt * H + tid] = g;
       }
       lds_barrier();
+      MTRSSM_CLUB_STAMP(7);
       {
         const int srow = tid / W1P, part = tid % W1P;
         if (srow < S) {
@@ -651,6 +731,7 @@
         lds[Lcs + tid] = a;
       }
       lds_barrier();
+      MTRSSM_CLUB_STAMP(8);
     }
     if (tid < UD) io.g_deter0[(size_t)row * D + member * UD + tid] = lds[Lcd + tid];
     if (member == 0 && tid < S) io.g_stoch0[(size_t)row * S + tid] = lds[Lcs + tid];
@@ -745,7 +826,10 @@
 
 static int cluster_np(int DH) { return DH == 200 ? 5 : (DH == 128 ? 4 : (DH == 64 ? 2 : 1)); }
 
-static size_t cluster_lds_floats(int D, int H, int S) {
+static int g_resident_heads = 1;
+void mrssm_cluster_set_resident_heads(int on) { g_resident_heads = on ? 1 : 0; }
+
+static size_t cluster_lds_floats(int D, int H, int S, bool resident_heads) {
   const int UD = D / kClu, UH = H / kClu, NG = 3 * UD, NH = 3 * UH, KW = cluster_kw(D, H), NP = cluster_np(KW);
   size_t o = 0;
   auto take = [&](size_t n) { o += (n + 3) & ~(size_t)3; };
@@ -754,8 +838,10 @@
   take((size_t)kClu * 3 * S);
   take((size_t)(2 * NG * NP > NH * NP ? 2 * NG * NP : NH * NP));
   take((size_t)S * H);
-  take((size_t)D * NH);
+  take(resident_heads ? 0 : (size_t)D * NH);
   take((size_t)3 * S);
+  take(resident_heads ? (size_t)3 * S * (((UH + 3) & ~3) | 4) : 0);
+  take(resident_heads ? (size_t)6 * UD + UH : 0);
   take(2 * 64);
   take(4);
   return o;
@@ -774,7 +860,7 @@
   if (D != H || (D != 32 && D != 64 && D != 128 && D != 200)) return 0;
   if (3 * S > kCluThreads || H / kClu > 64 || 3 * H / kClu > kCluThreads || d->K > 64) return 0;
   if (D > 4 * kWave || kClu * 3 * S > 6 * kWave) return 0;
-  if (cluster_lds_floats(D, H, S) * sizeof(float) > 160 * 1024) return 0;
+  if (cluster_lds_floats(D, H, S, g_resident_heads != 0) * sizeof(float) > 160 * 1024) return 0;
   const int nclusters = d->B < 64 ? d->B : 64;
   if (device_cu_count() < ((nclusters + 7) / 8) * 32) return 0;
   return 1;
@@ -800,25 +886,32 @@
   const int nclusters = d->B < 64 ? d->B : 64;
   const int groups = (nclusters + 7) / 8;
   const int grid = groups * 32;
-  const size_t lds = cluster_lds_floats(d->D, d->H, d->K * d->C) * sizeof(float);
+  const bool resident = g_resident_heads != 0;
+  const size_t lds = cluster_lds_floats(d->D, d->H, d->K * d->C, resident) * sizeof(float);
+  if (lds > 160 * 1024) { set_error("mrssm_rollout_fwd_cluster: %zu bytes of LDS", lds); return MTRSSM_ELDS; }
   if (int rc = clear_async(static_cast<char*>(workspace) + 16, mrssm_cluster_workspace_bytes(d) - 16, stream)) return rc;
   hipError_t e = hipSuccess;
   int* status = reinterpret_cast<int*>(workspace);
   unsigned long long* gran = reinterpret_cast<unsigned long long*>(reinterpret_cast<char*>(workspace) + 16);
   const int kw = cluster_kw(d->D, d->H);
-#define MTRSSM_CLU_LAUNCH_M(DHV, NPV, PPTV, MV)                                                                                     \
+#define MTRSSM_CLU_LAUNCH_M(DHV, NPV, PPTV, MV, RV)                                                                                 \
   {                                                                                                                               \
-    e = hipFuncSetAttribute(reinterpret_cast<const void*>(mrssm_fwd_cluster_kernel<DHV, NPV, PPTV, MV>),                          \
+    e = hipFuncSetAttribute(reinterpret_cast<const void*>(mrssm_fwd_cluster_kernel<DHV, NPV, PPTV, MV, RV>),                      \
                             hipFuncAttributeMaxDynamicSharedMemorySize, (int)lds);                                               \
     if (e != hipSuccess) { set_error("hipFuncSetAttribute(max dynamic LDS=%zu): %s", lds, hipGetErrorString(e)); return MTRSSM_ELAUNCH; } \
-    set_last_kernel("mtrssm::mrssm_fwd_cluster_kernel<" #DHV ", " #NPV ", " #PPTV ", " #MV ">");                                 \
-    hipLaunchKernelGGL((mrssm_fwd_cluster_kernel<DHV, NPV, PPTV, MV>), dim3(grid), dim3(kCluThreads), lds, stream, *d, *w, *io,     \
+    set_last_kernel("mtrssm::mrssm_fwd_cluster_kernel<" #DHV ", " #NPV ", " #PPTV ", " #MV ", " #RV ">");                        \
+    hipLaunchKernelGGL((mrssm_fwd_cluster_kernel<DHV, NPV, PPTV, MV, RV>), dim3(grid), dim3(kCluThreads), lds, stream, *d, *w, *io, \
                        gran, status, nclusters);                                                                                  \
   }
-#define MTRSSM_CLU_LAUNCH(DHV, NPV, PPTV)                      \
-  {                                                           \
-    if (io->modality) MTRSSM_CLU_LAUNCH_M(DHV, NPV, PPTV, true) \
-    else MTRSSM_CLU_LAUNCH_M(DHV, NPV, PPTV, false)             \
+#define MTRSSM_CLU_LAUNCH(DHV, NPV, PPTV)                                         \
+  {                                                                              \
+    if (io->modality) {                                                          \
+      if (resident) MTRSSM_CLU_LAUNCH_M(DHV, NPV, PPTV, true, true)              \
+      else MTRSSM_CLU_LAUNCH_M(DHV, NPV, PPTV, true, false)                      \
+    } else {                                                                     \
+      if (resident) MTRSSM_CLU_LAUNCH_M(DHV, NPV, PPTV, false, true)             \
+      else MTRSSM_CLU_LAUNCH_M(DHV, NPV, PPTV, false, false)                     \
+    }                                                                            \
   }
   if (kw == 32) MTRSSM_CLU_LAUNCH(32, 1, 1)
   else if (kw == 64) MTRSSM_CLU_LAUNCH(64, 2, 1)
diff --git a/multimodal_mtrssm_amd/scan.py b/multimodal_mtrssm_amd/scan.py
--- a/multimodal_mtrssm_amd/scan.py
+++ b/multimodal_mtrssm_amd/scan.py
@@ -33,6 +33,7 @@
 import os as _os
 
 CLUSTER_SCAN = _os.environ.get("MTRSSM_SCAN_CLUSTER", "1") != "0"
+CLUSTER_RESIDENT_HEADS = _os.environ.get("MTRSSM_CLUSTER_RESIDENT_HEADS", "1") != "0"
 WIDE_SCAN = _os.environ.get("MTRSSM_SCAN_WIDE", "1") != "0"
 WIDE_BWD = _os.environ.get("MTRSSM_SCAN_WIDE_BWD", "1") != "0"
 WIDE_PIECES = int(_os.environ.get("MTRSSM_WIDE_PIECES", "2"))
@@ -250,6 +251,8 @@
         per_bt = 3 * H + 2 * K + D + 3 * S + 1 + (2 * H + 4 * D + 3 * H + 2 * S if need_grad else 0)
         macs = S * H + H * H + 3 * D * H + 3 * D * D + 3 * H * D + 3 * S * H
         plain = cfg.rows_per_block == 0 and cfg.threads == 0
+        if CLUSTER_SCAN and plain:
+            lib.mtrssm_mrssm_cluster_set_resident_heads(int(CLUSTER_RESIDENT_HEADS))
         cluster = CLUSTER_SCAN and plain and bool(lib.mtrssm_mrssm_cluster_supported(C.byref(dims)))
         wide = WIDE_SCAN and plain and not cluster and bool(lib.mtrssm_mrssm_wide_supported(C.byref(dims), WIDE_PIECES))
         ctx.scan_kind = "cluster" if cluster else ("wide" if wide else None)
```
